# geekieo/collaborative-deep-metric-learning

Hardware: NVIDIA B200
Metric: train_triplets_per_sec (higher is better)
Workload: dtype fp16 operands / fp32 accumulate (tcgen05 kind::f16), fp32 master weights

## Files before the change

collaborative-deep-metric-learning_b200/csrc/gemm_launch.cuh:

```cuda
#pragma once
#include "../../include/cdml.h"
#include "ctx.cuh"
#include "gemm_sm100.cuh"
#include "gemm2_sm100.cuh"

#include <stdlib.h>

namespace cdml {

inline bool trace_on() {
  static int on = -1;
  if (on < 0) on = getenv("CDML_TRACE") != nullptr ? 1 : 0;
  return on == 1;
}
inline int trace_sync(const char* what, long M, long N, long K, int grid, cudaStream_t st) {
  if (!trace_on()) return 0;
  fprintf(stderr, "[cdml] %s M=%ld N=%ld K=%ld grid=%d ... ", what, M, N, K, grid);
  fflush(stderr);
  cudaError_t e = cudaStreamSynchronize(st);
  fprintf(stderr, "%s\n", cudaGetErrorString(e));
  fflush(stderr);
  return e == cudaSuccess ? 0 : -2;
}

constexpr int kBN = 256;
constexpr int kStages = 4;

inline int pick_splits(int num_sms, int tiles, int num_kb) {
  if (tiles >= 2 * num_sms || num_kb < 16) return 1;
  const int smax = max(1, min(64, num_kb / 8));
  int best = 1;
  double best_eff = -1.0;
  for (int s = 1; s <= smax; ++s) {
    const int per = (num_kb + s - 1) / s;
    const int seff = (num_kb + per - 1) / per;
    if (seff != s) continue;
    const long units = static_cast<long>(tiles) * s;
    const long waves = (units + num_sms - 1) / num_sms;
    double eff = static_cast<double>(units) / static_cast<double>(waves * num_sms);
    if (units < num_sms) eff *= 0.5;
    eff -= 0.002 * s;
    if (eff > best_eff) best_eff = eff, best = s;
  }
  return best;
}

inline bool two_cta_enabled() {
  static int on = -1;
  if (on < 0) {
    const char* e = getenv("CDML_2CTA");
    on = (e != nullptr && e[0] == '0') ? 0 : 1;
  }
  return on == 1;
}

template <int AMN, int BMN, class Epi>
static int launch_gemm2(cdml_ctx* ctx, const void* A, int64_t lda, const void* B, int64_t ldb, int64_t M, int64_t N,
                        int64_t K, int dtype16, int num_splits, const Epi& epi, cudaStream_t stream) {
  using L = Gemm2Smem;
  CUtensorMap ta, tb;
  int rc;
  if (AMN == 0) rc = make_tmap_2d(ctx, &ta, A, dtype16, K, M, lda, kBK, kBM);
  else rc = make_tmap_2d(ctx, &ta, A, dtype16, M, K, lda, 64, kBK);
  if (rc) return rc;
  if (BMN == 0) rc = make_tmap_2d(ctx, &tb, B, dtype16, K, N, ldb, kBK, kBN2 / 2);
  else rc = make_tmap_2d(ctx, &tb, B, dtype16, N, K, ldb, 64, kBK);
  if (rc) return rc;
  GemmShape s;
  s.M = static_cast<int>(M), s.N = static_cast<int>(N), s.K = static_cast<int>(K);
  s.m_tiles = (s.M + 2 * kBM - 1) / (2 * kBM);
  s.n_tiles = (s.N + kBN2 - 1) / kBN2;
  s.num_kb = (s.K + kBK - 1) / kBK;
  num_splits = max(1, min(num_splits, s.num_kb));
  s.kb_per_split = (s.num_kb + num_splits - 1) / num_splits;
  s.num_splits = (s.num_kb + s.kb_per_split - 1) / s.kb_per_split;
  s.idesc = make_idesc_f16(dtype16 == CDML_BF16 ? 1 : 0, AMN, BMN, 2 * kBM, kBN2);
  s.m_fastest = (s.num_splits > 1 && N >= M) ? 1 : 0;
  auto kern = gemm2_tcgen05_kernel<AMN, BMN, Epi>;
  static bool attr_set = false;
  if (!attr_set) {
    CDML_CHECK_CUDA(cudaFuncSetAttribute(kern, cudaFuncAttributeMaxDynamicSharedMemorySize, L::kTotal));
    attr_set = true;
  }
  const long units = static_cast<long>(s.m_tiles) * s.n_tiles * s.num_splits;
  const int clusters = static_cast<int>(units < ctx->num_sms / 2 ? units : ctx->num_sms / 2);
  cudaLaunchConfig_t cfg = {};
  cfg.gridDim = dim3(2 * clusters);
  cfg.blockDim = dim3(kGemmThreads);
  cfg.dynamicSmemBytes = L::kTotal;
  cfg.stream = stream;
  cudaLaunchAttribute attr[1];
  attr[0].id = cudaLaunchAttributeClusterDimension;
  attr[0].val.clusterDim.x = 2, attr[0].val.clusterDim.y = 1, attr[0].val.clusterDim.z = 1;
  cfg.attrs = attr;
  cfg.numAttrs = 1;
  CDML_CHECK_CUDA(cudaLaunchKernelEx(&cfg, kern, ta, tb, s, epi));
  if (trace_sync("gemm2_tcgen05", M, N, K, 2 * clusters, stream)) return -2;
  return s.num_splits;
}

template <int AMN, int BMN, class Epi>
static int launch_gemm(cdml_ctx* ctx, const void* A, int64_t lda, const void* B, int64_t ldb, int64_t M, int64_t N,
                       int64_t K, int dtype16, int num_splits, const Epi& epi, cudaStream_t stream) {
  {
    const int64_t kb_per = ((K + kBK - 1) / kBK + max(num_splits, 1) - 1) / max(num_splits, 1);
    if (two_cta_enabled() && M >= 2 * kBM && kb_per >= 8)
      return launch_gemm2<AMN, BMN>(ctx, A, lda, B, ldb, M, N, K, dtype16, num_splits, epi, stream);
  }
  using L = GemmSmem<kBN, kStages>;
  CUtensorMap ta, tb;
  int rc;
  if (AMN == 0) rc = make_tmap_2d(ctx, &ta, A, dtype16, K, M, lda, kBK, kBM);
  else rc = make_tmap_2d(ctx, &ta, A, dtype16, M, K, lda, 64, kBK);
  if (rc) return rc;
  if (BMN == 0) rc = make_tmap_2d(ctx, &tb, B, dtype16, K, N, ldb, kBK, kBN);
  else rc = make_tmap_2d(ctx, &tb, B, dtype16, N, K, ldb, 64, kBK);
  if (rc) return rc;

  GemmShape s;
  s.M = static_cast<int>(M), s.N = static_cast<int>(N), s.K = static_cast<int>(K);
  s.m_tiles = (s.M + kBM - 1) / kBM;
  s.n_tiles = (s.N + kBN - 1) / kBN;
  s.num_kb = (s.K + kBK - 1) / kBK;
  num_splits = max(1, min(num_splits, s.num_kb));
  s.kb_per_split = (s.num_kb + num_splits - 1) / num_splits;
  s.num_splits = (s.num_kb + s.kb_per_split - 1) / s.kb_per_split;
  s.idesc = make_idesc_f16(dtype16 == CDML_BF16 ? 1 : 0, AMN, BMN, kBM, kBN);
  s.m_fastest = (s.num_splits > 1 && N >= M) ? 1 : 0;

  auto kern = gemm_tcgen05_kernel<AMN, BMN, kBN, kStages, Epi>;
  static bool attr_set = false;
  if (!attr_set) {
    CDML_CHECK_CUDA(cudaFuncSetAttribute(kern, cudaFuncAttributeMaxDynamicSharedMemorySize, L::kTotal));
    attr_set = true;
  }
  const long units = static_cast<long>(s.m_tiles) * s.n_tiles * s.num_splits;
  const int grid = static_cast<int>(units < ctx->num_sms ? units : ctx->num_sms);
  kern<<<grid, kGemmThreads, L::kTotal, stream>>>(ta, tb, s, epi);
  CDML_CHECK_CUDA(cudaGetLastError());
  if (trace_sync("gemm_tcgen05", M, N, K, grid, stream)) return -2;
  return s.num_splits;
}

constexpr int kResBStages = 4;
inline bool resb_applicable(int64_t K) {
  static int off = -1;
  if (off < 0) off = getenv("CDML_NO_RESB") != nullptr ? 1 : 0;
  return off == 0 && K <= 4 * kBK;
}

template <class Epi, int kEpiWarps = 8>
static int launch_gemm_resb(cdml_ctx* ctx, const void* A, int64_t lda, const void* B, int64_t ldb, int64_t M, int64_t N,
                            int64_t K, int dtype16, const Epi& epi, cudaStream_t stream, int n_fastest = 0) {
  using L = ResBSmem<kBN, kResBStages, kEpiWarps, Epi::kRowConsts, Epi::kTmaStore ? 2 : 1>;
  static_assert(L::kTotal <= 232448, "resident-B kernel: shared memory over the 227 KB limit");
  CUtensorMap ta, tb;
  int rc = make_tmap_2d(ctx, &ta, A, dtype16, K, M, lda, kBK, kBM);
  if (rc) return rc;
  rc = make_tmap_2d(ctx, &tb, B, dtype16, K, N, ldb, kBK, kBN);
  if (rc) return rc;
  ResBShape s;
  s.M = static_cast<int>(M), s.N = static_cast<int>(N), s.K = static_cast<int>(K);
  s.m_tiles = (s.M + kBM - 1) / kBM;
  s.n_tiles = (s.N + kBN - 1) / kBN;
  s.num_kb = (s.K + kBK - 1) / kBK;
  int best = 1;
  double best_eff = -1.0;
  const int cmax = max(1, min(s.m_tiles / 8, 4 * ctx->num_sms));
  for (int c = 1; c <= cmax; ++c) {
    const int tpc = (s.m_tiles + c - 1) / c;
    const int ceff = (s.m_tiles + tpc - 1) / tpc;
    if (ceff != c) continue;
    const long units = static_cast<long>(s.n_tiles) * c;
    const long waves = (units + ctx->num_sms - 1) / ctx->num_sms;
    double eff = static_cast<double>(units) / static_cast<double>(waves * ctx->num_sms);
    eff -= 0.15 / tpc;
    if (eff > best_eff) best_eff = eff, best = c;
  }
  s.m_chunks = best;
  s.tiles_per_chunk = (s.m_tiles + best - 1) / best;
  s.n_fastest = n_fastest;
  s.idesc = make_idesc_f16(dtype16 == CDML_BF16 ? 1 : 0, 0, 0, kBM, kBN);
  auto kern = gemm_resb_tcgen05_kernel<kBN, kResBStages, Epi, kEpiWarps>;
  static bool attr_set = false;
  if (!attr_set) {
    CDML_CHECK_CUDA(cudaFuncSetAttribute(kern, cudaFuncAttributeMaxDynamicSharedMemorySize, L::kTotal));
    attr_set = true;
  }
  const long units = static_cast<long>(s.n_tiles) * s.m_chunks;
  const int grid = static_cast<int>(units < ctx->num_sms ? units : ctx->num_sms);
  kern<<<grid, 128 + 32 * kEpiWarps, L::kTotal, stream>>>(ta, tb, s, epi);
  CDML_CHECK_CUDA(cudaGetLastError());
  if (trace_sync(Epi::kTmaStore ? "gemm_resb[tma]" : "gemm_resb", M, N, K, grid, stream)) return -2;
  return 1;
}

}
```

collaborative-deep-metric-learning_b200/csrc/gemm_sm100.cuh:

```cuda
#pragma once
#include "common.cuh"

namespace cdml {

constexpr int kBM = 128;
constexpr int kBK = 64;
constexpr int kUK = 16;
constexpr uint32_t kEpiStageBytes = 16384;
constexpr int kGemmThreads = 384;

struct GemmShape {
  int M, N, K;
  int m_tiles, n_tiles;
  int num_kb;
  int kb_per_split;
  int num_splits;
  int m_fastest;
  uint32_t idesc;
};

template <int BN, int kStages>
struct GemmSmem {
  static constexpr uint32_t kABytes = kBM * kBK * 2;
  static constexpr uint32_t kBBytes = BN * kBK * 2;
  static constexpr uint32_t kEpiOff = kStages * (kABytes + kBBytes);
  static constexpr uint32_t kBarOff = kEpiOff + kEpiStageBytes;
  static constexpr uint32_t kNumBars = 2 * kStages + 4;
  static constexpr uint32_t kTotal = kBarOff + kNumBars * 8 + 16 + 1024;
};

__device__ __forceinline__ float leaky(float v, float alpha) { return v > 0.f ? v : alpha * v; }
__device__ __forceinline__ float chunk_bias(const float* bias, int nb, int N) {
  const int col = nb + static_cast<int>(threadIdx.x & 31);
  return (bias != nullptr && col < N) ? __ldg(bias + col) : 0.f;
}

__device__ __forceinline__ void store_chunk16(uint16_t* out, int64_t ld, int row_base, int nb, int M, int N, uint32_t stg,
                                              const uint32_t (&pk)[16]) {
  const int lane = threadIdx.x & 31;
  __syncwarp();
#pragma unroll
  for (int j = 0; j < 4; ++j)
    sts128(stg + lane * 64 + ((j ^ ((lane >> 1) & 3)) << 4), pk[4 * j], pk[4 * j + 1], pk[4 * j + 2], pk[4 * j + 3]);
  __syncwarp();
  const int cch = lane & 3;
  const int col = nb + 8 * cch;
  const bool vec = (ld & 7) == 0;
#pragma unroll
  for (int i = 0; i < 4; ++i) {
    const int r = 8 * i + (lane >> 2);
    const uint4 v = lds128(stg + r * 64 + ((cch ^ ((r >> 1) & 3)) << 4));
    const int grow = row_base + r;
    if (grow < M) {
      uint16_t* p = out + static_cast<int64_t>(grow) * ld + col;
      if (vec && col + 8 <= N) {
        *reinterpret_cast<uint4*>(p) = v;
      } else {
        const uint32_t w[4] = {v.x, v.y, v.z, v.w};
#pragma unroll
        for (int e = 0; e < 8; ++e)
          if (col + e < N) p[e] = static_cast<uint16_t>(w[e >> 1] >> ((e & 1) * 16));
      }
    }
  }
}

__device__ __forceinline__ void store_chunk32(float* out, int64_t ld, int row_base, int nb, int M, int N, uint32_t stg,
                                              const float (&f)[32]) {
  const int lane = threadIdx.x & 31;
  __syncwarp();
#pragma unroll
  for (int j = 0; j < 8; ++j)
    sts128(stg + lane * 128 + ((j ^ (lane & 7)) << 4), __float_as_uint(f[4 * j]), __float_as_uint(f[4 * j + 1]),
           __float_as_uint(f[4 * j + 2]), __float_as_uint(f[4 * j + 3]));
  __syncwarp();
  const int cch = lane & 7;
  const int col = nb + 4 * cch;
  const bool vec = (ld & 3) == 0;
#pragma unroll
  for (int i = 0; i < 8; ++i) {
    const int r = 4 * i + (lane >> 3);
    const uint4 v = lds128(stg + r * 128 + ((cch ^ (r & 7)) << 4));
    const int grow = row_base + r;
    if (grow < M) {
      float* p = out + static_cast<int64_t>(grow) * ld + col;
      if (vec && col + 4 <= N) {
        *reinterpret_cast<uint4*>(p) = v;
      } else {
        const uint32_t w[4] = {v.x, v.y, v.z, v.w};
#pragma unroll
        for (int e = 0; e < 4; ++e)
          if (col + e < N) p[e] = __uint_as_float(w[e]);
      }
    }
  }
}

constexpr uint32_t kColCacheOff = 128, kColTagOff = 640, kWarpSliceBytes = 2048;
__device__ __forceinline__ void col_cache_reset(uint32_t epi_smem) {
  for (int w = 0; w < 8; ++w)
    asm volatile("st.shared.b32 [%0], %1;" ::"r"(epi_smem + w * kWarpSliceBytes + kColTagOff), "r"(0u) : "memory");
}
template <class Fetch>
__device__ __forceinline__ void col_cache_fill(uint32_t stg, int n0, int c0, Fetch&& fetch) {
  uint32_t tag;
  asm volatile("ld.shared.b32 %0, [%1];" : "=r"(tag) : "r"(stg + kColTagOff) : "memory");
  if (tag == static_cast<uint32_t>(n0 + 1)) return;
  const int lane = threadIdx.x & 31;
  __syncwarp();
#pragma unroll
  for (int i = 0; i < 4; ++i) {
    const uint32_t v = fetch(n0 + (c0 + i) * 32 + lane);
    asm volatile("st.shared.b32 [%0], %1;" ::"r"(stg + kColCacheOff + 4 * (32 * i + lane)), "r"(v) : "memory");
  }
  if (lane == 0) asm volatile("st.shared.b32 [%0], %1;" ::"r"(stg + kColTagOff), "r"(n0 + 1) : "memory");
  __syncwarp();
}

template <int BN>
struct EpiStoreF32 {
  static constexpr bool kSplitColumns = true;
  struct State {};
  __device__ __forceinline__ void pre(State&, int, int, const GemmShape&, int, int, uint32_t) const {}
  static constexpr bool kPrefetchNext = false;
  static constexpr bool kRowConsts = false;
  static constexpr bool kEarlyRelease = false;
  static constexpr bool kTmaStore = false;
  __device__ __forceinline__ void cols(int, const GemmShape&, int, int, uint32_t) const {}
  __device__ __forceinline__ void block_begin(uint32_t) const {}
  __device__ __forceinline__ void block_end(uint32_t) const {}
  float* out;
  int64_t ld;
  int64_t split_stride;
  const float* bias;
  float alpha;
  __device__ __forceinline__ void run(uint32_t taddr, int row, int n0, int split, const GemmShape& s, int c0, int c1, uint32_t stg, State& st) const {
    float* orow = out + static_cast<int64_t>(split) * split_stride + static_cast<int64_t>(row) * ld;
    const bool row_ok = row < s.M;
#pragma unroll 1
    for (int c = c0; c < c1; ++c) {
      const int nb = n0 + c * 32;
      if (nb >= s.N) break;
      uint32_t v[32];
      tmem_ld_32x32(taddr + c * 32, v);
      const float b_lane = chunk_bias(bias, nb, s.N);
      tmem_ld_wait();
      float f[32];
#pragma unroll
      for (int j = 0; j < 32; ++j)
        f[j] = leaky(__uint_as_float(v[j]) + __shfl_sync(0xffffffffu, b_lane, j), alpha);
      if (row_ok) {
        if (nb + 32 <= s.N && (ld & 3) == 0) {
          float4* p = reinterpret_cast<float4*>(orow + nb);
#pragma unroll
          for (int j = 0; j < 8; ++j) p[j] = make_float4(f[4 * j], f[4 * j + 1], f[4 * j + 2], f[4 * j + 3]);
        } else {
#pragma unroll
          for (int j = 0; j < 32; ++j)
            if (nb + j < s.N) orow[nb + j] = f[j];
        }
      }
    }
  }
};

template <int BN, int kBf16>
struct EpiStore16 {
  static constexpr bool kSplitColumns = true;
  struct State {};
  __device__ __forceinline__ void pre(State&, int, int, const GemmShape&, int, int, uint32_t) const {}
  static constexpr bool kPrefetchNext = false;
  static constexpr bool kRowConsts = false;
  static constexpr bool kEarlyRelease = false;
  static constexpr bool kTmaStore = false;
  __device__ __forceinline__ void cols(int, const GemmShape&, int, int, uint32_t) const {}
  __device__ __forceinline__ void block_begin(uint32_t) const {}
  __device__ __forceinline__ void block_end(uint32_t) const {}
  uint16_t* out;
  int64_t ld;
  const float* bias;
  float alpha;
  uint32_t* mask_out;
  int64_t ld_mask;
  __device__ __forceinline__ void run(uint32_t taddr, int row, int n0, int , const GemmShape& s, int c0, int c1, uint32_t stg, State& st) const {
#pragma unroll 1
    for (int c = c0; c < c1; ++c) {
      const int nb = n0 + c * 32;
      if (nb >= s.N) break;
      uint32_t v[32];
      tmem_ld_32x32(taddr + c * 32, v);
      const float b_lane = chunk_bias(bias, nb, s.N);
      tmem_ld_wait();
      uint32_t pk[16];
      uint32_t bits = 0u;
#pragma unroll
      for (int j = 0; j < 16; ++j) {
        const float x0 = __uint_as_float(v[2 * j]) + __shfl_sync(0xffffffffu, b_lane, 2 * j);
        const float x1 = __uint_as_float(v[2 * j + 1]) + __shfl_sync(0xffffffffu, b_lane, 2 * j + 1);
        bits |= (x0 > 0.f ? 1u : 0u) << (2 * j);
        bits |= (x1 > 0.f ? 1u : 0u) << (2 * j + 1);
        pk[j] = pack2<kBf16>(leaky(x0, alpha), leaky(x1, alpha));
      }
      if (mask_out != nullptr && row < s.M) mask_out[static_cast<int64_t>(nb >> 5) * ld_mask + row] = bits;
      store_chunk16(out, ld, row - static_cast<int>(threadIdx.x & 31), nb, s.M, s.N, stg, pk);
    }
  }
};

template <int BN, int kBf16>
struct EpiL2Norm {
  static constexpr bool kSplitColumns = false;
  struct State {};
  __device__ __forceinline__ void pre(State&, int, int, const GemmShape&, int, int, uint32_t) const {}
  static constexpr bool kPrefetchNext = false;
  static constexpr bool kRowConsts = false;
  static constexpr bool kEarlyRelease = false;
  static constexpr bool kTmaStore = false;
  __device__ __forceinline__ void cols(int, const GemmShape&, int, int, uint32_t) const {}
  __device__ __forceinline__ void block_begin(uint32_t) const {}
  __device__ __forceinline__ void block_end(uint32_t) const {}
  float* out;
  int64_t ld;
  const float* bias;
  float alpha;
  float* rinv;
  uint16_t* out16;
  int64_t ld16;
  __device__ __forceinline__ void run(uint32_t taddr, int row, int n0, int , const GemmShape& s, int c0, int c1, uint32_t stg, State& st) const {
    const bool row_ok = row < s.M;
    float ss = 0.f;
#pragma unroll 1
    for (int c = c0; c < c1; ++c) {
      const int nb = n0 + c * 32;
      if (nb >= s.N) break;
      uint32_t v[32];
      tmem_ld_32x32(taddr + c * 32, v);
      const float b_lane = chunk_bias(bias, nb, s.N);
      tmem_ld_wait();
#pragma unroll
      for (int j = 0; j < 32; ++j) {
        const float x = leaky(__uint_as_float(v[j]) + __shfl_sync(0xffffffffu, b_lane, j), alpha);
        ss = fmaf(x, x, ss);
      }
    }
    const float r = rsqrtf(fmaxf(ss, 1e-12f));
    if (row_ok && rinv != nullptr) rinv[row] = r;
#pragma unroll 1
    for (int c = c0; c < c1; ++c) {
      const int nb = n0 + c * 32;
      if (nb >= s.N) break;
      uint32_t v[32];
      tmem_ld_32x32(taddr + c * 32, v);
      const float b_lane = chunk_bias(bias, nb, s.N);
      tmem_ld_wait();
      float f[32];
#pragma unroll
      for (int j = 0; j < 32; ++j)
        f[j] = leaky(__uint_as_float(v[j]) + __shfl_sync(0xffffffffu, b_lane, j), alpha) * r;
      store_chunk32(out, ld, row - static_cast<int>(threadIdx.x & 31), nb, s.M, s.N, stg, f);
      if (out16 != nullptr) {
        uint32_t pk[16];
#pragma unroll
        for (int j = 0; j < 16; ++j) pk[j] = pack2<kBf16>(f[2 * j], f[2 * j + 1]);
        store_chunk16(out16, ld16, row - static_cast<int>(threadIdx.x & 31), nb, s.M, s.N, stg, pk);
      }
    }
  }
};

template <int BN, int kBf16>
struct EpiMaskLeaky {
  static constexpr bool kSplitColumns = true;
  struct State {
    uint4 raw[4][4];
  };
  static constexpr bool kPrefetchNext = false;
  static constexpr bool kRowConsts = false;
  static constexpr bool kEarlyRelease = false;
  static constexpr bool kTmaStore = false;
  __device__ __forceinline__ void cols(int, const GemmShape&, int, int, uint32_t) const {}
  __device__ __forceinline__ void block_begin(uint32_t) const {}
  __device__ __forceinline__ void block_end(uint32_t) const {}
  uint16_t* out;
  int64_t ld;
  const uint16_t* mask;
  int64_t ld_mask;
  float alpha;
  __device__ __forceinline__ void fetch_mask(int row_base, int nb, int M, int N, bool active, uint4 (&raw)[4]) const {
    const int lane = threadIdx.x & 31;
    const int col = nb + 8 * (lane & 3);
#pragma unroll
    for (int i = 0; i < 4; ++i) {
      const int grow = row_base + 8 * i + (lane >> 2);
      raw[i] = make_uint4(0u, 0u, 0u, 0u);
      if (active && grow < M) {
        const uint16_t* p = mask + static_cast<int64_t>(grow) * ld_mask + col;
        if ((ld_mask & 7) == 0 && col + 8 <= N) {
          raw[i] = __ldg(reinterpret_cast<const uint4*>(p));
        } else {
          uint32_t w[4] = {0u, 0u, 0u, 0u};
#pragma unroll
          for (int e = 0; e < 8; ++e)
            if (col + e < N) w[e >> 1] |= static_cast<uint32_t>(p[e]) << ((e & 1) * 16);
          raw[i] = make_uint4(w[0], w[1], w[2], w[3]);
        }
      }
    }
  }
  __device__ __forceinline__ void transpose_mask(uint32_t stg, const uint4 (&raw)[4], uint32_t (&mk)[16]) const {
    const int lane = threadIdx.x & 31;
    const int cch = lane & 3;
    __syncwarp();
#pragma unroll
    for (int i = 0; i < 4; ++i) {
      const int r = 8 * i + (lane >> 2);
      sts128(stg + r * 64 + ((cch ^ ((r >> 1) & 3)) << 4), raw[i].x, raw[i].y, raw[i].z, raw[i].w);
    }
    __syncwarp();
#pragma unroll
    for (int j = 0; j < 4; ++j) {
      const uint4 t = lds128(stg + lane * 64 + ((j ^ ((lane >> 1) & 3)) << 4));
      mk[4 * j] = t.x, mk[4 * j + 1] = t.y, mk[4 * j + 2] = t.z, mk[4 * j + 3] = t.w;
    }
  }
  __device__ __forceinline__ void pre(State& st, int row, int n0, const GemmShape& s, int c0, int c1, uint32_t ) const {
    static_assert(BN == 256, "a warp owns 4 chunks of the tile");
    const int row_base = row - static_cast<int>(threadIdx.x & 31);
#pragma unroll
    for (int cc = 0; cc < 4; ++cc)
      fetch_mask(row_base, n0 + (c0 + cc) * 32, s.M, s.N, c0 + cc < c1 && n0 + (c0 + cc) * 32 < s.N, st.raw[cc]);
  }
  __device__ __forceinline__ void run(uint32_t taddr, int row, int n0, int , const GemmShape& s, int c0, int c1,
                                      uint32_t stg, State& st) const {
    const int row_base = row - static_cast<int>(threadIdx.x & 31);
#pragma unroll
    for (int cc = 0; cc < 4; ++cc) {
      const int c = c0 + cc;
      const int nb = n0 + c * 32;
      if (c < c1 && nb < s.N) {
        uint32_t v[32];
        tmem_ld_32x32(taddr + c * 32, v);
        uint32_t mk[16];
        transpose_mask(stg, st.raw[cc], mk);
        tmem_ld_wait();
        uint32_t pk[16];
#pragma unroll
        for (int j = 0; j < 16; ++j) {
          const float2 m = unpack2<kBf16>(mk[j]);
          const float x0 = __uint_as_float(v[2 * j]) * (m.x > 0.f ? 1.f : alpha);
          const float x1 = __uint_as_float(v[2 * j + 1]) * (m.y > 0.f ? 1.f : alpha);
          pk[j] = pack2<kBf16>(x0, x1);
        }
        store_chunk16(out, ld, row_base, nb, s.M, s.N, stg, pk);
      }
    }
  }
};

template <int BN, int kBf16>
struct EpiMaskBits {
  static constexpr bool kSplitColumns = true;
  struct State {
    uint32_t bits[4];
  };
  static constexpr bool kPrefetchNext = true;
  static constexpr bool kRowConsts = false;
  static constexpr bool kEarlyRelease = false;
  static constexpr bool kTmaStore = false;
  __device__ __forceinline__ void cols(int, const GemmShape&, int, int, uint32_t) const {}
  __device__ __forceinline__ void block_begin(uint32_t) const {}
  __device__ __forceinline__ void block_end(uint32_t) const {}
  uint16_t* out;
  int64_t ld;
  const uint32_t* mask;
  int64_t ld_mask;
  float alpha;
  __device__ __forceinline__ void pre(State& st, int row, int n0, const GemmShape& s, int c0, int c1, uint32_t ) const {
    static_assert(BN == 256, "a warp owns 4 chunks of the tile");
#pragma unroll
    for (int cc = 0; cc < 4; ++cc) {
      const int nb = n0 + (c0 + cc) * 32;
      st.bits[cc] = (c0 + cc < c1 && nb < s.N && row < s.M) ? __ldg(mask + static_cast<int64_t>(nb >> 5) * ld_mask + row) : 0u;
    }
  }
  __device__ __forceinline__ void run(uint32_t taddr, int row, int n0, int , const GemmShape& s, int c0, int c1,
                                      uint32_t stg, State& st) const {
    const int row_base = row - static_cast<int>(threadIdx.x & 31);
    auto ok = [&](int cc) { return c0 + cc < c1 && n0 + (c0 + cc) * 32 < s.N; };
    auto chunk = [&](const uint32_t (&v)[32], int cc) {
      const uint32_t b = st.bits[cc];
      uint32_t pk[16];
#pragma unroll
      for (int j = 0; j < 16; ++j) {
        const float x0 = __uint_as_float(v[2 * j]) * ((b >> (2 * j)) & 1u ? 1.f : alpha);
        const float x1 = __uint_as_float(v[2 * j + 1]) * ((b >> (2 * j + 1)) & 1u ? 1.f : alpha);
        pk[j] = pack2<kBf16>(x0, x1);
      }
      store_chunk16(out, ld, row_base, n0 + (c0 + cc) * 32, s.M, s.N, stg, pk);
    };
    uint32_t va[32], vb[32];
    if (ok(0)) tmem_ld_32x32(taddr + c0 * 32, va);
#pragma unroll
    for (int cc = 0; cc < 4; cc += 2) {
      tmem_ld_wait();
      if (ok(cc + 1)) tmem_ld_32x32(taddr + (c0 + cc + 1) * 32, vb);
      if (ok(cc)) chunk(va, cc);
      tmem_ld_wait();
      if (cc + 2 < 4 && ok(cc + 2)) tmem_ld_32x32(taddr + (c0 + cc + 2) * 32, va);
      if (ok(cc + 1)) chunk(vb, cc + 1);
    }
  }
};

template <int BN, int kBf16>
struct EpiMaskBitsTma {
  static constexpr bool kSplitColumns = true;
  struct State {
    uint32_t bits[4];
    uint32_t release_bar;
  };
  static constexpr bool kPrefetchNext = true;
  static constexpr bool kRowConsts = false;
  static constexpr bool kEarlyRelease = true;
  static constexpr bool kTmaStore = true;
  __device__ __forceinline__ void cols(int, const GemmShape&, int, int, uint32_t) const {}
  __device__ __forceinline__ void block_begin(uint32_t) const {}
  __device__ __forceinline__ void block_end(uint32_t) const {}
  CUtensorMap out_map;
  const uint32_t* mask;
  int64_t ld_mask;
  float alpha;
  __device__ __forceinline__ void pre(State& st, int row, int n0, const GemmShape& s, int c0, int c1, uint32_t ) const {
    static_assert(BN == 256, "a warp owns 4 chunks of the tile");
#pragma unroll
    for (int cc = 0; cc < 4; ++cc) {
      const int nb = n0 + (c0 + cc) * 32;
      st.bits[cc] = (c0 + cc < c1 && nb < s.N && row < s.M) ? __ldg(mask + static_cast<int64_t>(nb >> 5) * ld_mask + row) : 0u;
    }
    st.release_bar = 0u;
  }
  __device__ __forceinline__ void run(uint32_t taddr, int row, int n0, int , const GemmShape& s, int c0, int c1,
                                      uint32_t stg0, State& st) const {
    const int lane = threadIdx.x & 31;
    const int row_base = row - lane;
    auto ok = [&](int cc) { return c0 + cc < c1 && n0 + (c0 + cc) * 32 < s.N; };
    const int boxes = ok(0) + ok(1) + ok(2) + ok(3);
    auto chunk = [&](const uint32_t (&v)[32], int cc) {
      const uint32_t b = st.bits[cc];
      uint32_t pk[16];
#pragma unroll
      for (int j = 0; j < 16; ++j) {
        const float x0 = __uint_as_float(v[2 * j]) * ((b >> (2 * j)) & 1u ? 1.f : alpha);
        const float x1 = __uint_as_float(v[2 * j + 1]) * ((b >> (2 * j + 1)) & 1u ? 1.f : alpha);
        pk[j] = pack2<kBf16>(x0, x1);
      }
      const uint32_t stg = stg0 + ((cc + boxes) & 1) * 2048u;
      if (lane == 0) {
        if (cc == 0 && (boxes & 1)) bulk_wait_read0();
        else bulk_wait_read1();
      }
      __syncwarp();
#pragma unroll
      for (int j = 0; j < 4; ++j)
        sts128(stg + lane * 64 + ((j ^ ((lane >> 1) & 3)) << 4), pk[4 * j], pk[4 * j + 1], pk[4 * j + 2], pk[4 * j + 3]);
      fence_proxy_async();
      __syncwarp();
      if (lane == 0) {
        tma_store_2d(&out_map, stg, n0 + (c0 + cc) * 32, row_base);
        bulk_commit();
      }
    };
    uint32_t va[32], vb[32];
    if (ok(0)) tmem_ld_32x32(taddr + c0 * 32, va);
#pragma unroll
    for (int cc = 0; cc < 4; cc += 2) {
      tmem_ld_wait();
      if (ok(cc + 1)) tmem_ld_32x32(taddr + (c0 + cc + 1) * 32, vb);
      if (ok(cc)) chunk(va, cc);
      tmem_ld_wait();
      if (cc + 2 < 4 && ok(cc + 2)) tmem_ld_32x32(taddr + (c0 + cc + 2) * 32, va);
      if (cc + 2 >= 4 && st.release_bar != 0u) {
        tc_fence_before();
        __syncwarp();
        if (lane == 0) mbar_arrive(st.release_bar);
      }
      if (ok(cc + 1)) chunk(vb, cc + 1);
    }
  }
};

template <int BN, int kReadTmem>
struct EpiNull {
  static constexpr bool kSplitColumns = true;
  struct State {};
  __device__ __forceinline__ void pre(State&, int, int, const GemmShape&, int, int, uint32_t) const {}
  static constexpr bool kPrefetchNext = false;
  static constexpr bool kRowConsts = false;
  static constexpr bool kEarlyRelease = false;
  static constexpr bool kTmaStore = false;
  __device__ __forceinline__ void cols(int, const GemmShape&, int, int, uint32_t) const {}
  __device__ __forceinline__ void block_begin(uint32_t) const {}
  __device__ __forceinline__ void block_end(uint32_t) const {}
  float* out;
  __device__ __forceinline__ void run(uint32_t taddr, int row, int n0, int , const GemmShape& s, int c0, int c1, uint32_t stg, State& st) const {
    if (kReadTmem) {
      uint32_t acc = 0u;
#pragma unroll 1
      for (int c = c0; c < c1; ++c) {
        uint32_t v[32];
        tmem_ld_32x32(taddr + c * 32, v);
        tmem_ld_wait();
#pragma unroll
        for (int j = 0; j < 32; ++j) acc ^= v[j];
      }
      if (acc == 0x7fc12345u && row == s.M + 7) out[0] = 1.f;
    }
  }
};

template <int kAMajorMN, int kBMajorMN, int BN, int kStages, class Epi>
__global__ void __launch_bounds__(kGemmThreads, 1)
gemm_tcgen05_kernel(const __grid_constant__ CUtensorMap tma_a, const __grid_constant__ CUtensorMap tma_b,
                    const GemmShape s, const Epi epi) {
  using L = GemmSmem<BN, kStages>;
  extern __shared__ uint8_t smem_raw[];
  const uint32_t raw_u32 = smem_u32(smem_raw);
  const uint32_t base = (raw_u32 + 1023u) & ~1023u;
  const uint32_t bar0 = base + L::kBarOff;
  auto a_smem = [&](int st) { return base + st * L::kABytes; };
  auto b_smem = [&](int st) { return base + kStages * L::kABytes + st * L::kBBytes; };
  auto full_bar = [&](int st) { return bar0 + 8u * st; };
  auto empty_bar = [&](int st) { return bar0 + 8u * (kStages + st); };
  auto tfull_bar = [&](int i) { return bar0 + 8u * (2 * kStages + i); };
  auto tempty_bar = [&](int i) { return bar0 + 8u * (2 * kStages + 2 + i); };
  const uint32_t tmem_slot = bar0 + 8u * L::kNumBars;
  volatile uint32_t* tmem_slot_ptr = reinterpret_cast<volatile uint32_t*>(smem_raw + (tmem_slot - raw_u32));

  const int warp = threadIdx.x >> 5;
  const int lane = threadIdx.x & 31;
  constexpr uint32_t kTmemCols = (2 * BN <= 32) ? 32 : (2 * BN <= 64) ? 64 : (2 * BN <= 128) ? 128 : (2 * BN <= 256) ? 256 : 512;
  static_assert(2 * BN <= 512, "two accumulator stages must fit TMEM");

  if (warp == 0 && lane == 0) {
    tma_prefetch_desc(&tma_a);
    tma_prefetch_desc(&tma_b);
  }
  if (warp == 1 && lane == 0) {
    for (int i = 0; i < kStages; ++i) {
      mbar_init(full_bar(i), 1);
      mbar_init(empty_bar(i), 1);
    }
    for (int i = 0; i < 2; ++i) {
      mbar_init(tfull_bar(i), 1);
      mbar_init(tempty_bar(i), 8);
    }
    fence_mbar_init();
  }
  if (warp == 2) {
    tmem_alloc(tmem_slot, kTmemCols);
    tmem_relinquish();
  }
  if (threadIdx.x == 96) epi.block_begin(base + L::kEpiOff);
  tc_fence_before();
  __syncthreads();
  tc_fence_after();
  const uint32_t tmem_base = *tmem_slot_ptr;

  const int tiles = s.m_tiles * s.n_tiles;
  const int units = tiles * s.num_splits;

  if (warp == 0 && lane == 0) {
    int stage = 0;
    uint32_t phase = 0;
    for (int u = blockIdx.x; u < units; u += gridDim.x) {
      const int split = u / tiles, t = u - split * tiles;
      const int m0 = (s.m_fastest ? t % s.m_tiles : t / s.n_tiles) * kBM;
      const int n0 = (s.m_fastest ? t / s.m_tiles : t % s.n_tiles) * BN;
      const int kb0 = split * s.kb_per_split;
      const int kb1 = min(s.num_kb, kb0 + s.kb_per_split);
      for (int kb = kb0; kb < kb1; ++kb) {
        mbar_wait(empty_bar(stage), phase ^ 1, 100 + stage);
        mbar_arrive_expect_tx(full_bar(stage), L::kABytes + L::kBBytes);
        const int k0 = kb * kBK;
        if constexpr (kAMajorMN == 0) {
          tma_load_2d(a_smem(stage), &tma_a, full_bar(stage), k0, m0);
        } else {
#pragma unroll
          for (int i = 0; i < kBM / 64; ++i)
            tma_load_2d(a_smem(stage) + i * (kBK * 128), &tma_a, full_bar(stage), m0 + i * 64, k0);
        }
        if constexpr (kBMajorMN == 0) {
          tma_load_2d(b_smem(stage), &tma_b, full_bar(stage), k0, n0);
        } else {
#pragma unroll
          for (int i = 0; i < BN / 64; ++i)
            tma_load_2d(b_smem(stage) + i * (kBK * 128), &tma_b, full_bar(stage), n0 + i * 64, k0);
        }
        if (++stage == kStages) stage = 0, phase ^= 1;
      }
    }
  } else if (warp == 1 && lane == 0) {
    int stage = 0;
    uint32_t phase = 0;
    int it = 0;
    constexpr uint32_t kAStep = kAMajorMN ? (kUK * 128) : (kUK * 2);
    constexpr uint32_t kBStep = kBMajorMN ? (kUK * 128) : (kUK * 2);
    constexpr uint32_t kALbo = kAMajorMN ? (kBK * 128) : 16;
    constexpr uint32_t kBLbo = kBMajorMN ? (kBK * 128) : 16;
    for (int u = blockIdx.x; u < units; u += gridDim.x, ++it) {
      const int split = u / tiles;
      const int kb0 = split * s.kb_per_split;
      const int kb1 = min(s.num_kb, kb0 + s.kb_per_split);
      const int as = it & 1;
      const uint32_t ap = (it >> 1) & 1;
      mbar_wait(tempty_bar(as), ap ^ 1, 200 + as);
      tc_fence_after();
      const uint32_t tmem_d = tmem_base + as * BN;
      for (int kb = kb0; kb < kb1; ++kb) {
        mbar_wait(full_bar(stage), phase, 300 + stage);
        tc_fence_after();
#pragma unroll
        for (int k = 0; k < kBK / kUK; ++k) {
          const uint64_t ad = make_smem_desc(a_smem(stage) + k * kAStep, kALbo, 1024);
          const uint64_t bd = make_smem_desc(b_smem(stage) + k * kBStep, kBLbo, 1024);
          umma_f16(tmem_d, ad, bd, s.idesc, (kb > kb0 || k > 0) ? 1u : 0u);
        }
        tc_commit(empty_bar(stage));
        if (kb == kb1 - 1) tc_commit(tfull_bar(as));
        if (++stage == kStages) stage = 0, phase ^= 1;
      }
    }
  } else if (warp >= 4) {
    const int q = warp & 3;
    const int half = (warp - 4) >> 2;
    const uint32_t stg = base + L::kEpiOff + (warp - 4) * (Epi::kSplitColumns ? 2048u : 4096u);
    int it = 0;
    for (int u = blockIdx.x; u < units; u += gridDim.x, ++it) {
      const int split = u / tiles, t = u - split * tiles;
      const int m0 = (s.m_fastest ? t % s.m_tiles : t / s.n_tiles) * kBM;
      const int n0 = (s.m_fastest ? t / s.m_tiles : t % s.n_tiles) * BN;
      const int as = it & 1;
      const uint32_t ap = (it >> 1) & 1;
      const int ec0 = Epi::kSplitColumns ? half * (BN / 64) : 0, ec1 = Epi::kSplitColumns ? (half + 1) * (BN / 64) : BN / 32;
      typename Epi::State est;
      if (Epi::kSplitColumns || half == 0) {
        epi.cols(n0, s, ec0, ec1, stg);
        epi.pre(est, m0 + q * 32 + lane, n0, s, ec0, ec1, stg);
      }
      mbar_wait(tfull_bar(as), ap, 400 + as);
      tc_fence_after();
      const uint32_t taddr = tmem_base + (static_cast<uint32_t>(q * 32) << 16) + as * BN;
      if (Epi::kSplitColumns || half == 0) epi.run(taddr, m0 + q * 32 + lane, n0, split, s, ec0, ec1, stg, est);
      tc_fence_before();
      __syncwarp();
      if (lane == 0) mbar_arrive(tempty_bar(as));
    }
  }

  tc_fence_before();
  __syncthreads();
  if (threadIdx.x == 96) epi.block_end(base + L::kEpiOff);
  if (warp == 2) {
    tc_fence_after();
    tmem_dealloc(tmem_base, kTmemCols);
  }
}

struct ResBShape {
  int M, N, K;
  int m_tiles, n_tiles, num_kb;
  int m_chunks;
  int tiles_per_chunk;
  int n_fastest;
  uint32_t idesc;
};

template <int BN, int kAStages, int kEpiWarps = 8, bool kRowSlots = false, int kStageSlices = 1>
struct ResBSmem {
  static constexpr uint32_t kABytes = kBM * kBK * 2;
  static constexpr uint32_t kBPanel = BN * kBK * 2;
  static constexpr uint32_t kMaxKb = 4;
  static constexpr uint32_t kEpiOff = kMaxKb * kBPanel + kAStages * kABytes;
  static constexpr uint32_t kEpiBytes = kEpiWarps * 2048 * kStageSlices;
  static constexpr uint32_t kRowConstOff = kEpiOff + kEpiBytes;
  static constexpr uint32_t kRowConstSlot = kRowSlots ? kBM * 32 : 0;
  static constexpr uint32_t kBarOff = kRowConstOff + 2 * kRowConstSlot;
  static constexpr uint32_t kNumBars = 2 * kAStages + 2 + 4 + 2;
  static constexpr uint32_t kTotal = kBarOff + kNumBars * 8 + 16 + 1024;
};

template <int BN, int kAStages, class Epi, int kEpiWarps = 8>
__global__ void __launch_bounds__(128 + 32 * kEpiWarps, 1)
gemm_resb_tcgen05_kernel(const __grid_constant__ CUtensorMap tma_a, const __grid_constant__ CUtensorMap tma_b,
                         const ResBShape s, const __grid_constant__ Epi epi) {
  using L = ResBSmem<BN, kAStages, kEpiWarps, Epi::kRowConsts, Epi::kTmaStore ? 2 : 1>;
  static_assert(kEpiWarps == 8 || kEpiWarps == 16, "two or four epilogue warps per TMEM lane quarter");
  static_assert(kEpiWarps == 8 || Epi::kSplitColumns, "four warps per quarter split the tile's columns");
  extern __shared__ uint8_t smem_raw[];
  const uint32_t raw_u32 = smem_u32(smem_raw);
  const uint32_t base = (raw_u32 + 1023u) & ~1023u;
  const uint32_t bar0 = base + L::kBarOff;
  auto b_panel = [&](int kb) { return base + kb * L::kBPanel; };
  auto a_smem = [&](int st) { return base + L::kMaxKb * L::kBPanel + st * L::kABytes; };
  auto a_full = [&](int st) { return bar0 + 8u * st; };
  auto a_empty = [&](int st) { return bar0 + 8u * (kAStages + st); };
  const uint32_t b_full = bar0 + 8u * (2 * kAStages);
  const uint32_t b_empty = bar0 + 8u * (2 * kAStages + 1);
  auto tfull_bar = [&](int i) { return bar0 + 8u * (2 * kAStages + 2 + i); };
  auto tempty_bar = [&](int i) { return bar0 + 8u * (2 * kAStages + 4 + i); };
  auto cfull_bar = [&](int i) { return bar0 + 8u * (2 * kAStages + 6 + i); };
  auto cslot = [&](int i) { return base + L::kRowConstOff + i * L::kRowConstSlot; };
  const uint32_t tmem_slot = bar0 + 8u * L::kNumBars;
  volatile uint32_t* tmem_slot_ptr = reinterpret_cast<volatile uint32_t*>(smem_raw + (tmem_slot - raw_u32));
  const int warp = threadIdx.x >> 5;
  const int lane = threadIdx.x & 31;
  constexpr uint32_t kTmemCols = 512;
  static_assert(2 * BN <= 512, "two accumulator stages must fit TMEM");

  if (warp == 0 && lane == 0) {
    tma_prefetch_desc(&tma_a);
    tma_prefetch_desc(&tma_b);
  }
  if (warp == 1 && lane == 0) {
    for (int i = 0; i < kAStages; ++i) {
      mbar_init(a_full(i), 1);
      mbar_init(a_empty(i), 1);
    }
    mbar_init(b_full, 1);
    mbar_init(b_empty, 1);
    for (int i = 0; i < 2; ++i) {
      mbar_init(tfull_bar(i), 1);
      mbar_init(tempty_bar(i), kEpiWarps);
      mbar_init(cfull_bar(i), 1);
    }
    fence_mbar_init();
  }
  if (warp == 2) {
    tmem_alloc(tmem_slot, kTmemCols);
    tmem_relinquish();
  }
  if (threadIdx.x == 96) epi.block_begin(base + L::kEpiOff);
  tc_fence_before();
  __syncthreads();
  tc_fence_after();
  const uint32_t tmem_base = *tmem_slot_ptr;

  const int units = s.n_tiles * s.m_chunks;
  if (warp == 0 && lane == 0) {
    int stage = 0;
    uint32_t phase = 0, bphase = 0;
    for (int u = blockIdx.x; u < units; u += gridDim.x) {
      const int chunk = s.n_fastest ? u / s.n_tiles : u % s.m_chunks, nblk = s.n_fastest ? u % s.n_tiles : u / s.m_chunks;
      const int t0 = chunk * s.tiles_per_chunk, t1 = min(s.m_tiles, t0 + s.tiles_per_chunk);
      if (t0 >= t1) continue;
      mbar_wait(b_empty, bphase ^ 1, 500);
      mbar_arrive_expect_tx(b_full, s.num_kb * L::kBPanel);
      for (int kb = 0; kb < s.num_kb; ++kb) tma_load_2d(b_panel(kb), &tma_b, b_full, kb * kBK, nblk * BN);
      bphase ^= 1;
      for (int t = t0; t < t1; ++t) {
        for (int kb = 0; kb < s.num_kb; ++kb) {
          mbar_wait(a_empty(stage), phase ^ 1, 100 + stage);
          mbar_arrive_expect_tx(a_full(stage), L::kABytes);
          tma_load_2d(a_smem(stage), &tma_a, a_full(stage), kb * kBK, t * kBM);
          if (++stage == kAStages) stage = 0, phase ^= 1;
        }
      }
    }
  } else if (warp == 1 && lane == 0) {
    int stage = 0, it = 0;
    uint32_t phase = 0, bphase = 0;
    for (int u = blockIdx.x; u < units; u += gridDim.x) {
      const int chunk = s.n_fastest ? u / s.n_tiles : u % s.m_chunks, nblk = s.n_fastest ? u % s.n_tiles : u / s.m_chunks;
      const int t0 = chunk * s.tiles_per_chunk, t1 = min(s.m_tiles, t0 + s.tiles_per_chunk);
      if (t0 >= t1) continue;
      mbar_wait(b_full, bphase, 600);
      bphase ^= 1;
      tc_fence_after();
      for (int t = t0; t < t1; ++t, ++it) {
        const int as = it & 1;
        const uint32_t ap = (it >> 1) & 1;
        mbar_wait(tempty_bar(as), ap ^ 1, 200 + as);
        tc_fence_after();
        const uint32_t tmem_d = tmem_base + as * BN;
        for (int kb = 0; kb < s.num_kb; ++kb) {
          mbar_wait(a_full(stage), phase, 300 + stage);
          tc_fence_after();
#pragma unroll
          for (int k = 0; k < kBK / kUK; ++k) {
            const uint64_t ad = make_smem_desc(a_smem(stage) + k * (kUK * 2), 16, 1024);
            const uint64_t bd = make_smem_desc(b_panel(kb) + k * (kUK * 2), 16, 1024);
            umma_f16(tmem_d, ad, bd, s.idesc, (kb > 0 || k > 0) ? 1u : 0u);
          }
          tc_commit(a_empty(stage));
          if (kb == s.num_kb - 1) tc_commit(tfull_bar(as));
          if (++stage == kAStages) stage = 0, phase ^= 1;
        }
      }
      tc_commit(b_empty);
    }
  } else if (warp == 3) {
   if constexpr (Epi::kRowConsts) {
    int it = 0;
    GemmShape gs;
    gs.M = s.M, gs.N = s.N, gs.K = s.K;
    for (int u = blockIdx.x; u < units; u += gridDim.x) {
      const int chunk = s.n_fastest ? u / s.n_tiles : u % s.m_chunks;
      const int t0 = chunk * s.tiles_per_chunk, t1 = min(s.m_tiles, t0 + s.tiles_per_chunk);
      for (int t = t0; t < t1; ++t, ++it) {
        const int as = it & 1;
        const uint32_t ap = (it >> 1) & 1;
        mbar_wait(tempty_bar(as), ap ^ 1, 700 + as);
#pragma unroll
        for (int r = lane; r < kBM; r += 32) epi.row_consts(t * kBM + r, gs, cslot(as) + r * 32);
        __syncwarp();
        if (lane == 0) mbar_arrive(cfull_bar(as));
      }
    }
   }
  } else if (warp >= 4) {
    const int q = warp & 3;
    const int half = (warp - 4) >> 2;
    const uint32_t stg = base + L::kEpiOff + (warp - 4) * (Epi::kTmaStore ? 4096u : (Epi::kSplitColumns || kEpiWarps == 16) ? 2048u : 4096u);
    int it = 0;
    GemmShape gs;
    gs.M = s.M, gs.N = s.N, gs.K = s.K, gs.m_tiles = s.m_tiles, gs.n_tiles = s.n_tiles, gs.num_kb = s.num_kb;
    gs.kb_per_split = s.num_kb, gs.num_splits = 1, gs.m_fastest = 0, gs.idesc = s.idesc;
    struct TileIter {
      int u, t, t1, nblk;
      bool valid;
    };
    auto seek = [&](TileIter& ti) {
      ti.valid = false;
      for (; ti.u < units; ti.u += gridDim.x) {
        const int chunk = s.n_fastest ? ti.u / s.n_tiles : ti.u % s.m_chunks;
        const int t0 = chunk * s.tiles_per_chunk, t1 = min(s.m_tiles, t0 + s.tiles_per_chunk);
        if (t0 < t1) {
          ti.t = t0, ti.t1 = t1, ti.nblk = s.n_fastest ? ti.u % s.n_tiles : ti.u / s.m_chunks, ti.valid = true;
          return;
        }
      }
    };
    const bool active = Epi::kSplitColumns || half == 0;
    constexpr int kChunksPerWarp = (BN / 32) / (kEpiWarps / 4);
    const int ec0 = Epi::kSplitColumns ? half * kChunksPerWarp : 0, ec1 = Epi::kSplitColumns ? (half + 1) * kChunksPerWarp : BN / 32;
    TileIter cur;
    cur.u = blockIdx.x;
    seek(cur);
    typename Epi::State est;
    if (cur.valid && active) {
      epi.cols(cur.nblk * BN, gs, ec0, ec1, stg);
      if constexpr (!Epi::kRowConsts) epi.pre(est, cur.t * kBM + q * 32 + lane, cur.nblk * BN, gs, ec0, ec1, stg);
    }
    while (cur.valid) {
      TileIter nxt = cur;
      if (++nxt.t >= nxt.t1) {
        nxt.u += gridDim.x;
        seek(nxt);
      }
      const int as = it & 1;
      const uint32_t ap = (it >> 1) & 1;
      typename Epi::State est_next;
      if constexpr (Epi::kRowConsts) {
        mbar_wait(cfull_bar(as), ap, 800 + as);
        if (active) epi.load_state(est, cslot(as) + (q * 32 + lane) * 32);
        est_next = est;
      }
      mbar_wait(tfull_bar(as), ap, 400 + as);
      tc_fence_after();
      const uint32_t taddr = tmem_base + (static_cast<uint32_t>(q * 32) << 16) + as * BN;
      if (active) {
        if constexpr (!Epi::kRowConsts)
          if (Epi::kPrefetchNext && nxt.valid) epi.pre(est_next, nxt.t * kBM + q * 32 + lane, nxt.nblk * BN, gs, ec0, ec1, stg);
        if constexpr (Epi::kEarlyRelease) est.release_bar = tempty_bar(as);
        epi.run(taddr, cur.t * kBM + q * 32 + lane, cur.nblk * BN, 0, gs, ec0, ec1, stg, est);
      }
      if (!(Epi::kEarlyRelease && active)) {
        tc_fence_before();
        __syncwarp();
        if (lane == 0) mbar_arrive(tempty_bar(as));
      }
      if (active && nxt.valid) {
        epi.cols(nxt.nblk * BN, gs, ec0, ec1, stg);
        if constexpr (!Epi::kRowConsts)
          if (!Epi::kPrefetchNext) epi.pre(est_next, nxt.t * kBM + q * 32 + lane, nxt.nblk * BN, gs, ec0, ec1, stg);
      }
      est = est_next;
      cur = nxt;
      ++it;
    }
    if constexpr (Epi::kTmaStore) {
      if (lane == 0) bulk_wait_all();
    }
  }

  tc_fence_before();
  __syncthreads();
  if (threadIdx.x == 96) epi.block_end(base + L::kEpiOff);
  if (warp == 2) {
    tc_fence_after();
    tmem_dealloc(tmem_base, kTmemCols);
  }
}

}
```

collaborative-deep-metric-learning_b200/csrc/knn.cu:

```cuda
#include <math.h>
#include <string.h>

#include <algorithm>

#include <vector>

#include "gemm_launch.cuh"

namespace cdml {

constexpr int kCandCap = 2048;
constexpr int kKeepCap = 2048;
constexpr int kMaxGroups = 4096;
constexpr int kRefineThreads = 256;

__device__ __forceinline__ uint32_t f2key(float f) {
  const uint32_t u = __float_as_uint(f);
  return (u & 0x80000000u) ? ~u : (u | 0x80000000u);
}
__device__ __forceinline__ float key2f(uint32_t k) {
  return __uint_as_float((k & 0x80000000u) ? (k & 0x7FFFFFFFu) : ~k);
}
__device__ __forceinline__ float neg_inf() { return __int_as_float(0xff800000); }
__device__ __forceinline__ float pos_inf() { return __int_as_float(0x7f800000); }

__device__ __forceinline__ float4 ld4_or(const float* p, int col, int N, float fill) {
  if (col + 4 <= N) return __ldg(reinterpret_cast<const float4*>(p + col));
  float4 r;
  r.x = col < N ? __ldg(p + col) : fill;
  r.y = col + 1 < N ? __ldg(p + col + 1) : fill;
  r.z = col + 2 < N ? __ldg(p + col + 2) : fill;
  r.w = col + 3 < N ? __ldg(p + col + 3) : fill;
  return r;
}

template <int BN>
struct EpiKnnGroupMax {
  static constexpr bool kSplitColumns = true;
  static constexpr bool kPrefetchNext = false;
  static constexpr bool kRowConsts = false;
  static constexpr bool kEarlyRelease = false;
  static constexpr bool kTmaStore = false;
  struct State {};
  __device__ __forceinline__ void pre(State&, int, int, const GemmShape&, int, int, uint32_t) const {}
  __device__ __forceinline__ void block_begin(uint32_t epi_smem) const { col_cache_reset(epi_smem); }
  __device__ __forceinline__ void block_end(uint32_t) const {}
  const float* h;
  float* gmax;
  int64_t ldg;
  int wide;
  __device__ __forceinline__ void cols(int n0, const GemmShape& s, int c0, int , uint32_t stg) const {
    static_assert(BN == 256, "a warp owns 4 chunks (128 columns) of the tile");
    col_cache_fill(stg, n0, c0, [&](int col) { return __float_as_uint(col < s.N ? __ldg(h + col) : pos_inf()); });
  }
  __device__ __forceinline__ void run(uint32_t taddr, int row, int n0, int , const GemmShape& s, int c0,
                                      int , uint32_t stg, State& ) const {
    float g[4];
    uint32_t va[32], vb[32];
    auto group = [&](const uint32_t (&v)[32], int cc) {
      const uint32_t hbase = stg + kColCacheOff + 128 * cc;
      float b0 = neg_inf(), b1 = neg_inf();
#pragma unroll
      for (int j = 0; j < 8; ++j) {
        const uint4 t = lds128(hbase + 16 * j);
        const float2 lo = sub2(__uint_as_float(v[4 * j]), __uint_as_float(v[4 * j + 1]), __uint_as_float(t.x), __uint_as_float(t.y));
        const float2 hi = sub2(__uint_as_float(v[4 * j + 2]), __uint_as_float(v[4 * j + 3]), __uint_as_float(t.z), __uint_as_float(t.w));
        b0 = fmax3(b0, lo.x, lo.y);
        b1 = fmax3(b1, hi.x, hi.y);
      }
      return fmaxf(b0, b1);
    };
    auto ok = [&](int cc) { return n0 + (c0 + cc) * 32 < s.N; };
    tmem_ld_32x32(taddr + c0 * 32, va);
#pragma unroll
    for (int cc = 0; cc < 4; cc += 2) {
      tmem_ld_wait();
      if (ok(cc + 1)) tmem_ld_32x32(taddr + (c0 + cc + 1) * 32, vb);
      g[cc] = ok(cc) ? group(va, cc) : neg_inf();
      tmem_ld_wait();
      if (cc + 2 < 4 && ok(cc + 2)) tmem_ld_32x32(taddr + (c0 + cc + 2) * 32, va);
      g[cc + 1] = ok(cc + 1) ? group(vb, cc + 1) : neg_inf();
    }
    if (row < s.M) {
      if (wide) gmax[static_cast<int64_t>(row) * ldg + n0 / 128 + c0 / 4] = fmaxf(fmaxf(g[0], g[1]), fmaxf(g[2], g[3]));
      else *reinterpret_cast<float4*>(gmax + static_cast<int64_t>(row) * ldg + n0 / 32 + c0) = make_float4(g[0], g[1], g[2], g[3]);
    }
  }
};

constexpr uint32_t kKnnWarpStage = kWarpSliceBytes;
constexpr uint32_t kKnnThrOff = kColCacheOff, kKnnCurOff = 644;
constexpr int kKnnLogsPerCta = 8;

template <int BN>
struct EpiKnnCollect {
  static constexpr bool kSplitColumns = true;
  const float* h;
  const float* thr;
  uint4* log;
  int32_t* log_count;
  int32_t* log_overflow;
  unsigned int warp_cap;
  struct State {
    float hr;
    uint32_t release_bar;
  };
  static constexpr bool kPrefetchNext = true;
  static constexpr bool kRowConsts = false;
  static constexpr bool kEarlyRelease = true;
  static constexpr bool kTmaStore = false;
  __device__ __forceinline__ void block_begin(uint32_t epi_smem) const {
    col_cache_reset(epi_smem);
    for (int w = 0; w < kKnnLogsPerCta; ++w)
      asm volatile("st.shared.b32 [%0], %1;" ::"r"(epi_smem + w * kKnnWarpStage + kKnnCurOff), "r"(0u) : "memory");
  }
  __device__ __forceinline__ void block_end(uint32_t epi_smem) const {
    for (int w = 0; w < kKnnLogsPerCta; ++w) {
      unsigned int n;
      asm volatile("ld.shared.b32 %0, [%1];" : "=r"(n) : "r"(epi_smem + w * kKnnWarpStage + kKnnCurOff) : "memory");
      log_count[blockIdx.x * kKnnLogsPerCta + w] = static_cast<int32_t>(n < warp_cap ? n : warp_cap);
      if (n > warp_cap) atomicOr(log_overflow, 1);
    }
  }
  __device__ __forceinline__ void pre(State& st, int row, int, const GemmShape& s, int, int, uint32_t) const {
    st.hr = row < s.M ? __ldg(h + row) : pos_inf();
    st.release_bar = 0u;
  }
  __device__ __forceinline__ void cols(int n0, const GemmShape& s, int c0, int , uint32_t stg) const {
    static_assert(BN == 256, "a warp owns 4 chunks (128 columns) of the tile");
    col_cache_fill(stg, n0, c0, [&](int col) { return __float_as_uint(col < s.N ? __ldg(thr + col) : pos_inf()); });
  }
  __device__ __forceinline__ void run(uint32_t taddr, int row, int n0, int , const GemmShape& s, int c0,
                                      int c1, uint32_t stg, State& st) const {
    const float hr = st.hr;
    const int lane = threadIdx.x & 31;
    const int warp_slot = (threadIdx.x >> 5) - 4;
    uint4* my_log = log + (static_cast<size_t>(blockIdx.x) * kKnnLogsPerCta + warp_slot) * warp_cap;
    unsigned int cursor;
    asm volatile("ld.shared.b32 %0, [%1];" : "=r"(cursor) : "r"(stg + kKnnCurOff) : "memory");
    uint32_t va[32], vb[32];
    tmem_ld_32x32(taddr + c0 * 32, va);
    auto chunk = [&](const uint32_t (&v)[32], int cc) {
      const int nb = n0 + (c0 + cc) * 32;
      const uint32_t tbase = stg + kKnnThrOff + 128 * cc;
      float m0 = neg_inf(), m1 = neg_inf();
#pragma unroll
      for (int j = 0; j < 8; ++j) {
        const uint4 t = lds128(tbase + 16 * j);
        const float2 lo = sub2(__uint_as_float(v[4 * j]), __uint_as_float(v[4 * j + 1]), __uint_as_float(t.x), __uint_as_float(t.y));
        const float2 hi = sub2(__uint_as_float(v[4 * j + 2]), __uint_as_float(v[4 * j + 3]), __uint_as_float(t.z), __uint_as_float(t.w));
        m0 = fmax3(m0, lo.x, lo.y);
        m1 = fmax3(m1, hi.x, hi.y);
      }
      unsigned int hits = __ballot_sync(0xffffffffu, fmaxf(m0, m1) > hr);
      if (hits != 0u) {
        float thr_lane;
        asm volatile("ld.shared.f32 %0, [%1];" : "=f"(thr_lane) : "r"(tbase + 4 * lane) : "memory");
        do {
          const int src = __ffs(hits) - 1;
          hits &= hits - 1u;
          __syncwarp();
          if (lane == src) {
#pragma unroll
            for (int j = 0; j < 8; ++j) sts128(stg + 16 * j, v[4 * j], v[4 * j + 1], v[4 * j + 2], v[4 * j + 3]);
          }
          __syncwarp();
          float val;
          asm volatile("ld.shared.f32 %0, [%1];" : "=f"(val) : "r"(stg + 4 * lane) : "memory");
          const float hr_src = __shfl_sync(0xffffffffu, hr, src);
          const bool pass = val - thr_lane > hr_src;
          const unsigned int pm = __ballot_sync(0xffffffffu, pass);
          const unsigned int pos = cursor + static_cast<unsigned int>(__popc(pm & ((1u << lane) - 1u)));
          if (pass && pos < warp_cap)
            my_log[pos] = make_uint4(static_cast<uint32_t>(nb + lane), static_cast<uint32_t>(row - lane + src),
                                     __float_as_uint(val - hr_src), 0u);
          cursor += static_cast<unsigned int>(__popc(pm));
        } while (hits != 0u);
      }
    };
#pragma unroll
    for (int cc = 0; cc < 4; cc += 2) {
      const bool ok0 = c0 + cc < c1 && n0 + (c0 + cc) * 32 < s.N;
      const bool ok1 = c0 + cc + 1 < c1 && n0 + (c0 + cc + 1) * 32 < s.N;
      const bool ok2 = cc + 2 < 4 && c0 + cc + 2 < c1 && n0 + (c0 + cc + 2) * 32 < s.N;
      tmem_ld_wait();
      if (ok1) tmem_ld_32x32(taddr + (c0 + cc + 1) * 32, vb);
      if (ok0) chunk(va, cc);
      tmem_ld_wait();
      if (ok2) tmem_ld_32x32(taddr + (c0 + cc + 2) * 32, va);
      if (cc + 2 >= 4 && st.release_bar != 0u) {
        tc_fence_before();
        __syncwarp();
        if (lane == 0) mbar_arrive(st.release_bar);
      }
      if (ok1) chunk(vb, cc + 1);
    }
    __syncwarp();
    if (lane == 0) asm volatile("st.shared.b32 [%0], %1;" ::"r"(stg + kKnnCurOff), "r"(cursor) : "memory");
  }
};

__global__ void __launch_bounds__(256)
knn_bin_kernel(const uint4* __restrict__ log, const int32_t* __restrict__ log_count, unsigned int log_cap,
               int32_t* __restrict__ cand_idx, float* __restrict__ cand_val, int32_t* __restrict__ cnt, int cap) {
  const int n = log_count[blockIdx.y];
  const uint4* my = log + static_cast<size_t>(blockIdx.y) * log_cap;
  for (int i = blockIdx.x * blockDim.x + threadIdx.x; i < n; i += gridDim.x * blockDim.x) {
    const uint4 e = my[i];
    const int pos = atomicAdd(cnt + e.x, 1);
    if (pos < cap) {
      cand_idx[static_cast<int64_t>(e.x) * cap + pos] = static_cast<int32_t>(e.y);
      cand_val[static_cast<int64_t>(e.x) * cap + pos] = __uint_as_float(e.z);
    }
  }
}

__global__ void __launch_bounds__(256)
row_sumsq32_kernel(const float* __restrict__ X, int64_t n, int d, int64_t ld, float* __restrict__ ss, float half_scale,
                   float* __restrict__ half_out) {
  const int warp = threadIdx.x >> 5, lane = threadIdx.x & 31;
  for (int64_t r = static_cast<int64_t>(blockIdx.x) * 8 + warp; r < n; r += static_cast<int64_t>(gridDim.x) * 8) {
    const float* x = X + r * ld;
    float a = 0.f;
    for (int j = lane; j < d; j += 32) a = fmaf(x[j], x[j], a);
#pragma unroll
    for (int o = 16; o > 0; o >>= 1) a += __shfl_xor_sync(0xffffffffu, a, o);
    if (lane == 0) {
      ss[r] = a;
      if (half_out != nullptr) half_out[r] = a * half_scale;
    }
  }
}

__global__ void max_reduce_kernel(const float* __restrict__ x, int64_t n, float* __restrict__ out) {
  __shared__ float sh[32];
  float m = 0.f;
  for (int64_t i = threadIdx.x; i < n; i += blockDim.x) m = fmaxf(m, x[i]);
#pragma unroll
  for (int o = 16; o > 0; o >>= 1) m = fmaxf(m, __shfl_xor_sync(0xffffffffu, m, o));
  if ((threadIdx.x & 31) == 0) sh[threadIdx.x >> 5] = m;
  __syncthreads();
  if (threadIdx.x < 32) {
    m = threadIdx.x < (blockDim.x >> 5) ? sh[threadIdx.x] : 0.f;
#pragma unroll
    for (int o = 16; o > 0; o >>= 1) m = fmaxf(m, __shfl_xor_sync(0xffffffffu, m, o));
    if (threadIdx.x == 0) *out = m;
  }
}

__global__ void fill_f32_kernel(float* p, int64_t n, float v) {
  for (int64_t i = static_cast<int64_t>(blockIdx.x) * blockDim.x + threadIdx.x; i < n;
       i += static_cast<int64_t>(gridDim.x) * blockDim.x)
    p[i] = v;
}

__device__ __forceinline__ int block_sum(int v, int* sh) {
  v = __reduce_add_sync(0xffffffffu, v);
  __syncthreads();
  if ((threadIdx.x & 31) == 0) sh[threadIdx.x >> 5] = v;
  __syncthreads();
  int t = 0;
  for (int w = 0; w < (blockDim.x >> 5); ++w) t += sh[w];
  return t;
}

constexpr int kSelectBits = 20;
template <int kPer, bool kDual>
__global__ void __launch_bounds__(kRefineThreads)
knn_kth_kernel(const float* __restrict__ gmax, int64_t ldg, int G, int k, int k2, const float* __restrict__ qss,
               float slack_scale, float slack_abs, float* __restrict__ thr, float* __restrict__ thr2, float sign2) {
  __shared__ int sh[kRefineThreads / 32];
  const int q = blockIdx.x;
  const float* g = gmax + static_cast<int64_t>(q) * ldg;
  uint32_t keys[kPer];
#pragma unroll
  for (int i = 0; i < kPer; ++i) {
    const int j = threadIdx.x + i * kRefineThreads;
    keys[i] = j < G ? f2key(g[j]) : 0u;
  }
  uint32_t T = 0, T2 = 0;
  for (int bit = 31; bit >= 32 - kSelectBits; --bit) {
    const uint32_t cand = T | (1u << bit), cand2 = T2 | (1u << bit);
    int c = 0;
#pragma unroll
    for (int i = 0; i < kPer; ++i) c += (keys[i] >= cand ? 1 : 0) + (kDual && keys[i] >= cand2 ? 65536 : 0);
    c = block_sum(c, sh);
    if ((c & 0xffff) >= k) T = cand;
    if (kDual && (c >> 16) >= k2) T2 = cand2;
  }
  if (threadIdx.x == 0) {
    const float slack = slack_scale * sqrtf(qss[q]) + slack_abs;
    thr[q] = T > f2key(neg_inf()) ? key2f(T) - slack : neg_inf();
    if (kDual) thr2[q] = sign2 * (T2 > f2key(neg_inf()) ? key2f(T2) - slack : neg_inf());
  }
}

template <bool kDual>
__global__ void __launch_bounds__(256)
knn_kth_warp_kernel(const float* __restrict__ gmax, int64_t ldg, int G, int k, int k2, const float* __restrict__ qss,
                    int64_t nq, float slack_scale, float slack_abs, float* __restrict__ thr, float* __restrict__ thr2,
                    float sign2) {
  const int lane = threadIdx.x & 31;
  const int64_t q = static_cast<int64_t>(blockIdx.x) * 8 + (threadIdx.x >> 5);
  if (q >= nq) return;
  const float* g = gmax + q * ldg;
  uint32_t keys[32];
#pragma unroll
  for (int i = 0; i < 32; ++i) {
    const int j = lane + 32 * i;
    keys[i] = j < G ? f2key(g[j]) : 0u;
  }
  uint32_t T = 0, T2 = 0;
  for (int bit = 31; bit >= 32 - kSelectBits; --bit) {
    const uint32_t cand = T | (1u << bit), cand2 = T2 | (1u << bit);
    int c = 0;
#pragma unroll
    for (int i = 0; i < 32; ++i) c += (keys[i] >= cand ? 1 : 0) + (kDual && keys[i] >= cand2 ? 65536 : 0);
    c = __reduce_add_sync(0xffffffffu, c);
    if ((c & 0xffff) >= k) T = cand;
    if (kDual && (c >> 16) >= k2) T2 = cand2;
  }
  if (lane == 0) {
    const float slack = slack_scale * sqrtf(qss[q]) + slack_abs;
    thr[q] = T > f2key(neg_inf()) ? key2f(T) - slack : neg_inf();
    if (kDual) thr2[q] = sign2 * (T2 > f2key(neg_inf()) ? key2f(T2) - slack : neg_inf());
  }
}

__global__ void __launch_bounds__(256)
knn_nominee_kth_kernel(const float* __restrict__ cand_val, const int32_t* __restrict__ cnt, int cap, int k, int k2,
                       int64_t nq, float* __restrict__ pair) {
  const int lane = threadIdx.x & 31;
  const int64_t q = static_cast<int64_t>(blockIdx.x) * 8 + (threadIdx.x >> 5);
  if (q >= nq) return;
  const int n = cnt[q];
  float a = neg_inf(), b = neg_inf();
  if (n <= cap && n >= min(k, k2)) {
    const float* v = cand_val + q * cap;
    uint32_t keys[8];
    const bool in_regs = n <= 256;
#pragma unroll
    for (int i = 0; i < 8; ++i) keys[i] = (in_regs && lane + 32 * i < n) ? f2key(v[lane + 32 * i]) : 0u;
    uint32_t T = 0, T2 = 0;
    for (int bit = 31; bit >= 32 - kSelectBits; --bit) {
      const uint32_t cand = T | (1u << bit), cand2 = T2 | (1u << bit);
      int c = 0;
      if (in_regs) {
#pragma unroll
        for (int i = 0; i < 8; ++i) c += (keys[i] >= cand ? 1 : 0) + (keys[i] >= cand2 ? 65536 : 0);
      } else {
        for (int i = lane; i < n; i += 32) {
          const uint32_t key = f2key(v[i]);
          c += (key >= cand ? 1 : 0) + (key >= cand2 ? 65536 : 0);
        }
      }
      c = __reduce_add_sync(0xffffffffu, c);
      if ((c & 0xffff) >= k) T = cand;
      if ((c >> 16) >= k2) T2 = cand2;
    }
    if (n >= k && T > f2key(neg_inf())) a = key2f(T);
    if (n >= k2 && T2 > f2key(neg_inf())) b = key2f(T2);
  }
  if (lane == 0) pair[q] = a, pair[nq + q] = -b;
}

__global__ void knn_thr_combine_kernel(const float* __restrict__ full, const float* __restrict__ part,
                                       const float* __restrict__ qss, int64_t n, float slack_scale, float slack_abs,
                                       float* __restrict__ thr, float part_sign) {
  const int64_t i = static_cast<int64_t>(blockIdx.x) * blockDim.x + threadIdx.x;
  if (i >= n) return;
  const float b = fmaxf(full[i], part_sign * part[i]);
  thr[i] = b > neg_inf() ? b - (slack_scale * sqrtf(qss[i]) + slack_abs) : neg_inf();
}

__global__ void __launch_bounds__(kRefineThreads)
knn_refine_kernel(const float* __restrict__ Q, int64_t ldq, int d, const float* __restrict__ qss,
                  const float* __restrict__ X, int64_t ldx, const float* __restrict__ xss,
                  const int32_t* __restrict__ cand_idx, const float* __restrict__ cand_val,
                  const int32_t* __restrict__ cnt, int cap, int k, int metric, float slack_scale, float slack_abs,
                  int64_t id_offset, float* __restrict__ D, int64_t* __restrict__ I, int64_t out_ld,
                  int32_t* __restrict__ overflow, int n_all, const float* __restrict__ prune_pair, int64_t prune_ld,
                  const int32_t* __restrict__ handled) {
  __shared__ unsigned long long kept[kKeepCap];
  __shared__ int sh[kRefineThreads / 32];
  __shared__ uint32_t shu[2 * (kRefineThreads / 32)];
  __shared__ int n_keep;
  const int q = blockIdx.x;
  const int tid = threadIdx.x;
  if (handled != nullptr && handled[q] != 0) return;
  const int n = n_all > 0 ? 0 : cnt[q];
  if (n > cap) {
    if (tid == 0) overflow[q] = 1;
    return;
  }
  constexpr int kPer = kCandCap / kRefineThreads;
  uint32_t keys[kPer];
  int32_t idxs[kPer];
  uint32_t kmax = 0u, kmin = 0xffffffffu;
#pragma unroll
  for (int t = 0; t < kPer; ++t) {
    const int i = tid + t * kRefineThreads;
    keys[t] = 0u, idxs[t] = 0;
    if (i < n) {
      keys[t] = f2key(cand_val[static_cast<int64_t>(q) * cap + i]);
      idxs[t] = cand_idx[static_cast<int64_t>(q) * cap + i];
      kmax = max(kmax, keys[t]), kmin = min(kmin, keys[t]);
    }
  }
  if (tid == 0) n_keep = 0;
  uint32_t T = 0;
  if (n > k) {
    kmax = __reduce_max_sync(0xffffffffu, kmax), kmin = __reduce_min_sync(0xffffffffu, kmin);
    if ((tid & 31) == 0) shu[tid >> 5] = kmax, shu[kRefineThreads / 32 + (tid >> 5)] = kmin;
    __syncthreads();
#pragma unroll
    for (int w = 0; w < kRefineThreads / 32; ++w) kmax = max(kmax, shu[w]), kmin = min(kmin, shu[kRefineThreads / 32 + w]);
    const uint32_t diff = kmax ^ kmin;
    const int top = diff == 0u ? -1 : 31 - __clz(diff);
    T = top >= 31 ? 0u : (kmax >> (top + 1)) << (top + 1);
    for (int bit = top; bit >= 32 - kSelectBits; --bit) {
      const uint32_t cand = T | (1u << bit);
      int c = 0;
#pragma unroll
      for (int t = 0; t < kPer; ++t) c += keys[t] >= cand ? 1 : 0;
      if (block_sum(c, sh) >= k) T = cand;
    }
  } else {
    __syncthreads();
  }
  const float slack = slack_scale * sqrtf(qss[q]) + slack_abs;
  uint32_t keep_key = n > k ? f2key(key2f(T) - slack) : 0u;
  if (prune_pair != nullptr) {
    const float tg = fmaxf(prune_pair[q], -prune_pair[prune_ld + q]);
    if (tg > neg_inf()) keep_key = max(keep_key, f2key(tg - slack));
  }
#pragma unroll
  for (int t = 0; t < kPer; ++t) {
    if (tid + t * kRefineThreads < n && keys[t] >= keep_key) {
      const int pos = atomicAdd(&n_keep, 1);
      if (pos < kKeepCap) kept[pos] = static_cast<unsigned long long>(static_cast<uint32_t>(idxs[t]));
    }
  }
  if (n_all > 0) {
    for (int i = tid; i < n_all; i += kRefineThreads) kept[i] = static_cast<unsigned long long>(i);
    if (tid == 0) n_keep = n_all;
  }
  __syncthreads();
  const int nk = n_keep;
  if (nk > kKeepCap) {
    if (tid == 0) overflow[q] = 1;
    return;
  }
  const int warp = tid >> 5, lane = tid & 31;
  const float* qv = Q + static_cast<int64_t>(q) * ldq;
  const float qn = qss[q];
  const bool vec = (d & 3) == 0 && (ldx & 3) == 0 && (ldq & 3) == 0 &&
                   ((reinterpret_cast<uintptr_t>(X) | reinterpret_cast<uintptr_t>(Q)) & 15) == 0;
  for (int i0 = warp * 4; i0 < nk; i0 += (kRefineThreads / 32) * 4) {
    uint32_t id[4];
    float dot[4] = {0.f, 0.f, 0.f, 0.f};
#pragma unroll
    for (int c = 0; c < 4; ++c) id[c] = static_cast<uint32_t>(kept[min(i0 + c, nk - 1)]);
    if (vec) {
      for (int j = lane * 4; j < d; j += 128) {
        const float4 qq = __ldg(reinterpret_cast<const float4*>(qv + j));
        float4 xx[4];
#pragma unroll
        for (int c = 0; c < 4; ++c) xx[c] = __ldg(reinterpret_cast<const float4*>(X + static_cast<int64_t>(id[c]) * ldx + j));
#pragma unroll
        for (int c = 0; c < 4; ++c)
          dot[c] = fmaf(qq.x, xx[c].x, fmaf(qq.y, xx[c].y, fmaf(qq.z, xx[c].z, fmaf(qq.w, xx[c].w, dot[c]))));
      }
    } else {
      for (int j = lane; j < d; j += 32) {
        const float qj = qv[j];
#pragma unroll
        for (int c = 0; c < 4; ++c) dot[c] = fmaf(qj, X[static_cast<int64_t>(id[c]) * ldx + j], dot[c]);
      }
    }
#pragma unroll
    for (int c = 0; c < 4; ++c) {
#pragma unroll
      for (int o = 16; o > 0; o >>= 1) dot[c] += __shfl_xor_sync(0xffffffffu, dot[c], o);
    }
    __syncwarp();
    if (lane < 4 && i0 + lane < nk) {
      const float dsel = lane == 0 ? dot[0] : lane == 1 ? dot[1] : lane == 2 ? dot[2] : dot[3];
      const uint32_t isel = lane == 0 ? id[0] : lane == 1 ? id[1] : lane == 2 ? id[2] : id[3];
      const float key = metric == 0 ? fmaxf(qn + xss[isel] - 2.f * dsel, 0.f) : -dsel;
      kept[i0 + lane] = (static_cast<unsigned long long>(f2key(key)) << 32) | isel;
    }
  }
  __syncthreads();
  const auto emit = [&](int i, unsigned long long e) {
    const float key = key2f(static_cast<uint32_t>(e >> 32));
    D[static_cast<int64_t>(q) * out_ld + i] = metric == 0 ? key : -key;
    I[static_cast<int64_t>(q) * out_ld + i] = static_cast<int64_t>(static_cast<uint32_t>(e)) + id_offset;
  };
  if (nk <= 2 * kRefineThreads) {
    for (int i = tid; i < nk; i += kRefineThreads) {
      const unsigned long long e = kept[i];
      int rank = 0;
      for (int j = 0; j < nk; ++j) rank += kept[j] < e ? 1 : 0;
      if (rank < k) emit(rank, e);
    }
  } else {
    int P = 2;
    while (P < nk) P <<= 1;
    for (int i = nk + tid; i < P; i += kRefineThreads) kept[i] = ~0ull;
    __syncthreads();
    for (int size = 2; size <= P; size <<= 1) {
      for (int stride = size >> 1; stride > 0; stride >>= 1) {
        for (int t = tid; t < (P >> 1); t += kRefineThreads) {
          const int lo = ((t / stride) * (stride << 1)) + (t % stride);
          const int hi = lo + stride;
          const bool up = (lo & size) == 0;
          const unsigned long long a = kept[lo], b = kept[hi];
          if ((a > b) == up) kept[lo] = b, kept[hi] = a;
        }
        __syncthreads();
      }
    }
    for (int i = tid; i < k && i < nk; i += kRefineThreads) emit(i, kept[i]);
  }
  for (int i = nk + tid; i < k; i += kRefineThreads) {
    D[static_cast<int64_t>(q) * out_ld + i] = metric == 0 ? pos_inf() : neg_inf();
    I[static_cast<int64_t>(q) * out_ld + i] = -1;
  }
}

constexpr int kWarpNom = 256;
constexpr int kWarpKeep = 96;
__global__ void __launch_bounds__(256)
knn_refine_warp_kernel(const float* __restrict__ Q, int64_t ldq, int d, const float* __restrict__ qss,
                       const float* __restrict__ X, int64_t ldx, const float* __restrict__ xss,
                       const int32_t* __restrict__ cand_idx, const float* __restrict__ cand_val,
                       const int32_t* __restrict__ cnt, int cap, int k, int metric, float slack_scale, float slack_abs,
                       int64_t id_offset, float* __restrict__ D, int64_t* __restrict__ I, int64_t out_ld,
                       const float* __restrict__ prune_pair, int64_t prune_ld, int64_t nq, int32_t* __restrict__ handled) {
  __shared__ unsigned long long kept_all[8][kWarpKeep];
  const int warp = threadIdx.x >> 5, lane = threadIdx.x & 31;
  const int64_t q = static_cast<int64_t>(blockIdx.x) * 8 + warp;
  if (q >= nq) return;
  unsigned long long* kept = kept_all[warp];
  const int n = cnt[q];
  const float tg = fmaxf(prune_pair[q], -prune_pair[prune_ld + q]);
  if (n > kWarpNom || n > cap || !(tg > neg_inf())) {
    if (lane == 0) handled[q] = 0;
    return;
  }
  const float slack = slack_scale * sqrtf(qss[q]) + slack_abs;
  const uint32_t keep_key = f2key(tg - slack);
  int nk = 0;
#pragma unroll
  for (int t = 0; t < kWarpNom / 32; ++t) {
    const int i = lane + 32 * t;
    const bool pass = i < n && f2key(cand_val[q * cap + i]) >= keep_key;
    const unsigned int m = __ballot_sync(0xffffffffu, pass);
    const int pos = nk + __popc(m & ((1u << lane) - 1u));
    if (pass && pos < kWarpKeep) kept[pos] = static_cast<unsigned long long>(static_cast<uint32_t>(cand_idx[q * cap + i]));
    nk += __popc(m);
  }
  if (nk > kWarpKeep) {
    if (lane == 0) handled[q] = 0;
    return;
  }
  __syncwarp();
  const float* qv = Q + q * ldq;
  const float qn = qss[q];
  const bool vec = (d & 3) == 0 && (ldx & 3) == 0 && (ldq & 3) == 0 &&
                   ((reinterpret_cast<uintptr_t>(X) | reinterpret_cast<uintptr_t>(Q)) & 15) == 0;
  for (int i0 = 0; i0 < nk; i0 += 4) {
    uint32_t id[4];
    float dot[4] = {0.f, 0.f, 0.f, 0.f};
#pragma unroll
    for (int c = 0; c < 4; ++c) id[c] = static_cast<uint32_t>(kept[min(i0 + c, nk - 1)]);
    if (vec) {
      for (int j = lane * 4; j < d; j += 128) {
        const float4 qq = __ldg(reinterpret_cast<const float4*>(qv + j));
        float4 xx[4];
#pragma unroll
        for (int c = 0; c < 4; ++c) xx[c] = __ldg(reinterpret_cast<const float4*>(X + static_cast<int64_t>(id[c]) * ldx + j));
#pragma unroll
        for (int c = 0; c < 4; ++c)
          dot[c] = fmaf(qq.x, xx[c].x, fmaf(qq.y, xx[c].y, fmaf(qq.z, xx[c].z, fmaf(qq.w, xx[c].w, dot[c]))));
      }
    } else {
      for (int j = lane; j < d; j += 32) {
        const float qj = qv[j];
#pragma unroll
        for (int c = 0; c < 4; ++c) dot[c] = fmaf(qj, X[static_cast<int64_t>(id[c]) * ldx + j], dot[c]);
      }
    }
#pragma unroll
    for (int c = 0; c < 4; ++c) {
#pragma unroll
      for (int o = 16; o > 0; o >>= 1) dot[c] += __shfl_xor_sync(0xffffffffu, dot[c], o);
    }
    __syncwarp();
    if (lane < 4 && i0 + lane < nk) {
      const float dsel = lane == 0 ? dot[0] : lane == 1 ? dot[1] : lane == 2 ? dot[2] : dot[3];
      const uint32_t isel = lane == 0 ? id[0] : lane == 1 ? id[1] : lane == 2 ? id[2] : id[3];
      const float key = metric == 0 ? fmaxf(qn + xss[isel] - 2.f * dsel, 0.f) : -dsel;
      kept[i0 + lane] = (static_cast<unsigned long long>(f2key(key)) << 32) | isel;
    }
    __syncwarp();
  }
  for (int i = lane; i < nk; i += 32) {
    const unsigned long long e = kept[i];
    int rank = 0;
    for (int j = 0; j < nk; ++j) rank += kept[j] < e ? 1 : 0;
    if (rank < k) {
      const float key = key2f(static_cast<uint32_t>(e >> 32));
      D[q * out_ld + rank] = metric == 0 ? key : -key;
      I[q * out_ld + rank] = static_cast<int64_t>(static_cast<uint32_t>(e)) + id_offset;
    }
  }
  for (int i = nk + lane; i < k; i += 32) {
    D[q * out_ld + i] = metric == 0 ? pos_inf() : neg_inf();
    I[q * out_ld + i] = -1;
  }
  if (lane == 0) handled[q] = 1;
}

constexpr int kFbQueries = 8;
constexpr int kFbThreads = 256;
constexpr int kFbRound = (kFbThreads / 32) * 32;

__global__ void __launch_bounds__(kFbThreads)
knn_exact_batch_kernel(const int32_t* __restrict__ qlist, int nlist, const float* __restrict__ Q, int64_t ldq, int d,
                       const float* __restrict__ X, int64_t N, int64_t ldx, const float* __restrict__ xss, int metric,
                       int k, int kcap, int64_t id_offset, float* __restrict__ D, int64_t* __restrict__ I, int compact_out) {
  extern __shared__ unsigned long long fb_smem[];
  unsigned long long* buf = fb_smem;
  float* qs = reinterpret_cast<float*>(buf + kFbQueries * 2 * kcap);
  __shared__ uint32_t thr_key[kFbQueries];
  __shared__ int cnt[kFbQueries];
  __shared__ float qnorm[kFbQueries];
  const int tid = threadIdx.x, warp = tid >> 5, lane = tid & 31;
  const int q0 = blockIdx.x * kFbQueries;
  const int nqs = min(kFbQueries, nlist - q0);
  const int cap = 2 * kcap;
  for (int i = tid; i < kFbQueries * d; i += kFbThreads) {
    const int j = i / d;
    qs[i] = j < nqs ? Q[static_cast<int64_t>(qlist[q0 + j]) * ldq + (i - j * d)] : 0.f;
  }
  if (tid < kFbQueries) thr_key[tid] = 0xffffffffu, cnt[tid] = 0;
  __syncthreads();
  if (warp < kFbQueries) {
    float a = 0.f;
    for (int c = lane; c < d; c += 32) a = fmaf(qs[warp * d + c], qs[warp * d + c], a);
#pragma unroll
    for (int o = 16; o > 0; o >>= 1) a += __shfl_xor_sync(0xffffffffu, a, o);
    if (lane == 0) qnorm[warp] = a;
  }
  __syncthreads();
  auto compact = [&](int j) {
    const int n = min(cnt[j], cap);
    unsigned long long* b = buf + static_cast<size_t>(j) * cap;
    int P = 2;
    while (P < n) P <<= 1;
    for (int i = n + tid; i < P; i += kFbThreads) b[i] = ~0ull;
    __syncthreads();
    for (int size = 2; size <= P; size <<= 1)
      for (int stride = size >> 1; stride > 0; stride >>= 1) {
        for (int t = tid; t < (P >> 1); t += kFbThreads) {
          const int lo = ((t / stride) * (stride << 1)) + (t % stride), hi = lo + stride;
          const bool up = (lo & size) == 0;
          const unsigned long long x = b[lo], y = b[hi];
          if ((x > y) == up) b[lo] = y, b[hi] = x;
        }
        __syncthreads();
      }
    if (tid == 0) {
      const int keep = min(n, k);
      cnt[j] = keep;
      if (keep == k) thr_key[j] = static_cast<uint32_t>(b[k - 1] >> 32);
    }
    __syncthreads();
  };
  const int64_t row_lo = N * blockIdx.y / gridDim.y, row_hi = N * (blockIdx.y + 1) / gridDim.y;
  float qreg[kFbQueries][8];
#pragma unroll
  for (int j = 0; j < kFbQueries; ++j)
#pragma unroll
    for (int p = 0; p < 8; ++p) qreg[j][p] = (d <= 256 && lane + 32 * p < d) ? qs[j * d + lane + 32 * p] : 0.f;
  for (int64_t r0 = row_lo; r0 < row_hi; r0 += kFbRound) {
    auto offer = [&](int64_t r, const float (&dot)[kFbQueries]) {
      if (lane < nqs) {
        float dsel = dot[0];
#pragma unroll
        for (int j = 1; j < kFbQueries; ++j) dsel = lane == j ? dot[j] : dsel;
        const float key = metric == 0 ? fmaxf(qnorm[lane] + xss[r] - 2.f * dsel, 0.f) : -dsel;
        const uint32_t kk = f2key(key);
        if (kk <= thr_key[lane]) {
          const int pos = atomicAdd(&cnt[lane], 1);
          if (pos < cap) buf[static_cast<size_t>(lane) * cap + pos] = (static_cast<unsigned long long>(kk) << 32) | static_cast<uint32_t>(r);
        }
      }
    };
    if (d <= 256) {
      for (int rr = 0; rr < 32; rr += 4) {
        const int64_t rb = r0 + warp * 32 + rr;
        if (rb >= row_hi) break;
        float x[4][8];
#pragma unroll
        for (int a = 0; a < 4; ++a) {
          const float* xv = X + min(rb + a, row_hi - 1) * ldx;
#pragma unroll
          for (int p = 0; p < 8; ++p) x[a][p] = lane + 32 * p < d ? __ldg(xv + lane + 32 * p) : 0.f;
        }
#pragma unroll
        for (int a = 0; a < 4; ++a) {
          float dot[kFbQueries];
#pragma unroll
          for (int j = 0; j < kFbQueries; ++j) {
            float t = 0.f;
#pragma unroll
            for (int p = 0; p < 8; ++p) t = fmaf(x[a][p], qreg[j][p], t);
#pragma unroll
            for (int o = 16; o > 0; o >>= 1) t += __shfl_xor_sync(0xffffffffu, t, o);
            dot[j] = t;
          }
          if (rb + a < row_hi) offer(rb + a, dot);
        }
      }
    } else {
      for (int rr = 0; rr < 32; ++rr) {
        const int64_t r = r0 + warp * 32 + rr;
        if (r >= row_hi) break;
        const float* xv = X + r * ldx;
        float dot[kFbQueries];
#pragma unroll
        for (int j = 0; j < kFbQueries; ++j) dot[j] = 0.f;
        for (int c = lane; c < d; c += 32) {
          const float x = __ldg(xv + c);
#pragma unroll
          for (int j = 0; j < kFbQueries; ++j) dot[j] = fmaf(x, qs[j * d + c], dot[j]);
        }
#pragma unroll
        for (int j = 0; j < kFbQueries; ++j) {
#pragma unroll
          for (int o = 16; o > 0; o >>= 1) dot[j] += __shfl_xor_sync(0xffffffffu, dot[j], o);
        }
        offer(r, dot);
      }
    }
    __syncthreads();
    unsigned int need = 0u;
    for (int j = 0; j < nqs; ++j) need |= (cnt[j] + kFbRound > cap ? 1u : 0u) << j;
    __syncthreads();
    for (int j = 0; j < nqs; ++j)
      if ((need >> j) & 1u) compact(j);
  }
  for (int j = 0; j < nqs; ++j) {
    compact(j);
    const int64_t q = compact_out ? static_cast<int64_t>(blockIdx.y) * nlist + q0 + j : qlist[q0 + j];
    const int have = cnt[j];
    for (int i = tid; i < k; i += kFbThreads) {
      if (i < have) {
        const unsigned long long e = buf[static_cast<size_t>(j) * cap + i];
        const float key = key2f(static_cast<uint32_t>(e >> 32));
        D[q * k + i] = metric == 0 ? key : -key;
        I[q * k + i] = static_cast<int64_t>(static_cast<uint32_t>(e)) + id_offset;
      } else {
        D[q * k + i] = metric == 0 ? pos_inf() : neg_inf();
        I[q * k + i] = -1;
      }
    }
    __syncthreads();
  }
}

__global__ void knn_scatter_rows_kernel(const int32_t* __restrict__ qlist, int nlist, int k, const float* __restrict__ Dm,
                                        const int64_t* __restrict__ Im, float* __restrict__ D, int64_t* __restrict__ I) {
  const int64_t i = static_cast<int64_t>(blockIdx.x) * blockDim.x + threadIdx.x;
  if (i >= static_cast<int64_t>(nlist) * k) return;
  const int64_t q = qlist[i / k];
  D[q * k + i % k] = Dm[i], I[q * k + i % k] = Im[i];
}

__global__ void __launch_bounds__(256)
knn_merge_kernel(const float* __restrict__ Dg, const int64_t* __restrict__ Ig, int G, int64_t nq, int k, int metric,
                 float* __restrict__ D, int64_t* __restrict__ I) {
  extern __shared__ unsigned long long mk[];
  const int64_t q = blockIdx.x;
  const int tid = threadIdx.x;
  const int n = G * k;
  int P = 2;
  while (P < n) P <<= 1;
  unsigned long long* key = mk;
  int* src = reinterpret_cast<int*>(mk + P);
  for (int i = tid; i < P; i += 256) {
    if (i < n) {
      const int g = i / k, j = i % k;
      const int64_t off = (static_cast<int64_t>(g) * nq + q) * k + j;
      const int64_t id = Ig[off];
      const float dv = Dg[off];
      key[i] = id < 0 ? ~0ull : ((static_cast<unsigned long long>(f2key(metric == 0 ? dv : -dv)) << 32) |
                                 static_cast<uint32_t>(id));
    } else {
      key[i] = ~0ull;
    }
    src[i] = i;
  }
  __syncthreads();
  for (int size = 2; size <= P; size <<= 1) {
    for (int stride = size >> 1; stride > 0; stride >>= 1) {
      for (int t = tid; t < (P >> 1); t += 256) {
        const int lo = ((t / stride) * (stride << 1)) + (t % stride);
        const int hi = lo + stride;
        const bool up = (lo & size) == 0;
        const unsigned long long a = key[lo], b = key[hi];
        if ((a > b) == up) {
          key[lo] = b, key[hi] = a;
          const int s = src[lo];
          src[lo] = src[hi], src[hi] = s;
        }
      }
      __syncthreads();
    }
  }
  for (int i = tid; i < k; i += 256) {
    const int s = src[i];
    if (key[i] != ~0ull && s < n) {
      const int g = s / k, j = s % k;
      const int64_t off = (static_cast<int64_t>(g) * nq + q) * k + j;
      D[q * k + i] = Dg[off];
      I[q * k + i] = Ig[off];
    } else {
      D[q * k + i] = metric == 0 ? pos_inf() : neg_inf();
      I[q * k + i] = -1;
    }
  }
}

__global__ void knn_any_overflow_kernel(const int32_t* __restrict__ overflow, int64_t n, const int32_t* __restrict__ log_overflow,
                                        int32_t* __restrict__ flag) {
  int any = (threadIdx.x == 0 && *log_overflow != 0) ? 1 : 0;
  for (int64_t i = threadIdx.x; i < n; i += blockDim.x) any |= overflow[i] != 0 ? 1 : 0;
  if (__syncthreads_or(any) && threadIdx.x == 0) *flag = 1;
}

__global__ void knn_pack_kernel(const float* __restrict__ D, const int64_t* __restrict__ I, int64_t n, int metric,
                                unsigned long long* __restrict__ rec) {
  const int64_t i = static_cast<int64_t>(blockIdx.x) * blockDim.x + threadIdx.x;
  if (i >= n) return;
  const int64_t id = I[i];
  const float dv = D[i];
  rec[i] = id < 0 ? ~0ull : ((static_cast<unsigned long long>(f2key(metric == 0 ? dv : -dv)) << 32) | static_cast<uint32_t>(id));
}

__global__ void knn_unpack_kernel(const unsigned long long* __restrict__ rec, int64_t n, int metric, float* __restrict__ D,
                                  int64_t* __restrict__ I) {
  const int64_t i = static_cast<int64_t>(blockIdx.x) * blockDim.x + threadIdx.x;
  if (i >= n) return;
  const unsigned long long e = rec[i];
  if (e == ~0ull) {
    D[i] = metric == 0 ? pos_inf() : neg_inf();
    I[i] = -1;
  } else {
    const float key = key2f(static_cast<uint32_t>(e >> 32));
    D[i] = metric == 0 ? key : -key;
    I[i] = static_cast<int64_t>(static_cast<uint32_t>(e));
  }
}

__global__ void __launch_bounds__(256)
knn_merge_packed_kernel(const unsigned long long* __restrict__ rec, int G, int64_t nq, int k, int metric, int warps,
                        float* __restrict__ D, int64_t* __restrict__ I, unsigned long long* __restrict__ rec_out) {
  extern __shared__ unsigned long long ms[];
  const int warp = threadIdx.x >> 5, lane = threadIdx.x & 31;
  if (warp >= warps) return;
  const int64_t q = static_cast<int64_t>(blockIdx.x) * warps + warp;
  if (q >= nq) return;
  unsigned long long* mine = ms + static_cast<size_t>(warp) * G * k;
  for (int g = 0; g < G; ++g)
    for (int j = lane; j < k; j += 32) mine[g * k + j] = rec[(static_cast<int64_t>(g) * nq + q) * k + j];
  __syncwarp();
  int pos = 0;
  unsigned long long head = lane < G ? mine[lane * k] : ~0ull;
  for (int i = 0; i < k; ++i) {
    const uint32_t hi = static_cast<uint32_t>(head >> 32);
    const uint32_t mhi = __reduce_min_sync(0xffffffffu, hi);
    const uint32_t lo = hi == mhi ? static_cast<uint32_t>(head) : 0xffffffffu;
    const uint32_t mlo = __reduce_min_sync(0xffffffffu, lo);
    const bool win = hi == mhi && static_cast<uint32_t>(head) == mlo && head != ~0ull;
    const unsigned int who = __ballot_sync(0xffffffffu, win);
    if (who == 0u) {
      if (lane == 0) {
        if (rec_out != nullptr) {
          rec_out[q * k + i] = ~0ull;
        } else {
          D[q * k + i] = metric == 0 ? pos_inf() : neg_inf();
          I[q * k + i] = -1;
        }
      }
      continue;
    }
    if (lane == __ffs(who) - 1) {
      if (rec_out != nullptr) {
        rec_out[q * k + i] = head;
      } else {
        const float key = key2f(mhi);
        D[q * k + i] = metric == 0 ? key : -key;
        I[q * k + i] = static_cast<int64_t>(mlo);
      }
      ++pos;
      head = pos < k ? mine[lane * k + pos] : ~0ull;
    }
  }
}

template <typename T>
static int dev_alloc(T** p, size_t n) {
  CDML_CHECK_CUDA(cudaMalloc(reinterpret_cast<void**>(p), n * sizeof(T)));
  return 0;
}

}

using namespace cdml;

struct cdml_index {
  cdml_ctx* ctx;
  int64_t N;
  int d, dpad, metric;
  float* x32;
  float* xss;
  float* h;
  uint16_t* x16;
  int64_t Ns;
  uint16_t* xs16;
  float* hs;
  float xmaxnorm;
  int64_t qc;
  uint16_t* q16;
  float *qss, *gmax, *thr, *cand_val;
  int32_t *cand_idx, *cnt, *overflow, *handled;
  uint4* log;
  int32_t* log_count;
  unsigned int log_cap;
  int32_t *h_cnt, *h_ovf, *h_logovf;
  float* h_qss;
  int64_t h_cap;
  int64_t ldg;
  int64_t stats[2];
  float* Dtmp;
  int64_t* Itmp;
  int64_t tmp_cap;
};

static void index_free(cdml_index* ix) {
  if (ix == nullptr) return;
  cudaFree(ix->x32), cudaFree(ix->xss), cudaFree(ix->h), cudaFree(ix->x16), cudaFree(ix->xs16), cudaFree(ix->hs);
  cudaFree(ix->q16), cudaFree(ix->qss), cudaFree(ix->gmax), cudaFree(ix->thr), cudaFree(ix->cand_val);
  cudaFree(ix->cand_idx), cudaFree(ix->cnt), cudaFree(ix->overflow), cudaFree(ix->handled);
  cudaFree(ix->log), cudaFree(ix->log_count);
  cudaFree(ix->Dtmp), cudaFree(ix->Itmp);
  cudaFreeHost(ix->h_cnt), cudaFreeHost(ix->h_ovf), cudaFreeHost(ix->h_qss), cudaFreeHost(ix->h_logovf);
  delete ix;
}

extern "C" {

int cdml_knn_index_build(cdml_ctx* ctx, const float* X, int64_t N, int d, int64_t ldx, int metric, void* stream,
                         cdml_index** out) {
  CDML_REQUIRE(ctx && X && out, "cdml_knn_index_build: NULL argument");
  CDML_REQUIRE(N > 0 && N < (1ll << 31) && d > 0 && ldx >= d && (metric == 0 || metric == 1),
               "cdml_knn_index_build: bad geometry N=%lld d=%d", (long long)N, d);
  cudaStream_t st = static_cast<cudaStream_t>(stream);
  cdml_index* ix = new cdml_index();
  memset(ix, 0, sizeof(*ix));
  ix->ctx = ctx, ix->N = N, ix->d = d, ix->dpad = (d + 7) / 8 * 8, ix->metric = metric;
  *out = nullptr;
  int rc = 0;
  rc |= dev_alloc(&ix->x32, static_cast<size_t>(N) * d);
  rc |= dev_alloc(&ix->xss, N + 1);
  rc |= dev_alloc(&ix->h, N);
  rc |= dev_alloc(&ix->x16, static_cast<size_t>(N) * ix->dpad);
  if (rc) { index_free(ix); return -2; }
  cudaError_t e = cudaMemcpy2DAsync(ix->x32, sizeof(float) * d, X, sizeof(float) * ldx, sizeof(float) * d, N,
                                    cudaMemcpyDeviceToDevice, st);
  if (e != cudaSuccess) { index_free(ix); set_error("index build copy failed: %s", cudaGetErrorString(e)); return -2; }
  const int grid = static_cast<int>(std::min<int64_t>((N + 7) / 8, ctx->num_sms * 8));
  row_sumsq32_kernel<<<grid, 256, 0, st>>>(ix->x32, N, d, d, ix->xss, metric == 0 ? 0.5f : 0.f, ix->h);
  max_reduce_kernel<<<1, 1024, 0, st>>>(ix->xss, N, ix->xss + N);
  rc = cdml_rows_normalize_cast(ctx, ix->x32, N, d, d, 0, 0.f, ix->x16, ix->dpad, CDML_F16, nullptr, 0, nullptr, stream);
  if (rc) { index_free(ix); return rc; }
  float maxss = 0.f;
  e = cudaMemcpyAsync(&maxss, ix->xss + N, sizeof(float), cudaMemcpyDeviceToHost, st);
  if (e == cudaSuccess) e = cudaStreamSynchronize(st);
  if (e != cudaSuccess) { index_free(ix); set_error("index build failed: %s", cudaGetErrorString(e)); return -2; }
  ix->xmaxnorm = sqrtf(maxss);
  if (N > kCandCap) {
    int64_t ns = std::max<int64_t>(N / 8, 4096);
    ns = std::min<int64_t>(std::min<int64_t>(ns, N), static_cast<int64_t>(kMaxGroups) * 32);
    ns = ns / 32 * 32;
    ix->Ns = ns;
    std::vector<int32_t> rows(ns);
    for (int64_t i = 0; i < ns; ++i) rows[i] = static_cast<int32_t>(i * N / ns);
    int32_t* drows = nullptr;
    rc |= dev_alloc(&drows, ns);
    rc |= dev_alloc(&ix->xs16, static_cast<size_t>(ns) * ix->dpad);
    rc |= dev_alloc(&ix->hs, ns);
    if (rc) { cudaFree(drows); index_free(ix); return -2; }
    cudaMemcpyAsync(drows, rows.data(), sizeof(int32_t) * ns, cudaMemcpyHostToDevice, st);
    rc = cdml_gather_rows(ctx, ix->x16, N, ix->dpad * 2, ix->dpad * 2, drows, 0, ns, ix->xs16, ix->dpad * 2, stream);
    if (!rc) rc = cdml_gather_rows(ctx, ix->h, N, 4, 4, drows, 0, ns, ix->hs, 4, stream);
    cudaStreamSynchronize(st);
    cudaFree(drows);
    if (rc) { index_free(ix); return rc; }
  }
  *out = ix;
  return 0;
}

int cdml_knn_index_destroy(cdml_index* index) {
  index_free(index);
  return 0;
}

int cdml_knn_last_stats(cdml_index* index, int64_t* stats) {
  CDML_REQUIRE(index && stats, "cdml_knn_last_stats: NULL argument");
  stats[0] = index->stats[0], stats[1] = index->stats[1];
  return 0;
}

static int ensure_workspace(cdml_index* ix, int64_t qc) {
  if (ix->qc >= qc) return 0;
  cudaFree(ix->q16), cudaFree(ix->qss), cudaFree(ix->gmax), cudaFree(ix->thr), cudaFree(ix->cand_val);
  cudaFree(ix->cand_idx), cudaFree(ix->cnt), cudaFree(ix->overflow), cudaFree(ix->log), cudaFree(ix->log_count);
  cudaFree(ix->handled);
  ix->handled = nullptr;
  ix->log = nullptr, ix->log_count = nullptr;
  ix->q16 = nullptr, ix->qss = ix->gmax = ix->thr = ix->cand_val = nullptr, ix->cand_idx = ix->cnt = ix->overflow = nullptr;
  ix->qc = 0;
  ix->ldg = ix->Ns > 0 ? ((ix->Ns / 32 + 7) / 8 * 8) : 8;
  int rc = 0;
  rc |= dev_alloc(&ix->q16, static_cast<size_t>(qc) * ix->dpad);
  rc |= dev_alloc(&ix->qss, qc);
  rc |= dev_alloc(&ix->gmax, static_cast<size_t>(qc) * ix->ldg);
  rc |= dev_alloc(&ix->thr, qc);
  rc |= dev_alloc(&ix->cand_val, static_cast<size_t>(qc) * kCandCap);
  rc |= dev_alloc(&ix->cand_idx, static_cast<size_t>(qc) * kCandCap);
  rc |= dev_alloc(&ix->cnt, qc);
  rc |= dev_alloc(&ix->overflow, qc);
  rc |= dev_alloc(&ix->handled, qc);
  const int sms = ix->ctx->num_sms;
  ix->log_cap = static_cast<unsigned int>(std::max<int64_t>(qc * 2048 / (sms * kKnnLogsPerCta), 16384));
  rc |= dev_alloc(&ix->log, static_cast<size_t>(sms) * kKnnLogsPerCta * ix->log_cap);
  rc |= dev_alloc(&ix->log_count, sms * kKnnLogsPerCta + 1);
  if (rc) return -2;
  ix->qc = qc;
  return 0;
}

static int knn_run(cdml_ctx* ctx, cdml_index* ix, const float* Q, int64_t nq, int64_t ldq, int k, float* D, int64_t* I,
                   int64_t id_offset, void* stream, const float* ext_full, const float* ext_part, int k_part,
                   float* out_full, float* out_part, int phase = 0, float part_sign = 1.f, float* nom_pair = nullptr,
                   const float* prune_pair = nullptr, int32_t* defer_flag = nullptr) {
  const bool bounds_only = out_full != nullptr;
  CDML_REQUIRE((phase == 0 && !(bounds_only && part_sign < 0.f)) || nq <= 65536,
               "cdml_knn_shard_*: one chunk of at most 65536 queries per call (got %lld)", (long long)nq);
  CDML_REQUIRE(ctx && ix && Q && (bounds_only || phase == 1 || (D && I)), "cdml_knn_search: NULL argument");
  CDML_REQUIRE(nq >= 0 && ldq >= ix->d && k >= 1 && k <= 1024, "cdml_knn_search: bad arguments (k=%d, supported 1..1024)", k);
  CDML_REQUIRE(k <= kKeepCap / 2, "cdml_knn_search: k=%d exceeds the re-rank capacity %d", k, kKeepCap / 2);
  if (nq == 0) return 0;
  cudaStream_t st = static_cast<cudaStream_t>(stream);
  const int64_t chunk = std::min<int64_t>(nq, (phase != 0 || (bounds_only && part_sign < 0.f)) ? 65536 : 32768);
  int rc = ensure_workspace(ix, chunk);
  if (rc) { set_error("cdml_knn_search: workspace allocation failed"); return rc; }
  if (phase != 2) ix->stats[0] = ix->stats[1] = 0;
  const int d = ix->d;
  const float rel = 1.5f * 0.0009765625f + 1.2e-7f * d;
  const float slack_scale = 2.f * rel * ix->xmaxnorm;
  const float slack_abs = 2.f * 1e-6f * (1.f + ix->xmaxnorm);
  if (ix->h_cap < nq) {
    cudaFreeHost(ix->h_cnt), cudaFreeHost(ix->h_ovf), cudaFreeHost(ix->h_qss), cudaFreeHost(ix->h_logovf);
    ix->h_cnt = ix->h_ovf = ix->h_logovf = nullptr, ix->h_qss = nullptr, ix->h_cap = 0;
    CDML_CHECK_CUDA(cudaMallocHost(reinterpret_cast<void**>(&ix->h_cnt), sizeof(int32_t) * nq));
    CDML_CHECK_CUDA(cudaMallocHost(reinterpret_cast<void**>(&ix->h_ovf), sizeof(int32_t) * nq));
    CDML_CHECK_CUDA(cudaMallocHost(reinterpret_cast<void**>(&ix->h_qss), sizeof(float) * nq));
    CDML_CHECK_CUDA(cudaMallocHost(reinterpret_cast<void**>(&ix->h_logovf), sizeof(int32_t) * (nq / chunk + 2)));
    ix->h_cap = nq;
  }
  for (int64_t q0 = 0; q0 < nq; q0 += chunk) {
    const int64_t qc = std::min<int64_t>(chunk, nq - q0);
    const float* Qc = Q + q0 * ldq;
    const bool tiny = ix->N <= kKeepCap;
    if (phase != 2) {
    rc = cdml_rows_normalize_cast(ctx, Qc, qc, d, ldq, 0, 0.f, ix->q16, ix->dpad, CDML_F16, nullptr, 0, nullptr, stream);
    if (rc) return rc;
    const int grid = static_cast<int>(std::min<int64_t>((qc + 7) / 8, ctx->num_sms * 8));
    row_sumsq32_kernel<<<grid, 256, 0, st>>>(Qc, qc, d, ldq, ix->qss, 0.f, nullptr);
    CDML_CHECK_CUDA(cudaMemsetAsync(ix->cnt, 0, sizeof(int32_t) * qc, st));
    CDML_CHECK_CUDA(cudaMemsetAsync(ix->overflow, 0, sizeof(int32_t) * qc, st));
    CDML_CHECK_CUDA(cudaMemsetAsync(ix->log_count, 0, sizeof(int32_t) * (ctx->num_sms * kKnnLogsPerCta + 1), st));
    if (bounds_only && (tiny || !(ix->Ns > 0 && ix->Ns / 32 >= k))) {
      fill_f32_kernel<<<64, 256, 0, st>>>(out_full + q0, qc, -INFINITY);
      fill_f32_kernel<<<64, 256, 0, st>>>(out_part + q0, qc, -INFINITY * part_sign);
      continue;
    }
    }
    if (!tiny) {
     if (phase != 2) {
      if (ext_full != nullptr) {
        knn_thr_combine_kernel<<<static_cast<int>((qc + 255) / 256), 256, 0, st>>>(ext_full + q0, ext_part + q0, ix->qss, qc,
                                                                                slack_scale, slack_abs, ix->thr, part_sign);
      } else if (ix->Ns > 0 && ix->Ns / 32 >= k) {
        const int wide = (ix->Ns / 128 >= 2 * static_cast<int64_t>(k)) ? 1 : 0;
        const int groups = wide ? static_cast<int>((ix->Ns + 255) / 256 * 2) : static_cast<int>(ix->Ns / 32);
        EpiKnnGroupMax<kBN> ea{ix->hs, ix->gmax, ix->ldg, wide};
        if (resb_applicable(ix->dpad) && qc >= 8 * kBM)
          rc = launch_gemm_resb(ctx, ix->q16, ix->dpad, ix->xs16, ix->dpad, qc, ix->Ns, ix->dpad, CDML_F16, ea, st);
        else
          rc = launch_gemm<0, 0>(ctx, ix->q16, ix->dpad, ix->xs16, ix->dpad, qc, ix->Ns, ix->dpad, CDML_F16, 1, ea, st);
        if (rc < 0) return rc;
        auto kth = [&](int kk, int kk2, float sc, float ab, float* out, float* out2) {
          const int grid = static_cast<int>(qc);
          if (groups <= 1024) {
            const int wgrid = static_cast<int>((qc + 7) / 8);
            if (out2) knn_kth_warp_kernel<true><<<wgrid, 256, 0, st>>>(ix->gmax, ix->ldg, groups, kk, kk2, ix->qss, qc, sc, ab, out, out2, part_sign);
            else knn_kth_warp_kernel<false><<<wgrid, 256, 0, st>>>(ix->gmax, ix->ldg, groups, kk, kk2, ix->qss, qc, sc, ab, out, out2, part_sign);
          } else if (groups <= 4 * kRefineThreads) {
            if (out2) knn_kth_kernel<4, true><<<grid, kRefineThreads, 0, st>>>(ix->gmax, ix->ldg, groups, kk, kk2, ix->qss, sc, ab, out, out2, part_sign);
            else knn_kth_kernel<4, false><<<grid, kRefineThreads, 0, st>>>(ix->gmax, ix->ldg, groups, kk, kk2, ix->qss, sc, ab, out, out2, part_sign);
          } else {
            constexpr int kP = kMaxGroups / kRefineThreads;
            if (out2) knn_kth_kernel<kP, true><<<grid, kRefineThreads, 0, st>>>(ix->gmax, ix->ldg, groups, kk, kk2, ix->qss, sc, ab, out, out2, part_sign);
            else knn_kth_kernel<kP, false><<<grid, kRefineThreads, 0, st>>>(ix->gmax, ix->ldg, groups, kk, kk2, ix->qss, sc, ab, out, out2, part_sign);
          }
        };
        if (bounds_only) {
          kth(k, std::max(1, std::min(k_part, k)), 0.f, 0.f, out_full + q0, out_part + q0);
          CDML_CHECK_CUDA(cudaGetLastError());
          continue;
        }
        kth(k, k, slack_scale, slack_abs, ix->thr, nullptr);
      } else {
        fill_f32_kernel<<<64, 256, 0, st>>>(ix->thr, qc, -INFINITY);
      }
      EpiKnnCollect<kBN> eb{ix->h, ix->thr, ix->log, ix->log_count, ix->log_count + ctx->num_sms * kKnnLogsPerCta, ix->log_cap};
      if (resb_applicable(ix->dpad) && ix->N >= 8 * kBM)
        rc = launch_gemm_resb(ctx, ix->x16, ix->dpad, ix->q16, ix->dpad, ix->N, qc, ix->dpad, CDML_F16, eb, st, 1);
      else
        rc = launch_gemm<0, 0>(ctx, ix->x16, ix->dpad, ix->q16, ix->dpad, ix->N, qc, ix->dpad, CDML_F16, 1, eb, st);
      if (rc < 0) return rc;
      knn_bin_kernel<<<dim3(4, ctx->num_sms * kKnnLogsPerCta), 256, 0, st>>>(ix->log, ix->log_count, ix->log_cap, ix->cand_idx, ix->cand_val,
                                                            ix->cnt, kCandCap);
     }
      if (phase == 1) {
        knn_nominee_kth_kernel<<<static_cast<int>((qc + 7) / 8), 256, 0, st>>>(ix->cand_val, ix->cnt, kCandCap, k,
                                                                              std::max(1, std::min(k_part, k)), qc, nom_pair);
        CDML_CHECK_CUDA(cudaGetLastError());
        continue;
      }
      if (prune_pair != nullptr)
        knn_refine_warp_kernel<<<static_cast<int>((qc + 7) / 8), 256, 0, st>>>(
            Qc, ldq, d, ix->qss, ix->x32, d, ix->xss, ix->cand_idx, ix->cand_val, ix->cnt, kCandCap, k, ix->metric,
            slack_scale, slack_abs, id_offset, D + q0 * k, I + q0 * k, k, prune_pair, qc, qc, ix->handled);
      knn_refine_kernel<<<static_cast<int>(qc), kRefineThreads, 0, st>>>(
          Qc, ldq, d, ix->qss, ix->x32, d, ix->xss, ix->cand_idx, ix->cand_val, ix->cnt, kCandCap, k, ix->metric,
          slack_scale, slack_abs, id_offset, D + q0 * k, I + q0 * k, k, ix->overflow, 0, prune_pair, qc,
          prune_pair != nullptr ? ix->handled : nullptr);
    } else {
      if (phase == 1) {
        fill_f32_kernel<<<64, 256, 0, st>>>(nom_pair, qc, -INFINITY);
        fill_f32_kernel<<<64, 256, 0, st>>>(nom_pair + qc, qc, INFINITY);
        CDML_CHECK_CUDA(cudaGetLastError());
        continue;
      }
      knn_refine_kernel<<<static_cast<int>(qc), kRefineThreads, 0, st>>>(
          Qc, ldq, d, ix->qss, ix->x32, d, ix->xss, ix->cand_idx, ix->cand_val, ix->cnt, kCandCap, k, ix->metric,
          slack_scale, slack_abs, id_offset, D + q0 * k, I + q0 * k, k, ix->overflow, static_cast<int>(ix->N), nullptr, 0, nullptr);
      ix->stats[0] += ix->N * qc;
    }
    CDML_CHECK_CUDA(cudaGetLastError());
    CDML_CHECK_CUDA(cudaMemcpyAsync(ix->h_cnt + q0, ix->cnt, sizeof(int32_t) * qc, cudaMemcpyDeviceToHost, st));
    CDML_CHECK_CUDA(cudaMemcpyAsync(ix->h_ovf + q0, ix->overflow, sizeof(int32_t) * qc, cudaMemcpyDeviceToHost, st));
    CDML_CHECK_CUDA(cudaMemcpyAsync(ix->h_qss + q0, ix->qss, sizeof(float) * qc, cudaMemcpyDeviceToHost, st));
    CDML_CHECK_CUDA(cudaMemcpyAsync(ix->h_logovf + q0 / chunk, ix->log_count + ctx->num_sms * kKnnLogsPerCta, sizeof(int32_t),
                                    cudaMemcpyDeviceToHost, st));
  }
  if (bounds_only || phase == 1) return 0;
  if (defer_flag != nullptr) {
    knn_any_overflow_kernel<<<1, 1024, 0, st>>>(ix->overflow, nq, ix->log_count + ctx->num_sms * kKnnLogsPerCta, defer_flag);
    CDML_CHECK_CUDA(cudaGetLastError());
    return 0;
  }
  CDML_CHECK_CUDA(cudaStreamSynchronize(st));
  std::vector<int32_t> redo;
  for (int64_t i = 0; i < nq; ++i) {
    ix->stats[0] += ix->N <= kKeepCap ? 0 : ix->h_cnt[i];
    if (ix->h_ovf[i] || ix->h_logovf[i / chunk]) redo.push_back(static_cast<int32_t>(i));
  }
  ix->stats[1] = static_cast<int64_t>(redo.size());
  if (!redo.empty()) {
    int kcap = 64;
    while (kcap < k) kcap <<= 1;
    kcap = std::max(kcap, kFbRound);
    const size_t smem = static_cast<size_t>(kFbQueries) * 2 * kcap * sizeof(unsigned long long) + static_cast<size_t>(kFbQueries) * d * sizeof(float);
    CDML_REQUIRE(smem <= 200 * 1024, "cdml_knn_search: exact fallback needs %zu bytes of shared memory (k=%d, d=%d)", smem, k, d);
    CDML_CHECK_CUDA(cudaFuncSetAttribute(knn_exact_batch_kernel, cudaFuncAttributeMaxDynamicSharedMemorySize, static_cast<int>(smem)));
    int32_t* dlist = nullptr;
    if (dev_alloc(&dlist, redo.size())) return -2;
    CDML_CHECK_CUDA(cudaMemcpyAsync(dlist, redo.data(), sizeof(int32_t) * redo.size(), cudaMemcpyHostToDevice, st));
    const int nlist = static_cast<int>(redo.size());
    const int blocks = (nlist + kFbQueries - 1) / kFbQueries;
    int splits = std::max(1, std::min(16, (2 * ctx->num_sms + blocks - 1) / blocks));
    if (ix->N < 64 * 1024) splits = 1;
    float* Dp = nullptr;
    int64_t* Ip = nullptr;
    if (splits > 1 && (dev_alloc(&Dp, static_cast<size_t>(splits + 1) * nlist * k) || dev_alloc(&Ip, static_cast<size_t>(splits + 1) * nlist * k))) {
      cudaFree(dlist), cudaFree(Dp);
      return -2;
    }
    knn_exact_batch_kernel<<<dim3(blocks, splits), kFbThreads, smem, st>>>(dlist, nlist, Q, ldq, d, ix->x32, ix->N, d, ix->xss,
                                                                          ix->metric, k, kcap, id_offset, splits > 1 ? Dp : D,
                                                                          splits > 1 ? Ip : I, splits > 1 ? 1 : 0);
    CDML_CHECK_CUDA(cudaGetLastError());
    if (splits > 1) {
      float* Dm = Dp + static_cast<size_t>(splits) * nlist * k;
      int64_t* Im = Ip + static_cast<size_t>(splits) * nlist * k;
      int rcm = cdml_knn_merge(ctx, Dp, Ip, splits, nlist, k, ix->metric, Dm, Im, stream);
      if (rcm) { cudaFree(dlist), cudaFree(Dp), cudaFree(Ip); return rcm; }
      const int64_t tot = static_cast<int64_t>(nlist) * k;
      knn_scatter_rows_kernel<<<static_cast<int>((tot + 255) / 256), 256, 0, st>>>(dlist, nlist, k, Dm, Im, D, I);
      CDML_CHECK_CUDA(cudaGetLastError());
    }
    CDML_CHECK_CUDA(cudaStreamSynchronize(st));
    cudaFree(dlist), cudaFree(Dp), cudaFree(Ip);
  }
  return 0;
}

int cdml_knn_search(cdml_ctx* ctx, cdml_index* ix, const float* Q, int64_t nq, int64_t ldq, int k, float* D,
                    int64_t* I, int64_t id_offset, void* stream) {
  return knn_run(ctx, ix, Q, nq, ldq, k, D, I, id_offset, stream, nullptr, nullptr, k, nullptr, nullptr);
}

int cdml_knn_bounds(cdml_ctx* ctx, cdml_index* ix, const float* Q, int64_t nq, int64_t ldq, int k_full, int k_part,
                    float* bound_full, float* bound_part, void* stream) {
  CDML_REQUIRE(bound_full && bound_part && k_part >= 1, "cdml_knn_bounds: NULL / bad argument");
  return knn_run(ctx, ix, Q, nq, ldq, k_full, nullptr, nullptr, 0, stream, nullptr, nullptr, k_part, bound_full, bound_part);
}

int cdml_knn_search_bounded(cdml_ctx* ctx, cdml_index* ix, const float* Q, int64_t nq, int64_t ldq, int k,
                            const float* bound_full, const float* bound_part, float* D, int64_t* I, int64_t id_offset,
                            void* stream) {
  CDML_REQUIRE(bound_full && bound_part, "cdml_knn_search_bounded: NULL bounds");
  return knn_run(ctx, ix, Q, nq, ldq, k, D, I, id_offset, stream, bound_full, bound_part, k, nullptr, nullptr);
}

int cdml_knn_shard_bounds(cdml_ctx* ctx, cdml_index* ix, const float* Q, int64_t nq, int64_t ldq, int k, int k_part,
                          float* pair, void* stream) {
  CDML_REQUIRE(pair && k_part >= 1, "cdml_knn_shard_bounds: NULL / bad argument");
  return knn_run(ctx, ix, Q, nq, ldq, k, nullptr, nullptr, 0, stream, nullptr, nullptr, k_part, pair, pair + nq, 0, -1.f);
}

int cdml_knn_shard_collect(cdml_ctx* ctx, cdml_index* ix, const float* Q, int64_t nq, int64_t ldq, int k, int k_part,
                           const float* pair, float* nom_pair, void* stream) {
  CDML_REQUIRE(pair && nom_pair && k_part >= 1, "cdml_knn_shard_collect: NULL / bad argument");
  return knn_run(ctx, ix, Q, nq, ldq, k, nullptr, nullptr, 0, stream, pair, pair + nq, k_part, nullptr, nullptr, 1, -1.f,
                 nom_pair);
}

int cdml_knn_shard_refine(cdml_ctx* ctx, cdml_index* ix, const float* Q, int64_t nq, int64_t ldq, int k,
                          const float* nom_pair, unsigned long long* rec, int64_t id_offset, int32_t* overflow_flag,
                          void* stream) {
  CDML_REQUIRE(ix && rec, "cdml_knn_shard_refine: NULL argument");
  CDML_REQUIRE(id_offset >= 0 && id_offset + ix->N <= (1ll << 32) - 1, "cdml_knn_shard_refine: global ids must fit 32 bits");
  if (ix->tmp_cap < nq * k) {
    cudaFree(ix->Dtmp), cudaFree(ix->Itmp);
    ix->Dtmp = nullptr, ix->Itmp = nullptr, ix->tmp_cap = 0;
    if (dev_alloc(&ix->Dtmp, static_cast<size_t>(nq) * k) || dev_alloc(&ix->Itmp, static_cast<size_t>(nq) * k)) return -2;
    ix->tmp_cap = nq * k;
  }
  int rc = knn_run(ctx, ix, Q, nq, ldq, k, ix->Dtmp, ix->Itmp, id_offset, stream, nullptr, nullptr, k, nullptr, nullptr, 2, -1.f,
                   nullptr, nom_pair, overflow_flag);
  if (rc) return rc;
  const int64_t n = nq * k;
  knn_pack_kernel<<<static_cast<unsigned>((n + 255) / 256), 256, 0, static_cast<cudaStream_t>(stream)>>>(ix->Dtmp, ix->Itmp, n, ix->metric, rec);
  CDML_CHECK_CUDA(cudaGetLastError());
  return 0;
}

int cdml_knn_unpack_records(cdml_ctx* ctx, const unsigned long long* rec, int64_t n, int metric, float* D, int64_t* I,
                            void* stream) {
  CDML_REQUIRE(ctx && rec && D && I && n >= 0, "cdml_knn_unpack_records: bad argument");
  if (n == 0) return 0;
  knn_unpack_kernel<<<static_cast<unsigned>((n + 255) / 256), 256, 0, static_cast<cudaStream_t>(stream)>>>(rec, n, metric, D, I);
  CDML_CHECK_CUDA(cudaGetLastError());
  return 0;
}

int cdml_knn_merge_packed(cdml_ctx* ctx, const unsigned long long* rec, int G, int64_t nq, int k, int metric, float* D,
                          int64_t* I, unsigned long long* rec_out, void* stream) {
  CDML_REQUIRE(ctx && rec && ((D && I) || rec_out) && G >= 1 && G <= 32 && k >= 1 && nq >= 0,
               "cdml_knn_merge_packed: bad argument (1 <= G <= 32)");
  if (nq == 0) return 0;
  const size_t per = static_cast<size_t>(G) * k * sizeof(unsigned long long);
  CDML_REQUIRE(per <= 200 * 1024, "cdml_knn_merge_packed: G*k=%d too large for one warp's staging", G * k);
  const int warps = static_cast<int>(std::max<size_t>(1, std::min<size_t>(8, (96 * 1024) / per)));
  const size_t smem = per * warps;
  if (smem > 48 * 1024)
    CDML_CHECK_CUDA(cudaFuncSetAttribute(knn_merge_packed_kernel, cudaFuncAttributeMaxDynamicSharedMemorySize, static_cast<int>(smem)));
  knn_merge_packed_kernel<<<static_cast<unsigned>((nq + warps - 1) / warps), 256, smem, static_cast<cudaStream_t>(stream)>>>(
      rec, G, nq, k, metric, warps, D, I, rec_out);
  CDML_CHECK_CUDA(cudaGetLastError());
  return 0;
}

int cdml_knn_merge(cdml_ctx* ctx, const float* Dg, const int64_t* Ig, int G, int64_t nq, int k, int metric, float* D,
                   int64_t* I, void* stream) {
  CDML_REQUIRE(ctx && Dg && Ig && D && I && G >= 1 && k >= 1 && nq >= 0, "cdml_knn_merge: bad argument");
  if (nq == 0) return 0;
  int P = 2;
  while (P < G * k) P <<= 1;
  const size_t smem = static_cast<size_t>(P) * (sizeof(unsigned long long) + sizeof(int));
  CDML_REQUIRE(smem <= 200 * 1024, "cdml_knn_merge: G*k=%d too large for one block", G * k);
  if (smem > 48 * 1024)
    CDML_CHECK_CUDA(cudaFuncSetAttribute(knn_merge_kernel, cudaFuncAttributeMaxDynamicSharedMemorySize, static_cast<int>(smem)));
  knn_merge_kernel<<<static_cast<unsigned>(nq), 256, smem, static_cast<cudaStream_t>(stream)>>>(Dg, Ig, G, nq, k, metric, D, I);
  CDML_CHECK_CUDA(cudaGetLastError());
  return 0;
}

}
```

collaborative-deep-metric-learning_b200/csrc/mine.cu:

```cuda
#include <algorithm>

#include "gemm_launch.cuh"

namespace cdml {

constexpr unsigned long long kNoCand = ~0ull;
constexpr int kMassHits = 4;

static int epi_warps() {
  static int w = -1;
  if (w < 0) {
    const char* e = getenv("CDML_MINE_EPI_WARPS");
    w = (e != nullptr && e[0] == '1') ? 16 : 8;
  }
  return w;
}

template <int BN, int kVariant = 0>
struct EpiMine {
  static constexpr bool kSplitColumns = true;
  static constexpr bool kPrefetchNext = (kVariant & 1) == 0;
  static constexpr bool kRowConsts = (kVariant & 4) != 0;
  struct State {
    float dpi, bound_d;
    int ga, gp;
    uint32_t bound_row;
    uint32_t release_bar;
  };
  static constexpr bool kEarlyRelease = true;
  static constexpr bool kTmaStore = false;
  const float* dp;
  const int32_t* guid;
  unsigned long long* best;
  int cand;
  unsigned long long* stats;
  __device__ __forceinline__ void row_consts(int row, const GemmShape& s, uint32_t dst) const {
    const bool row_ok = row < s.M;
    const uint32_t inf = 0x7f800000u;
    const uint32_t dpi = row_ok ? __float_as_uint(__ldg(dp + row)) : inf;
    const uint32_t ga = row_ok ? static_cast<uint32_t>(__ldg(guid + 3 * row)) : 0u;
    const uint32_t gp = row_ok ? static_cast<uint32_t>(__ldg(guid + 3 * row + 1)) : 0u;
    const unsigned long long key = row_ok ? *(reinterpret_cast<volatile unsigned long long*>(best) + row) : ~0ull;
    sts128(dst, dpi, ga, gp, static_cast<uint32_t>(key >> 32));
    asm volatile("st.shared.b32 [%0], %1;" ::"r"(dst + 16), "r"(static_cast<uint32_t>(key)) : "memory");
  }
  __device__ __forceinline__ void load_state(State& st, uint32_t src) const {
    const uint4 v = lds128(src);
    st.dpi = __uint_as_float(v.x), st.ga = static_cast<int>(v.y), st.gp = static_cast<int>(v.z), st.bound_d = __uint_as_float(v.w);
    asm volatile("ld.shared.b32 %0, [%1];" : "=r"(st.bound_row) : "r"(src + 16) : "memory");
    st.release_bar = 0u;
  }
  __device__ __forceinline__ void pre(State& st, int row, int , const GemmShape& s, int, int, uint32_t) const {
    const bool row_ok = row < s.M;
    const float inf = __int_as_float(0x7f800000);
    st.dpi = row_ok ? __ldg(dp + row) : inf;
    st.ga = row_ok ? __ldg(guid + 3 * row) : 0;
    st.gp = row_ok ? __ldg(guid + 3 * row + 1) : 0;
    const unsigned long long key = row_ok ? best[row] : ~0ull;
    st.bound_d = __uint_as_float(static_cast<uint32_t>(key >> 32));
    st.bound_row = static_cast<uint32_t>(key);
    st.release_bar = 0u;
  }
  __device__ __forceinline__ void cols(int n0, const GemmShape& s, int c0, int , uint32_t stg) const {
    static_assert(BN == 256, "a warp owns 4 chunks (128 columns) of the tile");
    col_cache_fill(stg, n0, c0, [&](int col) { return static_cast<uint32_t>(col < s.N ? __ldg(guid + 3 * col + cand) : -1); });
  }
  __device__ __forceinline__ void block_begin(uint32_t epi_smem) const { col_cache_reset(epi_smem); }
  __device__ __forceinline__ void block_end(uint32_t) const {}
  __device__ __forceinline__ void run(uint32_t taddr, int row, int n0, int , const GemmShape& s, int c0,
                                      int c1, uint32_t stg, State& st) const {
    const int lane = threadIdx.x & 31;
    const bool row_ok = row < s.M;
    const float inf = __int_as_float(0x7f800000);
    const float dpi = st.dpi;
    const float s_hi = row_ok ? 1.f - 0.5f * dpi : -inf;
    const int ga = st.ga, gp = st.gp;
    float bound_d = st.bound_d;
    if (!(bound_d == bound_d)) bound_d = inf;
    float s_lo = 1.f - 0.5f * bound_d;
    uint32_t brow = st.bound_row;
    float bd = inf;
    int br = -1;
    uint32_t va[32], vb[32];
    auto chunk = [&](const uint32_t (&v)[32], int cc) {
      const int nb = n0 + (c0 + cc) * 32;
      uint32_t u0 = 0xffffffffu, u1 = 0xffffffffu;
#pragma unroll
      for (int j = 0; j < 8; ++j) {
        const float2 lo = sub2(s_hi, s_hi, __uint_as_float(v[4 * j]), __uint_as_float(v[4 * j + 1]));
        const float2 hi = sub2(s_hi, s_hi, __uint_as_float(v[4 * j + 2]), __uint_as_float(v[4 * j + 3]));
        u0 = umin3(u0, __float_as_uint(lo.x), __float_as_uint(lo.y));
        u1 = umin3(u1, __float_as_uint(hi.x), __float_as_uint(hi.y));
      }
      const uint32_t mu = min(u0, u1), thr = __float_as_uint(s_hi - s_lo);
      unsigned int hits = __ballot_sync(0xffffffffu, mu < thr || (mu == thr && static_cast<uint32_t>(3 * nb + cand) < brow));
      if (hits != 0u && __popc(hits) >= kMassHits) {
        if (lane == 0) atomicAdd(stats, static_cast<unsigned long long>(__popc(hits)));
        if ((hits >> lane) & 1u) {
          uint32_t kbest = 0xffffffffu;
          int cbest = -1;
#pragma unroll
          for (int j = 0; j < 32; ++j) {
            int g;
            asm volatile("ld.shared.b32 %0, [%1];" : "=r"(g) : "r"(stg + kColCacheOff + 128 * cc + 4 * j) : "memory");
            const float sc = __uint_as_float(v[j]);
            const float d = fmaxf(fmaf(-2.f, sc, 2.f), 0.f);
            const bool pass = sc < s_hi && sc >= s_lo && d > dpi && d < bd && g != ga && g != gp && g >= 0;
            if (pass && __float_as_uint(d) < kbest) kbest = __float_as_uint(d), cbest = j;
          }
          if (cbest >= 0) {
            bd = __uint_as_float(kbest), br = 3 * (nb + cbest) + cand;
            const float s_new = 1.f - 0.5f * bd;
            if (s_new > s_lo || (s_new == s_lo && static_cast<uint32_t>(br) < brow)) brow = static_cast<uint32_t>(br);
            s_lo = fmaxf(s_lo, s_new);
          }
        }
        __syncwarp();
      } else if (hits != 0u) {
        if (lane == 0) atomicAdd(stats, static_cast<unsigned long long>(__popc(hits)));
        int g_lane;
        asm volatile("ld.shared.b32 %0, [%1];" : "=r"(g_lane) : "r"(stg + kColCacheOff + 128 * cc + 4 * lane) : "memory");
        do {
          const int src = __ffs(hits) - 1;
          hits &= hits - 1u;
          __syncwarp();
          if (lane == src) {
#pragma unroll
            for (int j = 0; j < 8; ++j) sts128(stg + 16 * j, v[4 * j], v[4 * j + 1], v[4 * j + 2], v[4 * j + 3]);
          }
          __syncwarp();
          float sc;
          asm volatile("ld.shared.f32 %0, [%1];" : "=f"(sc) : "r"(stg + 4 * lane) : "memory");
          const float hi_s = __shfl_sync(0xffffffffu, s_hi, src), lo_s = __shfl_sync(0xffffffffu, s_lo, src);
          const float dp_s = __shfl_sync(0xffffffffu, dpi, src), bd_s = __shfl_sync(0xffffffffu, bd, src);
          const int ga_s = __shfl_sync(0xffffffffu, ga, src), gp_s = __shfl_sync(0xffffffffu, gp, src);
          const float d = fmaxf(fmaf(-2.f, sc, 2.f), 0.f);
          const bool pass = sc < hi_s && sc >= lo_s && d > dp_s && d < bd_s && g_lane != ga_s && g_lane != gp_s && g_lane >= 0;
          const uint32_t kmin = __reduce_min_sync(0xffffffffu, pass ? __float_as_uint(d) : 0xffffffffu);
          if (kmin != 0xffffffffu) {
            const int col = __ffs(__ballot_sync(0xffffffffu, pass && __float_as_uint(d) == kmin)) - 1;
            if (lane == src) {
              bd = __uint_as_float(kmin), br = 3 * (nb + col) + cand;
              const float s_new = 1.f - 0.5f * bd;
              if (s_new > s_lo || (s_new == s_lo && static_cast<uint32_t>(br) < brow)) brow = static_cast<uint32_t>(br);
              s_lo = fmaxf(s_lo, s_new);
            }
          }
        } while (hits != 0u);
      }
    };
    auto ok = [&](int cc) { return c0 + cc < c1 && n0 + (c0 + cc) * 32 < s.N; };
    if constexpr ((kVariant & 2) == 0) {
      tmem_ld_32x32(taddr + c0 * 32, va);
#pragma unroll
      for (int cc = 0; cc < 4; cc += 2) {
        tmem_ld_wait();
        if (ok(cc + 1)) tmem_ld_32x32(taddr + (c0 + cc + 1) * 32, vb);
        if (ok(cc)) chunk(va, cc);
        tmem_ld_wait();
        if (cc + 2 < 4 && ok(cc + 2)) tmem_ld_32x32(taddr + (c0 + cc + 2) * 32, va);
        if (cc + 2 >= 4 && st.release_bar != 0u) {
          tc_fence_before();
          __syncwarp();
          if (lane == 0) mbar_arrive(st.release_bar);
        }
        if (ok(cc + 1)) chunk(vb, cc + 1);
      }
    } else {
#pragma unroll
      for (int cc = 0; cc < 4; ++cc) {
        if (ok(cc)) {
          tmem_ld_32x32(taddr + (c0 + cc) * 32, va);
          tmem_ld_wait();
          chunk(va, cc);
        }
      }
      if (st.release_bar != 0u) {
        tc_fence_before();
        __syncwarp();
        if (lane == 0) mbar_arrive(st.release_bar);
      }
    }
    if (br >= 0)
      atomicMin(best + row, (static_cast<unsigned long long>(__float_as_uint(bd)) << 32) | static_cast<uint32_t>(br));
  }
};

__global__ void mine_prepare_kernel(const float* __restrict__ E, int64_t ld, int D, const int64_t* __restrict__ guid64,
                                    int64_t B, float* __restrict__ dp, int32_t* __restrict__ guid32,
                                    unsigned long long* __restrict__ best, unsigned long long* __restrict__ stats) {
  const int warp = threadIdx.x >> 5, lane = threadIdx.x & 31;
  if (blockIdx.x == 0 && threadIdx.x < 2) stats[threadIdx.x] = 0ull;
  for (int64_t i = static_cast<int64_t>(blockIdx.x) * 8 + warp; i < B; i += static_cast<int64_t>(gridDim.x) * 8) {
    const float* a = E + 3 * i * ld;
    const float* p = a + ld;
    float s = 0.f;
    for (int j = lane; j < D; j += 32) {
      const float t = a[j] - p[j];
      s = fmaf(t, t, s);
    }
#pragma unroll
    for (int o = 16; o > 0; o >>= 1) s += __shfl_xor_sync(0xffffffffu, s, o);
    if (lane == 0) dp[i] = s, best[i] = kNoCand;
    if (lane < 3) guid32[3 * i + lane] = static_cast<int32_t>(guid64[3 * i + lane]);
  }
}

__global__ void mine_finalize_kernel(const float* __restrict__ E, int64_t ld, int D,
                                     const unsigned long long* __restrict__ best, int64_t B,
                                     int32_t* __restrict__ neg_row, float* __restrict__ d_an,
                                     unsigned long long* __restrict__ stats) {
  const int warp = threadIdx.x >> 5, lane = threadIdx.x & 31;
  unsigned int mined = 0;
  for (int64_t i = static_cast<int64_t>(blockIdx.x) * 8 + warp; i < B; i += static_cast<int64_t>(gridDim.x) * 8) {
    const unsigned long long kb = best[i];
    const int r = kb != kNoCand ? static_cast<int>(static_cast<uint32_t>(kb)) : static_cast<int>(3 * i + 2);
    mined += kb != kNoCand ? 1u : 0u;
    if (lane == 0) neg_row[i] = r;
    if (d_an != nullptr) {
      const float* a = E + 3 * i * ld;
      const float* n = E + static_cast<int64_t>(r) * ld;
      float s = 0.f;
      for (int j = lane; j < D; j += 32) {
        const float t = a[j] - n[j];
        s = fmaf(t, t, s);
      }
#pragma unroll
      for (int o = 16; o > 0; o >>= 1) s += __shfl_xor_sync(0xffffffffu, s, o);
      if (lane == 0) d_an[i] = s;
    }
  }
  if (lane == 0 && mined != 0u) atomicAdd(stats + 1, static_cast<unsigned long long>(mined));
}

}

using namespace cdml;

extern "C" int cdml_mine_semihard(cdml_ctx* ctx, const void* E16, int64_t ld16, int dtype16, const float* E32,
                                  int64_t ld32, const int64_t* guid, int64_t B, int D, float margin, int32_t* neg_row,
                                  float* d_an, void* stream) {
  CDML_REQUIRE(ctx && E16 && E32 && guid && neg_row, "cdml_mine_semihard: NULL argument");
  CDML_REQUIRE(B > 0 && 3 * B < (1ll << 31) && D > 0 && D % 8 == 0 && ld16 >= D && ld32 >= D,
               "cdml_mine_semihard: bad geometry B=%lld D=%d", (long long)B, D);
  cudaStream_t st = static_cast<cudaStream_t>(stream);
  const size_t bytes = static_cast<size_t>(B) * (8 + 4 + 12) + 64;
  uint8_t* ws = static_cast<uint8_t*>(ctx_scratch(ctx, bytes));
  if (ws == nullptr) return -2;
  if (ctx->mine_stats == nullptr) CDML_CHECK_CUDA(cudaMalloc(&ctx->mine_stats, 2 * sizeof(unsigned long long)));
  unsigned long long* stats = ctx->mine_stats;
  unsigned long long* best = reinterpret_cast<unsigned long long*>(ws);
  float* dp = reinterpret_cast<float*>(best + B);
  int32_t* guid32 = reinterpret_cast<int32_t*>(dp + B);
  const int grid = static_cast<int>(std::min<int64_t>((B + 7) / 8, ctx->num_sms * 8));
  mine_prepare_kernel<<<grid, 256, 0, st>>>(E32, ld32, D, guid, B, dp, guid32, best, stats);
  int rc = 0;
  const uint16_t* e16 = static_cast<const uint16_t*>(E16);
  for (int cand = 1; cand <= 2 && rc >= 0; ++cand) {
    EpiMine<kBN, 1> epi{dp, guid32, best, cand, stats};
    static int rowc = -1;
    if (rowc < 0) rowc = getenv("CDML_MINE_ROWCONSTS") != nullptr ? 1 : 0;
    if (resb_applicable(D) && B >= 8 * kBM && rowc) {
      EpiMine<kBN, 5> epi5{dp, guid32, best, cand, stats};
      rc = launch_gemm_resb(ctx, e16, 3 * ld16, e16 + cand * ld16, 3 * ld16, B, B, D, dtype16, epi5, st);
    } else if (resb_applicable(D) && B >= 8 * kBM && epi_warps() == 16)
      rc = launch_gemm_resb<EpiMine<kBN, 1>, 16>(ctx, e16, 3 * ld16, e16 + cand * ld16, 3 * ld16, B, B, D, dtype16, epi, st);
    else if (resb_applicable(D) && B >= 8 * kBM)
      rc = launch_gemm_resb(ctx, e16, 3 * ld16, e16 + cand * ld16, 3 * ld16, B, B, D, dtype16, epi, st);
    else
      rc = launch_gemm<0, 0>(ctx, e16, 3 * ld16, e16 + cand * ld16, 3 * ld16, B, B, D, dtype16, 1, epi, st);
  }
  if (rc >= 0) {
    mine_finalize_kernel<<<grid, 256, 0, st>>>(E32, ld32, D, best, B, neg_row, d_an, stats);
    rc = cudaGetLastError() == cudaSuccess ? 0 : -2;
  }
  return rc < 0 ? rc : 0;
}

extern "C" int cdml_mine_last_stats(cdml_ctx* ctx, int64_t* out2, void* stream) {
  CDML_REQUIRE(ctx && out2, "cdml_mine_last_stats: NULL argument");
  out2[0] = out2[1] = 0;
  if (ctx->mine_stats == nullptr) return 0;
  cudaStream_t st = static_cast<cudaStream_t>(stream);
  unsigned long long h[2];
  CDML_CHECK_CUDA(cudaMemcpyAsync(h, ctx->mine_stats, sizeof(h), cudaMemcpyDeviceToHost, st));
  CDML_CHECK_CUDA(cudaStreamSynchronize(st));
  out2[0] = static_cast<int64_t>(h[0]), out2[1] = static_cast<int64_t>(h[1]);
  return 0;
}
```

Measured before the change: 5.911 million.

## Fuse both semihard candidate scans into one 2-CTA resident-anchor mining kernel

The two per-candidate GEMM+epilogue launches are replaced by one dedicated 2-CTA cluster kernel. It keeps the anchor panel resident and streams positives and negatives together through an interleaved 3D tensor map, with a compact candidate-guid array prepared up front. The goal is to halve the launches and anchor reloads and to use the 256-row cta_group::2 MMA. It also removes the experimental row-constant and 16-warp epilogue options from the generic resident-B kernel. The cost is a new specialised kernel with its own pipeline, and a new restriction to D <= 256 with 16-byte-aligned ld16.

```diff
diff --git a/collaborative-deep-metric-learning_b200/csrc/gemm_launch.cuh b/collaborative-deep-metric-learning_b200/csrc/gemm_launch.cuh
--- a/collaborative-deep-metric-learning_b200/csrc/gemm_launch.cuh
+++ b/collaborative-deep-metric-learning_b200/csrc/gemm_launch.cuh
@@ -149,10 +149,10 @@
   return off == 0 && K <= 4 * kBK;
 }
 
-template <class Epi, int kEpiWarps = 8>
+template <class Epi>
 static int launch_gemm_resb(cdml_ctx* ctx, const void* A, int64_t lda, const void* B, int64_t ldb, int64_t M, int64_t N,
                             int64_t K, int dtype16, const Epi& epi, cudaStream_t stream, int n_fastest = 0) {
-  using L = ResBSmem<kBN, kResBStages, kEpiWarps, Epi::kRowConsts, Epi::kTmaStore ? 2 : 1>;
+  using L = ResBSmem<kBN, kResBStages, Epi::kTmaStore ? 2 : 1>;
   static_assert(L::kTotal <= 232448, "resident-B kernel: shared memory over the 227 KB limit");
   CUtensorMap ta, tb;
   int rc = make_tmap_2d(ctx, &ta, A, dtype16, K, M, lda, kBK, kBM);
@@ -181,7 +181,7 @@
   s.tiles_per_chunk = (s.m_tiles + best - 1) / best;
   s.n_fastest = n_fastest;
   s.idesc = make_idesc_f16(dtype16 == CDML_BF16 ? 1 : 0, 0, 0, kBM, kBN);
-  auto kern = gemm_resb_tcgen05_kernel<kBN, kResBStages, Epi, kEpiWarps>;
+  auto kern = gemm_resb_tcgen05_kernel<kBN, kResBStages, Epi>;
   static bool attr_set = false;
   if (!attr_set) {
     CDML_CHECK_CUDA(cudaFuncSetAttribute(kern, cudaFuncAttributeMaxDynamicSharedMemorySize, L::kTotal));
@@ -189,7 +189,7 @@
   }
   const long units = static_cast<long>(s.n_tiles) * s.m_chunks;
   const int grid = static_cast<int>(units < ctx->num_sms ? units : ctx->num_sms);
-  kern<<<grid, 128 + 32 * kEpiWarps, L::kTotal, stream>>>(ta, tb, s, epi);
+  kern<<<grid, kGemmThreads, L::kTotal, stream>>>(ta, tb, s, epi);
   CDML_CHECK_CUDA(cudaGetLastError());
   if (trace_sync(Epi::kTmaStore ? "gemm_resb[tma]" : "gemm_resb", M, N, K, grid, stream)) return -2;
   return 1;
diff --git a/collaborative-deep-metric-learning_b200/csrc/gemm_sm100.cuh b/collaborative-deep-metric-learning_b200/csrc/gemm_sm100.cuh
--- a/collaborative-deep-metric-learning_b200/csrc/gemm_sm100.cuh
+++ b/collaborative-deep-metric-learning_b200/csrc/gemm_sm100.cuh
@@ -123,7 +123,6 @@
   struct State {};
   __device__ __forceinline__ void pre(State&, int, int, const GemmShape&, int, int, uint32_t) const {}
   static constexpr bool kPrefetchNext = false;
-  static constexpr bool kRowConsts = false;
   static constexpr bool kEarlyRelease = false;
   static constexpr bool kTmaStore = false;
   __device__ __forceinline__ void cols(int, const GemmShape&, int, int, uint32_t) const {}
@@ -170,7 +169,6 @@
   struct State {};
   __device__ __forceinline__ void pre(State&, int, int, const GemmShape&, int, int, uint32_t) const {}
   static constexpr bool kPrefetchNext = false;
-  static constexpr bool kRowConsts = false;
   static constexpr bool kEarlyRelease = false;
   static constexpr bool kTmaStore = false;
   __device__ __forceinline__ void cols(int, const GemmShape&, int, int, uint32_t) const {}
@@ -213,7 +211,6 @@
   struct State {};
   __device__ __forceinline__ void pre(State&, int, int, const GemmShape&, int, int, uint32_t) const {}
   static constexpr bool kPrefetchNext = false;
-  static constexpr bool kRowConsts = false;
   static constexpr bool kEarlyRelease = false;
   static constexpr bool kTmaStore = false;
   __device__ __forceinline__ void cols(int, const GemmShape&, int, int, uint32_t) const {}
@@ -275,7 +272,6 @@
     uint4 raw[4][4];
   };
   static constexpr bool kPrefetchNext = false;
-  static constexpr bool kRowConsts = false;
   static constexpr bool kEarlyRelease = false;
   static constexpr bool kTmaStore = false;
   __device__ __forceinline__ void cols(int, const GemmShape&, int, int, uint32_t) const {}
@@ -364,7 +360,6 @@
     uint32_t bits[4];
   };
   static constexpr bool kPrefetchNext = true;
-  static constexpr bool kRowConsts = false;
   static constexpr bool kEarlyRelease = false;
   static constexpr bool kTmaStore = false;
   __device__ __forceinline__ void cols(int, const GemmShape&, int, int, uint32_t) const {}
@@ -420,7 +415,6 @@
     uint32_t release_bar;
   };
   static constexpr bool kPrefetchNext = true;
-  static constexpr bool kRowConsts = false;
   static constexpr bool kEarlyRelease = true;
   static constexpr bool kTmaStore = true;
   __device__ __forceinline__ void cols(int, const GemmShape&, int, int, uint32_t) const {}
@@ -495,7 +489,6 @@
   struct State {};
   __device__ __forceinline__ void pre(State&, int, int, const GemmShape&, int, int, uint32_t) const {}
   static constexpr bool kPrefetchNext = false;
-  static constexpr bool kRowConsts = false;
   static constexpr bool kEarlyRelease = false;
   static constexpr bool kTmaStore = false;
   __device__ __forceinline__ void cols(int, const GemmShape&, int, int, uint32_t) const {}
@@ -675,27 +668,23 @@
   uint32_t idesc;
 };
 
-template <int BN, int kAStages, int kEpiWarps = 8, bool kRowSlots = false, int kStageSlices = 1>
+template <int BN, int kAStages, int kStageSlices = 1>
 struct ResBSmem {
   static constexpr uint32_t kABytes = kBM * kBK * 2;
   static constexpr uint32_t kBPanel = BN * kBK * 2;
   static constexpr uint32_t kMaxKb = 4;
   static constexpr uint32_t kEpiOff = kMaxKb * kBPanel + kAStages * kABytes;
-  static constexpr uint32_t kEpiBytes = kEpiWarps * 2048 * kStageSlices;
-  static constexpr uint32_t kRowConstOff = kEpiOff + kEpiBytes;
-  static constexpr uint32_t kRowConstSlot = kRowSlots ? kBM * 32 : 0;
-  static constexpr uint32_t kBarOff = kRowConstOff + 2 * kRowConstSlot;
-  static constexpr uint32_t kNumBars = 2 * kAStages + 2 + 4 + 2;
+  static constexpr uint32_t kEpiBytes = 8 * 2048 * kStageSlices;
+  static constexpr uint32_t kBarOff = kEpiOff + kEpiBytes;
+  static constexpr uint32_t kNumBars = 2 * kAStages + 2 + 4;
   static constexpr uint32_t kTotal = kBarOff + kNumBars * 8 + 16 + 1024;
 };
 
-template <int BN, int kAStages, class Epi, int kEpiWarps = 8>
-__global__ void __launch_bounds__(128 + 32 * kEpiWarps, 1)
+template <int BN, int kAStages, class Epi>
+__global__ void __launch_bounds__(kGemmThreads, 1)
 gemm_resb_tcgen05_kernel(const __grid_constant__ CUtensorMap tma_a, const __grid_constant__ CUtensorMap tma_b,
                          const ResBShape s, const __grid_constant__ Epi epi) {
-  using L = ResBSmem<BN, kAStages, kEpiWarps, Epi::kRowConsts, Epi::kTmaStore ? 2 : 1>;
-  static_assert(kEpiWarps == 8 || kEpiWarps == 16, "two or four epilogue warps per TMEM lane quarter");
-  static_assert(kEpiWarps == 8 || Epi::kSplitColumns, "four warps per quarter split the tile's columns");
+  using L = ResBSmem<BN, kAStages, Epi::kTmaStore ? 2 : 1>;
   extern __shared__ uint8_t smem_raw[];
   const uint32_t raw_u32 = smem_u32(smem_raw);
   const uint32_t base = (raw_u32 + 1023u) & ~1023u;
@@ -708,8 +697,6 @@
   const uint32_t b_empty = bar0 + 8u * (2 * kAStages + 1);
   auto tfull_bar = [&](int i) { return bar0 + 8u * (2 * kAStages + 2 + i); };
   auto tempty_bar = [&](int i) { return bar0 + 8u * (2 * kAStages + 4 + i); };
-  auto cfull_bar = [&](int i) { return bar0 + 8u * (2 * kAStages + 6 + i); };
-  auto cslot = [&](int i) { return base + L::kRowConstOff + i * L::kRowConstSlot; };
   const uint32_t tmem_slot = bar0 + 8u * L::kNumBars;
   volatile uint32_t* tmem_slot_ptr = reinterpret_cast<volatile uint32_t*>(smem_raw + (tmem_slot - raw_u32));
   const int warp = threadIdx.x >> 5;
@@ -730,8 +717,7 @@
     mbar_init(b_empty, 1);
     for (int i = 0; i < 2; ++i) {
       mbar_init(tfull_bar(i), 1);
-      mbar_init(tempty_bar(i), kEpiWarps);
-      mbar_init(cfull_bar(i), 1);
+      mbar_init(tempty_bar(i), 8);
     }
     fence_mbar_init();
   }
@@ -798,29 +784,10 @@
       }
       tc_commit(b_empty);
     }
-  } else if (warp == 3) {
-   if constexpr (Epi::kRowConsts) {
-    int it = 0;
-    GemmShape gs;
-    gs.M = s.M, gs.N = s.N, gs.K = s.K;
-    for (int u = blockIdx.x; u < units; u += gridDim.x) {
-      const int chunk = s.n_fastest ? u / s.n_tiles : u % s.m_chunks;
-      const int t0 = chunk * s.tiles_per_chunk, t1 = min(s.m_tiles, t0 + s.tiles_per_chunk);
-      for (int t = t0; t < t1; ++t, ++it) {
-        const int as = it & 1;
-        const uint32_t ap = (it >> 1) & 1;
-        mbar_wait(tempty_bar(as), ap ^ 1, 700 + as);
-#pragma unroll
-        for (int r = lane; r < kBM; r += 32) epi.row_consts(t * kBM + r, gs, cslot(as) + r * 32);
-        __syncwarp();
-        if (lane == 0) mbar_arrive(cfull_bar(as));
-      }
-    }
-   }
   } else if (warp >= 4) {
     const int q = warp & 3;
     const int half = (warp - 4) >> 2;
-    const uint32_t stg = base + L::kEpiOff + (warp - 4) * (Epi::kTmaStore ? 4096u : (Epi::kSplitColumns || kEpiWarps == 16) ? 2048u : 4096u);
+    const uint32_t stg = base + L::kEpiOff + (warp - 4) * (Epi::kTmaStore ? 4096u : Epi::kSplitColumns ? 2048u : 4096u);
     int it = 0;
     GemmShape gs;
     gs.M = s.M, gs.N = s.N, gs.K = s.K, gs.m_tiles = s.m_tiles, gs.n_tiles = s.n_tiles, gs.num_kb = s.num_kb;
@@ -841,15 +808,14 @@
       }
     };
     const bool active = Epi::kSplitColumns || half == 0;
-    constexpr int kChunksPerWarp = (BN / 32) / (kEpiWarps / 4);
-    const int ec0 = Epi::kSplitColumns ? half * kChunksPerWarp : 0, ec1 = Epi::kSplitColumns ? (half + 1) * kChunksPerWarp : BN / 32;
+    const int ec0 = Epi::kSplitColumns ? half * (BN / 64) : 0, ec1 = Epi::kSplitColumns ? (half + 1) * (BN / 64) : BN / 32;
     TileIter cur;
     cur.u = blockIdx.x;
     seek(cur);
     typename Epi::State est;
     if (cur.valid && active) {
       epi.cols(cur.nblk * BN, gs, ec0, ec1, stg);
-      if constexpr (!Epi::kRowConsts) epi.pre(est, cur.t * kBM + q * 32 + lane, cur.nblk * BN, gs, ec0, ec1, stg);
+      epi.pre(est, cur.t * kBM + q * 32 + lane, cur.nblk * BN, gs, ec0, ec1, stg);
     }
     while (cur.valid) {
       TileIter nxt = cur;
@@ -860,17 +826,11 @@
       const int as = it & 1;
       const uint32_t ap = (it >> 1) & 1;
       typename Epi::State est_next;
-      if constexpr (Epi::kRowConsts) {
-        mbar_wait(cfull_bar(as), ap, 800 + as);
-        if (active) epi.load_state(est, cslot(as) + (q * 32 + lane) * 32);
-        est_next = est;
-      }
       mbar_wait(tfull_bar(as), ap, 400 + as);
       tc_fence_after();
       const uint32_t taddr = tmem_base + (static_cast<uint32_t>(q * 32) << 16) + as * BN;
       if (active) {
-        if constexpr (!Epi::kRowConsts)
-          if (Epi::kPrefetchNext && nxt.valid) epi.pre(est_next, nxt.t * kBM + q * 32 + lane, nxt.nblk * BN, gs, ec0, ec1, stg);
+        if (Epi::kPrefetchNext && nxt.valid) epi.pre(est_next, nxt.t * kBM + q * 32 + lane, nxt.nblk * BN, gs, ec0, ec1, stg);
         if constexpr (Epi::kEarlyRelease) est.release_bar = tempty_bar(as);
         epi.run(taddr, cur.t * kBM + q * 32 + lane, cur.nblk * BN, 0, gs, ec0, ec1, stg, est);
       }
@@ -881,8 +841,7 @@
       }
       if (active && nxt.valid) {
         epi.cols(nxt.nblk * BN, gs, ec0, ec1, stg);
-        if constexpr (!Epi::kRowConsts)
-          if (!Epi::kPrefetchNext) epi.pre(est_next, nxt.t * kBM + q * 32 + lane, nxt.nblk * BN, gs, ec0, ec1, stg);
+        if (!Epi::kPrefetchNext) epi.pre(est_next, nxt.t * kBM + q * 32 + lane, nxt.nblk * BN, gs, ec0, ec1, stg);
       }
       est = est_next;
       cur = nxt;
diff --git a/collaborative-deep-metric-learning_b200/csrc/knn.cu b/collaborative-deep-metric-learning_b200/csrc/knn.cu
--- a/collaborative-deep-metric-learning_b200/csrc/knn.cu
+++ b/collaborative-deep-metric-learning_b200/csrc/knn.cu
@@ -38,7 +38,6 @@
 struct EpiKnnGroupMax {
   static constexpr bool kSplitColumns = true;
   static constexpr bool kPrefetchNext = false;
-  static constexpr bool kRowConsts = false;
   static constexpr bool kEarlyRelease = false;
   static constexpr bool kTmaStore = false;
   struct State {};
@@ -106,7 +105,6 @@
     uint32_t release_bar;
   };
   static constexpr bool kPrefetchNext = true;
-  static constexpr bool kRowConsts = false;
   static constexpr bool kEarlyRelease = true;
   static constexpr bool kTmaStore = false;
   __device__ __forceinline__ void block_begin(uint32_t epi_smem) const {
diff --git a/collaborative-deep-metric-learning_b200/csrc/mine.cu b/collaborative-deep-metric-learning_b200/csrc/mine.cu
--- a/collaborative-deep-metric-learning_b200/csrc/mine.cu
+++ b/collaborative-deep-metric-learning_b200/csrc/mine.cu
@@ -6,191 +6,314 @@
 
 constexpr unsigned long long kNoCand = ~0ull;
 constexpr int kMassHits = 4;
-
-static int epi_warps() {
-  static int w = -1;
-  if (w < 0) {
-    const char* e = getenv("CDML_MINE_EPI_WARPS");
-    w = (e != nullptr && e[0] == '1') ? 16 : 8;
-  }
-  return w;
-}
-
-template <int BN, int kVariant = 0>
-struct EpiMine {
-  static constexpr bool kSplitColumns = true;
-  static constexpr bool kPrefetchNext = (kVariant & 1) == 0;
-  static constexpr bool kRowConsts = (kVariant & 4) != 0;
-  struct State {
-    float dpi, bound_d;
-    int ga, gp;
-    uint32_t bound_row;
-    uint32_t release_bar;
-  };
-  static constexpr bool kEarlyRelease = true;
-  static constexpr bool kTmaStore = false;
+constexpr int kMineTile = 256;
+constexpr int kMineStages = 8;
+
+struct MineSmem {
+  static constexpr uint32_t kAPanel = kBM * kBK * 2;
+  static constexpr uint32_t kBBytes = (kMineTile / 2) * kBK * 2;
+  static constexpr uint32_t kBOff = 4 * kAPanel;
+  static constexpr uint32_t kEpiOff = kBOff + kMineStages * kBBytes;
+  static constexpr uint32_t kBarOff = kEpiOff + 8 * kWarpSliceBytes;
+  static constexpr uint32_t kNumBars = 2 * kMineStages + 2 + 4;
+  static constexpr uint32_t kTotal = kBarOff + kNumBars * 8 + 16 + 1024;
+};
+static_assert(MineSmem::kTotal <= 232448, "mining scan: shared memory over the 227 KB limit");
+
+struct MineShape {
+  int B, num_kb;
+  int n_ab;
+  int n_ct;
+  int ranges;
+  int tpr;
+  uint32_t idesc;
+};
+
+struct MineArgs {
   const float* dp;
   const int32_t* guid;
+  const int32_t* guidc;
   unsigned long long* best;
-  int cand;
   unsigned long long* stats;
-  __device__ __forceinline__ void row_consts(int row, const GemmShape& s, uint32_t dst) const {
-    const bool row_ok = row < s.M;
-    const uint32_t inf = 0x7f800000u;
-    const uint32_t dpi = row_ok ? __float_as_uint(__ldg(dp + row)) : inf;
-    const uint32_t ga = row_ok ? static_cast<uint32_t>(__ldg(guid + 3 * row)) : 0u;
-    const uint32_t gp = row_ok ? static_cast<uint32_t>(__ldg(guid + 3 * row + 1)) : 0u;
-    const unsigned long long key = row_ok ? *(reinterpret_cast<volatile unsigned long long*>(best) + row) : ~0ull;
-    sts128(dst, dpi, ga, gp, static_cast<uint32_t>(key >> 32));
-    asm volatile("st.shared.b32 [%0], %1;" ::"r"(dst + 16), "r"(static_cast<uint32_t>(key)) : "memory");
-  }
-  __device__ __forceinline__ void load_state(State& st, uint32_t src) const {
-    const uint4 v = lds128(src);
-    st.dpi = __uint_as_float(v.x), st.ga = static_cast<int>(v.y), st.gp = static_cast<int>(v.z), st.bound_d = __uint_as_float(v.w);
-    asm volatile("ld.shared.b32 %0, [%1];" : "=r"(st.bound_row) : "r"(src + 16) : "memory");
-    st.release_bar = 0u;
-  }
-  __device__ __forceinline__ void pre(State& st, int row, int , const GemmShape& s, int, int, uint32_t) const {
-    const bool row_ok = row < s.M;
-    const float inf = __int_as_float(0x7f800000);
-    st.dpi = row_ok ? __ldg(dp + row) : inf;
-    st.ga = row_ok ? __ldg(guid + 3 * row) : 0;
-    st.gp = row_ok ? __ldg(guid + 3 * row + 1) : 0;
-    const unsigned long long key = row_ok ? best[row] : ~0ull;
-    st.bound_d = __uint_as_float(static_cast<uint32_t>(key >> 32));
-    st.bound_row = static_cast<uint32_t>(key);
-    st.release_bar = 0u;
-  }
-  __device__ __forceinline__ void cols(int n0, const GemmShape& s, int c0, int , uint32_t stg) const {
-    static_assert(BN == 256, "a warp owns 4 chunks (128 columns) of the tile");
-    col_cache_fill(stg, n0, c0, [&](int col) { return static_cast<uint32_t>(col < s.N ? __ldg(guid + 3 * col + cand) : -1); });
-  }
-  __device__ __forceinline__ void block_begin(uint32_t epi_smem) const { col_cache_reset(epi_smem); }
-  __device__ __forceinline__ void block_end(uint32_t) const {}
-  __device__ __forceinline__ void run(uint32_t taddr, int row, int n0, int , const GemmShape& s, int c0,
-                                      int c1, uint32_t stg, State& st) const {
-    const int lane = threadIdx.x & 31;
-    const bool row_ok = row < s.M;
-    const float inf = __int_as_float(0x7f800000);
-    const float dpi = st.dpi;
-    const float s_hi = row_ok ? 1.f - 0.5f * dpi : -inf;
-    const int ga = st.ga, gp = st.gp;
-    float bound_d = st.bound_d;
-    if (!(bound_d == bound_d)) bound_d = inf;
-    float s_lo = 1.f - 0.5f * bound_d;
-    uint32_t brow = st.bound_row;
-    float bd = inf;
-    int br = -1;
-    uint32_t va[32], vb[32];
-    auto chunk = [&](const uint32_t (&v)[32], int cc) {
-      const int nb = n0 + (c0 + cc) * 32;
-      uint32_t u0 = 0xffffffffu, u1 = 0xffffffffu;
-#pragma unroll
-      for (int j = 0; j < 8; ++j) {
-        const float2 lo = sub2(s_hi, s_hi, __uint_as_float(v[4 * j]), __uint_as_float(v[4 * j + 1]));
-        const float2 hi = sub2(s_hi, s_hi, __uint_as_float(v[4 * j + 2]), __uint_as_float(v[4 * j + 3]));
-        u0 = umin3(u0, __float_as_uint(lo.x), __float_as_uint(lo.y));
-        u1 = umin3(u1, __float_as_uint(hi.x), __float_as_uint(hi.y));
+};
+
+__device__ __forceinline__ uint32_t cand_row(int c) { return 3u * static_cast<uint32_t>(c >> 1) + 1u + static_cast<uint32_t>(c & 1); }
+
+__device__ __forceinline__ void tma_load_3d_pair(uint32_t dst, const CUtensorMap* m, uint32_t bar, int c0, int c1, int c2) {
+  asm volatile(
+      "cp.async.bulk.tensor.3d.cta_group::2.shared::cluster.global.mbarrier::complete_tx::bytes [%0], [%1, {%3, %4, %5}], [%2];"
+      ::"r"(dst), "l"(reinterpret_cast<uint64_t>(m)), "r"(bar & kPeerBitMask), "r"(c0), "r"(c1), "r"(c2)
+      : "memory");
+}
+
+__device__ __forceinline__ void mine_unit(const MineShape& s, int u, int& ab, int& t0, int& t1) {
+  ab = u % s.n_ab;
+  t0 = (u / s.n_ab) * s.tpr;
+  t1 = min(s.n_ct, t0 + s.tpr);
+}
+
+__global__ void __launch_bounds__(kGemmThreads, 1)
+mine_pair_kernel(const __grid_constant__ CUtensorMap tma_a, const __grid_constant__ CUtensorMap tma_b, const MineShape s,
+                 const MineArgs args) {
+  using L = MineSmem;
+  extern __shared__ uint8_t smem_raw[];
+  const uint32_t raw_u32 = smem_u32(smem_raw);
+  const uint32_t base = (raw_u32 + 1023u) & ~1023u;
+  const uint32_t bar0 = base + L::kBarOff;
+  auto a_panel = [&](int kb) { return base + kb * L::kAPanel; };
+  auto b_smem = [&](int st) { return base + L::kBOff + st * L::kBBytes; };
+  auto full_bar = [&](int st) { return bar0 + 8u * st; };
+  auto empty_bar = [&](int st) { return bar0 + 8u * (kMineStages + st); };
+  const uint32_t a_full = bar0 + 8u * (2 * kMineStages);
+  const uint32_t a_empty = bar0 + 8u * (2 * kMineStages + 1);
+  auto tfull_bar = [&](int i) { return bar0 + 8u * (2 * kMineStages + 2 + i); };
+  auto tempty_bar = [&](int i) { return bar0 + 8u * (2 * kMineStages + 4 + i); };
+  const uint32_t tmem_slot = bar0 + 8u * L::kNumBars;
+  volatile uint32_t* tmem_slot_ptr = reinterpret_cast<volatile uint32_t*>(smem_raw + (tmem_slot - raw_u32));
+
+  const int warp = threadIdx.x >> 5;
+  const int lane = threadIdx.x & 31;
+  const uint32_t rank = cluster_ctarank();
+  const bool leader = rank == 0;
+  const int cluster_id = blockIdx.x >> 1;
+  const int num_clusters = gridDim.x >> 1;
+  constexpr uint32_t kTmemCols = 512;
+  const int units = s.n_ab * s.ranges;
+
+  cluster_sync_all();
+  if (warp == 0 && lane == 0) {
+    tma_prefetch_desc(&tma_a);
+    tma_prefetch_desc(&tma_b);
+  }
+  if (warp == 1 && lane == 0) {
+    for (int i = 0; i < kMineStages; ++i) {
+      mbar_init(full_bar(i), 2);
+      mbar_init(empty_bar(i), 1);
+    }
+    mbar_init(a_full, 2);
+    mbar_init(a_empty, 1);
+    for (int i = 0; i < 2; ++i) {
+      mbar_init(tfull_bar(i), 1);
+      mbar_init(tempty_bar(i), 16);
+    }
+    fence_mbar_init();
+  }
+  if (warp == 2) {
+    tmem_alloc2(tmem_slot, kTmemCols);
+    tmem_relinquish2();
+  }
+  tc_fence_before();
+  cluster_sync_all();
+  tc_fence_after();
+  const uint32_t tmem_base = *tmem_slot_ptr;
+
+  if (warp == 0 && lane == 0) {
+    int stage = 0;
+    uint32_t phase = 0, aphase = 0;
+    for (int u = cluster_id; u < units; u += num_clusters) {
+      int ab, t0, t1;
+      mine_unit(s, u, ab, t0, t1);
+      if (t0 >= t1) continue;
+      mbar_wait(a_empty, aphase ^ 1, 500);
+      for (int kb = 0; kb < s.num_kb; ++kb)
+        tma_load_2d_pair(a_panel(kb), &tma_a, a_full, kb * kBK, ab * (2 * kBM) + static_cast<int>(rank) * kBM);
+      if (leader) mbar_arrive_expect_tx(a_full, 2 * s.num_kb * L::kAPanel);
+      else mbar_arrive_cluster(a_full & kPeerBitMask);
+      aphase ^= 1;
+      for (int t = t0; t < t1; ++t) {
+        const int j0 = t * (kMineTile / 2) + static_cast<int>(rank) * (kMineTile / 4);
+        for (int kb = 0; kb < s.num_kb; ++kb) {
+          mbar_wait(empty_bar(stage), phase ^ 1, 100 + stage);
+          tma_load_3d_pair(b_smem(stage), &tma_b, full_bar(stage), kb * kBK, 0, j0);
+          if (leader) mbar_arrive_expect_tx(full_bar(stage), 2 * L::kBBytes);
+          else mbar_arrive_cluster(full_bar(stage) & kPeerBitMask);
+          if (++stage == kMineStages) stage = 0, phase ^= 1;
+        }
       }
-      const uint32_t mu = min(u0, u1), thr = __float_as_uint(s_hi - s_lo);
-      unsigned int hits = __ballot_sync(0xffffffffu, mu < thr || (mu == thr && static_cast<uint32_t>(3 * nb + cand) < brow));
-      if (hits != 0u && __popc(hits) >= kMassHits) {
-        if (lane == 0) atomicAdd(stats, static_cast<unsigned long long>(__popc(hits)));
-        if ((hits >> lane) & 1u) {
-          uint32_t kbest = 0xffffffffu;
-          int cbest = -1;
-#pragma unroll
-          for (int j = 0; j < 32; ++j) {
-            int g;
-            asm volatile("ld.shared.b32 %0, [%1];" : "=r"(g) : "r"(stg + kColCacheOff + 128 * cc + 4 * j) : "memory");
-            const float sc = __uint_as_float(v[j]);
-            const float d = fmaxf(fmaf(-2.f, sc, 2.f), 0.f);
-            const bool pass = sc < s_hi && sc >= s_lo && d > dpi && d < bd && g != ga && g != gp && g >= 0;
-            if (pass && __float_as_uint(d) < kbest) kbest = __float_as_uint(d), cbest = j;
-          }
-          if (cbest >= 0) {
-            bd = __uint_as_float(kbest), br = 3 * (nb + cbest) + cand;
-            const float s_new = 1.f - 0.5f * bd;
-            if (s_new > s_lo || (s_new == s_lo && static_cast<uint32_t>(br) < brow)) brow = static_cast<uint32_t>(br);
-            s_lo = fmaxf(s_lo, s_new);
+    }
+  } else if (warp == 1 && lane == 0) {
+    if (leader) {
+      int stage = 0, it = 0;
+      uint32_t phase = 0, aphase = 0;
+      for (int u = cluster_id; u < units; u += num_clusters) {
+        int ab, t0, t1;
+        mine_unit(s, u, ab, t0, t1);
+        if (t0 >= t1) continue;
+        mbar_wait(a_full, aphase, 600);
+        aphase ^= 1;
+        tc_fence_after();
+        for (int t = t0; t < t1; ++t, ++it) {
+          const int as = it & 1;
+          const uint32_t ap = (it >> 1) & 1;
+          mbar_wait(tempty_bar(as), ap ^ 1, 200 + as);
+          tc_fence_after();
+          const uint32_t tmem_d = tmem_base + as * kMineTile;
+          for (int kb = 0; kb < s.num_kb; ++kb) {
+            mbar_wait(full_bar(stage), phase, 300 + stage);
+            tc_fence_after();
+#pragma unroll
+            for (int k = 0; k < kBK / kUK; ++k) {
+              const uint64_t ad = make_smem_desc(a_panel(kb) + k * (kUK * 2), 16, 1024);
+              const uint64_t bd = make_smem_desc(b_smem(stage) + k * (kUK * 2), 16, 1024);
+              umma2_f16(tmem_d, ad, bd, s.idesc, (kb > 0 || k > 0) ? 1u : 0u);
+            }
+            tc_commit2(empty_bar(stage));
+            if (kb == s.num_kb - 1) tc_commit2(tfull_bar(as));
+            if (++stage == kMineStages) stage = 0, phase ^= 1;
           }
         }
+        tc_commit2(a_empty);
+      }
+    }
+  } else if (warp >= 4) {
+    const int q = warp & 3;
+    const int half = (warp - 4) >> 2;
+    const uint32_t stg = base + L::kEpiOff + (warp - 4) * kWarpSliceBytes;
+    const int nc = 2 * s.B;
+    const float inf = __int_as_float(0x7f800000);
+    int it = 0;
+    for (int u = cluster_id; u < units; u += num_clusters) {
+      int ab, t0, t1;
+      mine_unit(s, u, ab, t0, t1);
+      if (t0 >= t1) continue;
+      const int row = ab * (2 * kBM) + static_cast<int>(rank) * kBM + q * 32 + lane;
+      const bool row_ok = row < s.B;
+      const float dpi = row_ok ? __ldg(args.dp + row) : inf;
+      const int ga = row_ok ? __ldg(args.guid + 3 * row) : 0;
+      const int gp = row_ok ? __ldg(args.guid + 3 * row + 1) : 0;
+      const unsigned long long key = row_ok ? *(reinterpret_cast<volatile unsigned long long*>(args.best) + row) : ~0ull;
+      const float s_hi = row_ok ? 1.f - 0.5f * dpi : -inf;
+      float bound_d = __uint_as_float(static_cast<uint32_t>(key >> 32));
+      if (!(bound_d == bound_d)) bound_d = inf;
+      float s_lo = 1.f - 0.5f * bound_d;
+      uint32_t brow = static_cast<uint32_t>(key);
+      float bd = inf;
+      int br = -1;
+      uint32_t gnext[4];
+#pragma unroll
+      for (int i = 0; i < 4; ++i) gnext[i] = static_cast<uint32_t>(__ldg(args.guidc + t0 * kMineTile + half * 128 + 32 * i + lane));
+      for (int t = t0; t < t1; ++t, ++it) {
+        const int nb0 = t * kMineTile + half * 128;
         __syncwarp();
-      } else if (hits != 0u) {
-        if (lane == 0) atomicAdd(stats, static_cast<unsigned long long>(__popc(hits)));
-        int g_lane;
-        asm volatile("ld.shared.b32 %0, [%1];" : "=r"(g_lane) : "r"(stg + kColCacheOff + 128 * cc + 4 * lane) : "memory");
-        do {
-          const int src = __ffs(hits) - 1;
-          hits &= hits - 1u;
-          __syncwarp();
-          if (lane == src) {
-#pragma unroll
-            for (int j = 0; j < 8; ++j) sts128(stg + 16 * j, v[4 * j], v[4 * j + 1], v[4 * j + 2], v[4 * j + 3]);
+#pragma unroll
+        for (int i = 0; i < 4; ++i)
+          asm volatile("st.shared.b32 [%0], %1;" ::"r"(stg + kColCacheOff + 4 * (32 * i + lane)), "r"(gnext[i]) : "memory");
+        __syncwarp();
+        if (t + 1 < t1) {
+#pragma unroll
+          for (int i = 0; i < 4; ++i) gnext[i] = static_cast<uint32_t>(__ldg(args.guidc + nb0 + kMineTile + 32 * i + lane));
+        }
+        const int as = it & 1;
+        const uint32_t ap = (it >> 1) & 1;
+        mbar_wait(tfull_bar(as), ap, 400 + as);
+        tc_fence_after();
+        const uint32_t taddr = tmem_base + (static_cast<uint32_t>(q * 32) << 16) + as * kMineTile + half * 128;
+        uint32_t va[32], vb[32];
+        auto chunk = [&](const uint32_t (&v)[32], int cc) {
+          const int nb = nb0 + cc * 32;
+          uint32_t u0 = 0xffffffffu, u1 = 0xffffffffu;
+#pragma unroll
+          for (int j = 0; j < 8; ++j) {
+            const float2 lo = sub2(s_hi, s_hi, __uint_as_float(v[4 * j]), __uint_as_float(v[4 * j + 1]));
+            const float2 hi = sub2(s_hi, s_hi, __uint_as_float(v[4 * j + 2]), __uint_as_float(v[4 * j + 3]));
+            u0 = umin3(u0, __float_as_uint(lo.x), __float_as_uint(lo.y));
+            u1 = umin3(u1, __float_as_uint(hi.x), __float_as_uint(hi.y));
           }
-          __syncwarp();
-          float sc;
-          asm volatile("ld.shared.f32 %0, [%1];" : "=f"(sc) : "r"(stg + 4 * lane) : "memory");
-          const float hi_s = __shfl_sync(0xffffffffu, s_hi, src), lo_s = __shfl_sync(0xffffffffu, s_lo, src);
-          const float dp_s = __shfl_sync(0xffffffffu, dpi, src), bd_s = __shfl_sync(0xffffffffu, bd, src);
-          const int ga_s = __shfl_sync(0xffffffffu, ga, src), gp_s = __shfl_sync(0xffffffffu, gp, src);
-          const float d = fmaxf(fmaf(-2.f, sc, 2.f), 0.f);
-          const bool pass = sc < hi_s && sc >= lo_s && d > dp_s && d < bd_s && g_lane != ga_s && g_lane != gp_s && g_lane >= 0;
-          const uint32_t kmin = __reduce_min_sync(0xffffffffu, pass ? __float_as_uint(d) : 0xffffffffu);
-          if (kmin != 0xffffffffu) {
-            const int col = __ffs(__ballot_sync(0xffffffffu, pass && __float_as_uint(d) == kmin)) - 1;
-            if (lane == src) {
-              bd = __uint_as_float(kmin), br = 3 * (nb + col) + cand;
-              const float s_new = 1.f - 0.5f * bd;
-              if (s_new > s_lo || (s_new == s_lo && static_cast<uint32_t>(br) < brow)) brow = static_cast<uint32_t>(br);
-              s_lo = fmaxf(s_lo, s_new);
+          const uint32_t mu = min(u0, u1), thr = __float_as_uint(s_hi - s_lo);
+          unsigned int hits = __ballot_sync(0xffffffffu, mu < thr || (mu == thr && cand_row(nb) < brow));
+          if (hits != 0u && __popc(hits) >= kMassHits) {
+            if (lane == 0) atomicAdd(args.stats, static_cast<unsigned long long>(__popc(hits)));
+            if ((hits >> lane) & 1u) {
+              uint32_t kbest = 0xffffffffu;
+              int cbest = -1;
+#pragma unroll
+              for (int j = 0; j < 32; ++j) {
+                int g;
+                asm volatile("ld.shared.b32 %0, [%1];" : "=r"(g) : "r"(stg + kColCacheOff + 128 * cc + 4 * j) : "memory");
+                const float sc = __uint_as_float(v[j]);
+                const float d = fmaxf(fmaf(-2.f, sc, 2.f), 0.f);
+                const bool pass = sc < s_hi && sc >= s_lo && d > dpi && d < bd && g != ga && g != gp && g >= 0;
+                if (pass && __float_as_uint(d) < kbest) kbest = __float_as_uint(d), cbest = j;
+              }
+              if (cbest >= 0) {
+                bd = __uint_as_float(kbest), br = static_cast<int>(cand_row(nb + cbest));
+                const float s_new = 1.f - 0.5f * bd;
+                if (s_new > s_lo || (s_new == s_lo && static_cast<uint32_t>(br) < brow)) brow = static_cast<uint32_t>(br);
+                s_lo = fmaxf(s_lo, s_new);
+              }
             }
+            __syncwarp();
+          } else if (hits != 0u) {
+            if (lane == 0) atomicAdd(args.stats, static_cast<unsigned long long>(__popc(hits)));
+            int g_lane;
+            asm volatile("ld.shared.b32 %0, [%1];" : "=r"(g_lane) : "r"(stg + kColCacheOff + 128 * cc + 4 * lane) : "memory");
+            do {
+              const int src = __ffs(hits) - 1;
+              hits &= hits - 1u;
+              __syncwarp();
+              if (lane == src) {
+#pragma unroll
+                for (int j = 0; j < 8; ++j) sts128(stg + 16 * j, v[4 * j], v[4 * j + 1], v[4 * j + 2], v[4 * j + 3]);
+              }
+              __syncwarp();
+              float sc;
+              asm volatile("ld.shared.f32 %0, [%1];" : "=f"(sc) : "r"(stg + 4 * lane) : "memory");
+              const float hi_s = __shfl_sync(0xffffffffu, s_hi, src), lo_s = __shfl_sync(0xffffffffu, s_lo, src);
+              const float dp_s = __shfl_sync(0xffffffffu, dpi, src), bd_s = __shfl_sync(0xffffffffu, bd, src);
+              const int ga_s = __shfl_sync(0xffffffffu, ga, src), gp_s = __shfl_sync(0xffffffffu, gp, src);
+              const float d = fmaxf(fmaf(-2.f, sc, 2.f), 0.f);
+              const bool pass = sc < hi_s && sc >= lo_s && d > dp_s && d < bd_s && g_lane != ga_s && g_lane != gp_s && g_lane >= 0;
+              const uint32_t kmin = __reduce_min_sync(0xffffffffu, pass ? __float_as_uint(d) : 0xffffffffu);
+              if (kmin != 0xffffffffu) {
+                const int col = __ffs(__ballot_sync(0xffffffffu, pass && __float_as_uint(d) == kmin)) - 1;
+                if (lane == src) {
+                  bd = __uint_as_float(kmin), br = static_cast<int>(cand_row(nb + col));
+                  const float s_new = 1.f - 0.5f * bd;
+                  if (s_new > s_lo || (s_new == s_lo && static_cast<uint32_t>(br) < brow)) brow = static_cast<uint32_t>(br);
+                  s_lo = fmaxf(s_lo, s_new);
+                }
+              }
+            } while (hits != 0u);
           }
-        } while (hits != 0u);
-      }
-    };
-    auto ok = [&](int cc) { return c0 + cc < c1 && n0 + (c0 + cc) * 32 < s.N; };
-    if constexpr ((kVariant & 2) == 0) {
-      tmem_ld_32x32(taddr + c0 * 32, va);
-#pragma unroll
-      for (int cc = 0; cc < 4; cc += 2) {
-        tmem_ld_wait();
-        if (ok(cc + 1)) tmem_ld_32x32(taddr + (c0 + cc + 1) * 32, vb);
-        if (ok(cc)) chunk(va, cc);
-        tmem_ld_wait();
-        if (cc + 2 < 4 && ok(cc + 2)) tmem_ld_32x32(taddr + (c0 + cc + 2) * 32, va);
-        if (cc + 2 >= 4 && st.release_bar != 0u) {
-          tc_fence_before();
-          __syncwarp();
-          if (lane == 0) mbar_arrive(st.release_bar);
-        }
-        if (ok(cc + 1)) chunk(vb, cc + 1);
-      }
-    } else {
-#pragma unroll
-      for (int cc = 0; cc < 4; ++cc) {
-        if (ok(cc)) {
-          tmem_ld_32x32(taddr + (c0 + cc) * 32, va);
+        };
+        auto ok = [&](int cc) { return nb0 + cc * 32 < nc; };
+        tmem_ld_32x32(taddr, va);
+#pragma unroll
+        for (int cc = 0; cc < 4; cc += 2) {
           tmem_ld_wait();
-          chunk(va, cc);
+          if (ok(cc + 1)) tmem_ld_32x32(taddr + (cc + 1) * 32, vb);
+          if (ok(cc)) chunk(va, cc);
+          tmem_ld_wait();
+          if (cc + 2 < 4 && ok(cc + 2)) tmem_ld_32x32(taddr + (cc + 2) * 32, va);
+          if (cc + 2 >= 4) {
+            tc_fence_before();
+            __syncwarp();
+            if (lane == 0) mbar_arrive_cluster(tempty_bar(as) & kPeerBitMask);
+          }
+          if (ok(cc + 1)) chunk(vb, cc + 1);
         }
       }
-      if (st.release_bar != 0u) {
-        tc_fence_before();
-        __syncwarp();
-        if (lane == 0) mbar_arrive(st.release_bar);
-      }
-    }
-    if (br >= 0)
-      atomicMin(best + row, (static_cast<unsigned long long>(__float_as_uint(bd)) << 32) | static_cast<uint32_t>(br));
-  }
-};
+      if (br >= 0)
+        atomicMin(args.best + row, (static_cast<unsigned long long>(__float_as_uint(bd)) << 32) | static_cast<uint32_t>(br));
+    }
+  }
+
+  tc_fence_before();
+  cluster_sync_all();
+  if (warp == 2) {
+    tc_fence_after();
+    tmem_dealloc2(tmem_base, kTmemCols);
+  }
+}
 
 __global__ void mine_prepare_kernel(const float* __restrict__ E, int64_t ld, int D, const int64_t* __restrict__ guid64,
                                     int64_t B, float* __restrict__ dp, int32_t* __restrict__ guid32,
-                                    unsigned long long* __restrict__ best, unsigned long long* __restrict__ stats) {
+                                    int32_t* __restrict__ guidc, int64_t nc_pad, unsigned long long* __restrict__ best,
+                                    unsigned long long* __restrict__ stats) {
   const int warp = threadIdx.x >> 5, lane = threadIdx.x & 31;
   if (blockIdx.x == 0 && threadIdx.x < 2) stats[threadIdx.x] = 0ull;
+  if (blockIdx.x == 0)
+    for (int64_t c = 2 * B + threadIdx.x; c < nc_pad; c += blockDim.x) guidc[c] = -1;
   for (int64_t i = static_cast<int64_t>(blockIdx.x) * 8 + warp; i < B; i += static_cast<int64_t>(gridDim.x) * 8) {
     const float* a = E + 3 * i * ld;
     const float* p = a + ld;
@@ -203,6 +326,7 @@
     for (int o = 16; o > 0; o >>= 1) s += __shfl_xor_sync(0xffffffffu, s, o);
     if (lane == 0) dp[i] = s, best[i] = kNoCand;
     if (lane < 3) guid32[3 * i + lane] = static_cast<int32_t>(guid64[3 * i + lane]);
+    if (lane >= 1 && lane < 3) guidc[2 * i + lane - 1] = static_cast<int32_t>(guid64[3 * i + lane]);
   }
 }
 
@@ -241,10 +365,32 @@
                                   int64_t ld32, const int64_t* guid, int64_t B, int D, float margin, int32_t* neg_row,
                                   float* d_an, void* stream) {
   CDML_REQUIRE(ctx && E16 && E32 && guid && neg_row, "cdml_mine_semihard: NULL argument");
-  CDML_REQUIRE(B > 0 && 3 * B < (1ll << 31) && D > 0 && D % 8 == 0 && ld16 >= D && ld32 >= D,
-               "cdml_mine_semihard: bad geometry B=%lld D=%d", (long long)B, D);
+  CDML_REQUIRE(B > 0 && 3 * B < (1ll << 31) && D > 0 && D <= 4 * kBK && D % 8 == 0 && ld16 >= D && ld16 % 8 == 0 &&
+                   ld32 >= D,
+               "cdml_mine_semihard: bad geometry B=%lld D=%d ld16=%lld (D <= 256, ld16 %% 8 == 0)", (long long)B, D,
+               (long long)ld16);
   cudaStream_t st = static_cast<cudaStream_t>(stream);
-  const size_t bytes = static_cast<size_t>(B) * (8 + 4 + 12) + 64;
+  MineShape s;
+  s.B = static_cast<int>(B);
+  s.num_kb = (D + kBK - 1) / kBK;
+  s.n_ab = static_cast<int>((B + 2 * kBM - 1) / (2 * kBM));
+  s.n_ct = static_cast<int>((2 * B + kMineTile - 1) / kMineTile);
+  s.idesc = make_idesc_f16(dtype16 == CDML_BF16 ? 1 : 0, 0, 0, 2 * kBM, kMineTile);
+  const int pairs = ctx->num_sms / 2;
+  int ranges = 1;
+  double best_eff = -1.0;
+  for (int r = 1; r <= std::max(1, s.n_ct / 8); ++r) {
+    const int tpr = (s.n_ct + r - 1) / r;
+    if ((s.n_ct + tpr - 1) / tpr != r) continue;
+    const long units = static_cast<long>(s.n_ab) * r;
+    const long waves = (units + pairs - 1) / pairs;
+    const double eff = static_cast<double>(units) / static_cast<double>(waves * pairs) - 1.0 / tpr;
+    if (eff > best_eff) best_eff = eff, ranges = r;
+  }
+  s.ranges = ranges;
+  s.tpr = (s.n_ct + ranges - 1) / ranges;
+  const int64_t nc_pad = static_cast<int64_t>(s.n_ct) * kMineTile;
+  const size_t bytes = static_cast<size_t>(B) * (8 + 4 + 12) + static_cast<size_t>(nc_pad) * 4 + 64;
   uint8_t* ws = static_cast<uint8_t*>(ctx_scratch(ctx, bytes));
   if (ws == nullptr) return -2;
   if (ctx->mine_stats == nullptr) CDML_CHECK_CUDA(cudaMalloc(&ctx->mine_stats, 2 * sizeof(unsigned long long)));
@@ -252,24 +398,45 @@
   unsigned long long* best = reinterpret_cast<unsigned long long*>(ws);
   float* dp = reinterpret_cast<float*>(best + B);
   int32_t* guid32 = reinterpret_cast<int32_t*>(dp + B);
+  int32_t* guidc = guid32 + 3 * B;
   const int grid = static_cast<int>(std::min<int64_t>((B + 7) / 8, ctx->num_sms * 8));
-  mine_prepare_kernel<<<grid, 256, 0, st>>>(E32, ld32, D, guid, B, dp, guid32, best, stats);
-  int rc = 0;
+  mine_prepare_kernel<<<grid, 256, 0, st>>>(E32, ld32, D, guid, B, dp, guid32, guidc, nc_pad, best, stats);
+
   const uint16_t* e16 = static_cast<const uint16_t*>(E16);
-  for (int cand = 1; cand <= 2 && rc >= 0; ++cand) {
-    EpiMine<kBN, 1> epi{dp, guid32, best, cand, stats};
-    static int rowc = -1;
-    if (rowc < 0) rowc = getenv("CDML_MINE_ROWCONSTS") != nullptr ? 1 : 0;
-    if (resb_applicable(D) && B >= 8 * kBM && rowc) {
-      EpiMine<kBN, 5> epi5{dp, guid32, best, cand, stats};
-      rc = launch_gemm_resb(ctx, e16, 3 * ld16, e16 + cand * ld16, 3 * ld16, B, B, D, dtype16, epi5, st);
-    } else if (resb_applicable(D) && B >= 8 * kBM && epi_warps() == 16)
-      rc = launch_gemm_resb<EpiMine<kBN, 1>, 16>(ctx, e16, 3 * ld16, e16 + cand * ld16, 3 * ld16, B, B, D, dtype16, epi, st);
-    else if (resb_applicable(D) && B >= 8 * kBM)
-      rc = launch_gemm_resb(ctx, e16, 3 * ld16, e16 + cand * ld16, 3 * ld16, B, B, D, dtype16, epi, st);
-    else
-      rc = launch_gemm<0, 0>(ctx, e16, 3 * ld16, e16 + cand * ld16, 3 * ld16, B, B, D, dtype16, 1, epi, st);
-  }
+  CUtensorMap ta, tb;
+  int rc = make_tmap_2d(ctx, &ta, e16, dtype16, D, B, 3 * ld16, kBK, kBM);
+  if (rc) return rc;
+  {
+    const cuuint64_t dims[3] = {static_cast<cuuint64_t>(D), 2, static_cast<cuuint64_t>(B)};
+    const cuuint64_t strides[2] = {static_cast<cuuint64_t>(ld16) * 2, static_cast<cuuint64_t>(ld16) * 6};
+    const cuuint32_t box[3] = {kBK, 2, kMineTile / 4};
+    const cuuint32_t estr[3] = {1, 1, 1};
+    CUresult r = ctx->encode_tiled(&tb, dtype16 == CDML_BF16 ? CU_TENSOR_MAP_DATA_TYPE_BFLOAT16 : CU_TENSOR_MAP_DATA_TYPE_FLOAT16,
+                                   3, const_cast<uint16_t*>(e16 + ld16), dims, strides, box, estr,
+                                   CU_TENSOR_MAP_INTERLEAVE_NONE, CU_TENSOR_MAP_SWIZZLE_128B,
+                                   CU_TENSOR_MAP_L2_PROMOTION_L2_256B, CU_TENSOR_MAP_FLOAT_OOB_FILL_NONE);
+    CDML_REQUIRE(r == CUDA_SUCCESS, "cdml_mine_semihard: candidate tensor map failed with CUresult %d", (int)r);
+  }
+  static bool attr_set = false;
+  if (!attr_set) {
+    CDML_CHECK_CUDA(cudaFuncSetAttribute(mine_pair_kernel, cudaFuncAttributeMaxDynamicSharedMemorySize, MineSmem::kTotal));
+    attr_set = true;
+  }
+  const long units = static_cast<long>(s.n_ab) * s.ranges;
+  const int clusters = static_cast<int>(units < pairs ? units : pairs);
+  cudaLaunchConfig_t cfg = {};
+  cfg.gridDim = dim3(2 * clusters);
+  cfg.blockDim = dim3(kGemmThreads);
+  cfg.dynamicSmemBytes = MineSmem::kTotal;
+  cfg.stream = st;
+  cudaLaunchAttribute attr[1];
+  attr[0].id = cudaLaunchAttributeClusterDimension;
+  attr[0].val.clusterDim.x = 2, attr[0].val.clusterDim.y = 1, attr[0].val.clusterDim.z = 1;
+  cfg.attrs = attr;
+  cfg.numAttrs = 1;
+  MineArgs args{dp, guid32, guidc, best, stats};
+  CDML_CHECK_CUDA(cudaLaunchKernelEx(&cfg, mine_pair_kernel, ta, tb, s, args));
+  if (trace_sync("mine_pair", B, 2 * B, D, 2 * clusters, st)) rc = -2;
   if (rc >= 0) {
     mine_finalize_kernel<<<grid, 256, 0, st>>>(E32, ld32, D, best, B, neg_row, d_an, stats);
     rc = cudaGetLastError() == cudaSuccess ? 0 : -2;
```

New measurement: 5.982 million (median of 6 runs). 1.01x the previous value.
